# GRatTWCU/Social-STGCNN

Hardware: AMD Instinct MI355X
Metric: scene-windows/sec fwd+bwd (obs=8,pred=12) (higher is better)
Workload: dtype f32; 1 GPU; synthetic V=32 scene-windows, obs 8 / pred 12, batch 2048 per GPU, f32 (BASELINE north-star: V<=32, batch=2048; SURVEY 8d generator); global_batch=2048, step=aggregation + forward + bivariate NLL + backward + SGD update, parallelism=dp1

## Files before the change

include/stgcnn_hip.h:

```cpp
#ifndef STGCNN_HIP_H
#define STGCNN_HIP_H

#include <stddef.h>
#include <stdint.h>

#ifdef __cplusplus
extern "C" {
#endif

#define STG_OK 0
#define STG_EINVAL (-1)
#define STG_EUNSUPPORTED (-2)
#define STG_ELDS (-3)

#define STG_ABI_VERSION 8
#define STG_MAX_BLOCKS 4

int stg_abi_version(void);
const char *stg_last_error(void);

int stg_adj_build(const float *rel, int64_t rel_sn, int64_t rel_sv, int64_t rel_sc, int64_t rel_st,
                  const int32_t *num_peds, int N, int V, int T, int normalize,
                  float *nodes, float *adj, void *stream);

int stg_spatial_agg_fwd(const float *x, int64_t x_sn, int64_t x_sc, int64_t x_st, int64_t x_sv,
                        const float *adj, int64_t a_sn, const int32_t *num_peds,
                        int N, int C, int T, int V, float *y, void *stream);
int stg_spatial_agg_bwd(const float *dy, const float *adj, int64_t a_sn, const int32_t *num_peds,
                        int N, int C, int T, int V, float *dx, void *stream);

int stg_conv_t_fwd(const float *x, int64_t x_sn, int64_t x_sc, int64_t x_st, int64_t x_sv,
                   const float *w, const float *b, const int32_t *num_peds,
                   int N, int Cin, int Cout, int T, int V, int kt, int pad, float *y, void *stream);
int stg_conv_t_bwd(const float *x, int64_t x_sn, int64_t x_sc, int64_t x_st, int64_t x_sv,
                   const float *w, const float *dy, const int32_t *num_peds,
                   int N, int Cin, int Cout, int T, int V, int kt, int pad,
                   float *dx, float *dw, float *db, void *stream);

typedef struct {
    int32_t n_stgcnn;
    int32_t n_txpcnn;
    int32_t c_in;
    int32_t c_out;
    int32_t t_obs;
    int32_t t_pred;
    int32_t kt;
    int32_t residual0;
    int32_t use_mdn;
    int32_t bn_mode;
    float bn_eps;
    float bn_momentum;
    int32_t flags;
    int32_t wg_waves;
} stg_model_desc;

#define STG_OPT_WG_PATH 1
#define STG_OPT_SPLIT_BF16 2
#define STG_OPT_BF16_STORE 8
#define STG_OPT_F32_MFMA 16
#define STG_OPT_SEPARATE_FB 32
#define STG_OPT_GENERIC_WGRAD 64
#define STG_OPT_WAVE_PATH 4

int64_t stg_model_param_count(const stg_model_desc *d);
int64_t stg_model_buffer_count(const stg_model_desc *d);
int64_t stg_model_ws_floats(const stg_model_desc *d, int V);
int64_t stg_model_ws_tail_floats(const stg_model_desc *d, int N, int V);
int64_t stg_model_stat_floats(const stg_model_desc *d);
int64_t stg_model_fwd_scratch_floats(const stg_model_desc *d, int N, int V);
int64_t stg_model_bwd_scratch_floats(const stg_model_desc *d, int N, int V);
int64_t stg_model_fwd_stamps_offset(const stg_model_desc *d, int N, int V);
int64_t stg_model_bwd_stamps_offset(const stg_model_desc *d, int N, int V);

int stg_model_fwd(const stg_model_desc *d, const float *params, const float *buffers,
                  const float *x, int64_t x_sn, int64_t x_sc, int64_t x_st, int64_t x_sv,
                  const float *adj, int64_t a_sn, const int32_t *num_peds, int N, int V,
                  float *y, float *ws, float *stats, float *scratch, void **events, int n_events, void *stream);
int stg_model_bwd(const stg_model_desc *d, const float *params, const float *buffers,
                  const float *x, int64_t x_sn, int64_t x_sc, int64_t x_st, int64_t x_sv,
                  const float *adj, int64_t a_sn, const int32_t *num_peds, int N, int V,
                  const float *dy, const float *ws, float *scratch, float *grad_params, float *dx,
                  void **events, int n_events, void *stream);

int stg_model_bwd_nll(const stg_model_desc *d, const float *params, const float *buffers, const float *x, int64_t x_sn,
                      int64_t x_sc, int64_t x_st, int64_t x_sv, const float *adj, int64_t a_sn, const int32_t *num_peds,
                      int N, int V, const float *y, const float *target, const float *weights, float *losses,
                      const float *ws, float *scratch, float *grad_params, void **events, int n_events, void *stream);

typedef struct stg_step_tail {
    float *params;
    const float *lr_dev;
    float lr;
    const float *stats;
    float *buffers;
    int64_t *const *nbt;
    int n_bn;
    float *total;
} stg_step_tail;
int stg_model_bwd_step(const stg_model_desc *d, const float *params, const float *buffers, const float *x, int64_t x_sn,
                       int64_t x_sc, int64_t x_st, int64_t x_sv, const float *adj, int64_t a_sn, const int32_t *num_peds,
                       int N, int V, const float *y, const float *target, const float *weights, float *losses,
                       const float *ws, float *scratch, float *grad_params, const stg_step_tail *tail, void **events,
                       int n_events, void *stream);
int stg_model_step(const stg_model_desc *d, const float *params, const float *buffers, const float *x, int64_t x_sn,
                   int64_t x_sc, int64_t x_st, int64_t x_sv, const float *adj, int64_t a_sn, const int32_t *num_peds,
                   int N, int V, float *y, float *ws, float *stats, float *fwd_scratch, const float *target,
                   const float *weights, float *losses, float *bwd_scratch, float *grad_params,
                   const stg_step_tail *tail, void **fwd_events, int n_fwd_events, void **bwd_events,
                   int n_bwd_events, void *stream);
int stg_bn_fold(const stg_model_desc *d, const float *stats, const int32_t *num_peds, int N,
                float *buffers, int64_t *const *nbt, int n_bn, void *stream);

int stg_nll_fwd(const float *pred, int64_t p_sn, int64_t p_sf, int64_t p_sp, int64_t p_sv,
                const float *target, const int32_t *num_peds, const float *grad_scale, int N, int P, int V,
                float *loss, float *grad, void *stream);
int stg_nll_bwd(const float *grad, const float *gloss, int N, int P, int V, float *out, void *stream);

int stg_sgd_step(float *params, const float *grads, int64_t count, float lr, void *stream);

int stg_scene_order(const int32_t *num_peds, int N, int V, int32_t *order, int32_t *key_start, void *stream);

int stg_optim_step(float *params, float *grads, int64_t count, const float *lr_dev, float lr, float max_norm,
                   float *grad_norm, void *stream);

int stg_gather_windows(const float *seq_rel_all, const int32_t *win_start, const int32_t *index, int n_windows, int N,
                       int V, int T_obs, int T_pred, float *obs_rel, float *target, int32_t *num_peds, void *stream);

int stg_dp_pack(const float *grads, const float *bn_before, const float *bn_after, const int32_t *num_peds, int N,
                float momentum, int rank, int world, int n_params, int n_buffers, float *pack, void *stream);
int stg_dp_fold(const float *pack, const float *bn_before, float momentum, int rank, int world, int n_params,
                int n_buffers, float *buffers, int64_t *const *nbt, int n_bn, void *stream);
int stg_weighted_sum(const float *values, const float *weights, int N, float *out, void *stream);

int stg_train_tail(const stg_model_desc *d, const float *stats, const int32_t *num_peds, int N, float *buffers,
                   int64_t *const *nbt, int n_bn, const float *losses, const float *weights, float *total,
                   float *params, float *grads, int64_t count, const float *lr_dev, float lr, float max_norm,
                   float *grad_norm, void *stream);

int stg_bestofk_eval(const float *pred, int64_t p_sn, int64_t p_sf, int64_t p_sp, int64_t p_sv,
                     const float *target_rel, const float *obs_last, const int32_t *num_peds, const float *noise,
                     uint64_t seed, int N, int P, int V, int K, float *ade, float *fde, void *stream);

int stg_sample_trajectories(const float *pred, int64_t p_sn, int64_t p_sf, int64_t p_sp, int64_t p_sv,
                            const float *obs_last, const int32_t *num_peds, const float *noise, uint64_t seed,
                            const uint64_t *seed_dev, int N, int P, int V, int K, float *samples, float *mean,
                            void *stream);

#define STG_TRACK_MAX_DETECTIONS 2048
#define STG_TRACK_MAX_SLOTS 2048
#define STG_TRACK_DUPLICATE 1
#define STG_TRACK_OVERFLOW 2
#define STG_TRACK_TRUNCATED 4
#define STG_TRACK_TOO_MANY 8
int stg_frame_scene_counts(const int32_t *frame_start, const int64_t *ids, int F, int T_obs, int32_t *count,
                           void *stream);
int stg_frame_scenes(const int32_t *frame_start, const int64_t *ids, const double *xy, const int32_t *frames, int N,
                     int V, int T_obs, double scale, double *obs_abs, int64_t *out_ids, int32_t *num_peds,
                     void *stream);
int stg_track_push(const int64_t *det_id, const double *det_xy, const int32_t *det_count, int M_max, int64_t *slot_id,
                   uint32_t *mask, double *ring, int32_t *head_flags, int S, int T_obs, double scale, int V,
                   double *obs_abs, int64_t *out_ids, int32_t *num_peds, void *stream);

#define STG_TRACK_MAX_STREAMS 4096
#define STG_TRACK_MAX_TOTAL_DETECTIONS (STG_TRACK_MAX_STREAMS * STG_TRACK_MAX_DETECTIONS)
int stg_track_push_streams(const int64_t *det_id, int64_t id_stride, const double *det_xy, int64_t xy_stride,
                           int M_total, const int32_t *det_start, const int32_t *pushed, int NS, int M_max,
                           int64_t *slot_id, uint32_t *mask, double *ring, int32_t *head_flags, int S, int T_obs,
                           double scale, int V, double *obs_abs, int64_t *out_ids, int32_t *num_peds,
                           int32_t *out_flags, int block_threads, void *stream);

int stg_fill_tracks(double *obs_abs, const int32_t *seen, const int32_t *num_peds, int N, int T_obs, int V,
                    double scale, void *stream);
int stg_frame_scene_counts_rule(const int32_t *frame_start, const int64_t *ids, int F, int T_obs, int min_seen,
                                int max_gap, int32_t *count, void *stream);
int stg_frame_scenes_rule(const int32_t *frame_start, const int64_t *ids, const double *xy, const int32_t *frames,
                          int N, int V, int T_obs, double scale, int min_seen, int max_gap, double *obs_abs,
                          int64_t *out_ids, int32_t *num_peds, int32_t *seen, void *stream);
int stg_track_push_rule(const int64_t *det_id, const double *det_xy, const int32_t *det_count, int M_max,
                        int64_t *slot_id, uint32_t *mask, double *ring, int32_t *head_flags, int S, int T_obs,
                        double scale, int V, int min_seen, int max_gap, double *obs_abs, int64_t *out_ids,
                        int32_t *num_peds, int32_t *seen, void *stream);
int stg_track_push_streams_rule(const int64_t *det_id, int64_t id_stride, const double *det_xy, int64_t xy_stride,
                                int M_total, const int32_t *det_start, const int32_t *pushed, int NS, int M_max,
                                int64_t *slot_id, uint32_t *mask, double *ring, int32_t *head_flags, int S, int T_obs,
                                double scale, int V, int min_seen, int max_gap, double *obs_abs, int64_t *out_ids,
                                int32_t *num_peds, int32_t *out_flags, int32_t *seen, int block_threads,
                                void *stream);

#define STG_TRACK_MAX_HISTORY 256
#define STG_TRACK_TIME_ORDER 16
int stg_track_push_timed(const int64_t *det_id, const double *det_xy, const int32_t *det_count,
                         const int64_t *det_time, int M_max, int64_t *slot_id, int64_t *t_ring, double *xy_ring,
                         int32_t *slot_head, int64_t *clock, int32_t *head_flags, int S, int R, int T_obs, double scale,
                         int V, int64_t step, int64_t max_dt, int min_seen, int max_gap, double *obs_abs,
                         int64_t *out_ids, int32_t *num_peds, int32_t *seen, void *stream);
int stg_track_push_streams_timed(const int64_t *det_id, int64_t id_stride, const double *det_xy, int64_t xy_stride,
                                 int M_total, const int32_t *det_start, const int32_t *pushed, const int64_t *det_time,
                                 int NS, int M_max, int64_t *slot_id, int64_t *t_ring, double *xy_ring,
                                 int32_t *slot_head, int64_t *clock, int32_t *head_flags, int S, int R, int T_obs,
                                 double scale, int V, int64_t step, int64_t max_dt, int min_seen, int max_gap,
                                 double *obs_abs, int64_t *out_ids, int32_t *num_peds, int32_t *out_flags,
                                 int32_t *seen, int block_threads, void *stream);

#define STG_RISK_MAX_V 256
#define STG_RISK_MAX_K 64
#define STG_RISK_MAX_Z 16
#define STG_RISK_MAX_P 32
int stg_sample_risk(const float *pred, int64_t p_sn, int64_t p_sf, int64_t p_sp, int64_t p_sv, const float *obs_last,
                    const int32_t *num_peds, const float *noise, uint64_t seed, const uint64_t *seed_dev, int N, int P,
                    int V, int K, float radius, const float *zones, int64_t z_sn, int Z, int32_t *conflict,
                    int32_t *conflict_any, int32_t *partner, int32_t *pair, int32_t *zone_any, int32_t *zone_count,
                    int32_t *ped_zone, void *stream);

#define STG_SCORE_MAX_V 256
#define STG_SCORE_MAX_K 64
#define STG_SCORE_MAX_P 32
#define STG_SCORE_MAX_Q 4
typedef struct stg_score_state {
    int64_t *rec_ids;
    int32_t *rec_peds;
    float *rec_mean, *rec_cov, *rec_samples, *acc, *acc_mean;
    int32_t *steps, *head;
    double *totals, *traj_totals;
} stg_score_state;
typedef struct stg_score_out {
    int64_t *rec_ids;
    int32_t *matched;
    float *err, *d2, *nll, *best;
    int32_t *traj_steps;
    float *traj_ade, *traj_fde, *traj_ade_mean, *traj_fde_mean;
} stg_score_out;
int stg_score_push(const int64_t *det_id, const double *det_xy, const int32_t *det_count, int M_max, double scale,
                   const float *mean, const float *v_pred, int64_t p_sn, int64_t p_sf, int64_t p_sp, int64_t p_sv,
                   const float *samples, const int64_t *ids, const int32_t *num_peds, int P, int V, int K,
                   const stg_score_state *state, const float *thr, int Q, const stg_score_out *out, void *stream);
int stg_score_push_streams(const int64_t *det_id, int64_t id_stride, const double *det_xy, int64_t xy_stride,
                           int M_total, const int32_t *det_start, const int32_t *pushed, int NS, int M_max,
                           double scale, const float *mean, const float *v_pred, int64_t p_sn, int64_t p_sf,
                           int64_t p_sp, int64_t p_sv, const float *samples, const int64_t *ids,
                           const int32_t *num_peds, int P, int V, int K, const stg_score_state *state,
                           const float *thr, int Q, const stg_score_out *out, void *stream);


#define STG_ASSOC_MAX_SLOTS STG_TRACK_MAX_SLOTS
#define STG_ASSOC_MAX_DETECTIONS STG_TRACK_MAX_DETECTIONS
#define STG_ASSOC_FULL 1
int stg_associate(int64_t *det_id, const double *det_xy, const int32_t *det_count, int M_max, int64_t *trk_id,
                  double *trk_pos, double *trk_vel, int32_t *trk_miss, int32_t *trk_hits, int64_t *next_id,
                  int32_t *assoc_flags, int C, double scale, double gate2, double gate_new2, int max_miss,
                  void *stream);
int stg_associate_streams(int64_t *det_id, int64_t id_stride, const double *det_xy, int64_t xy_stride, int M_total,
                          const int32_t *det_start, const int32_t *pushed, int NS, int M_max, int64_t *trk_id,
                          double *trk_pos, double *trk_vel, int32_t *trk_miss, int32_t *trk_hits, int64_t *next_id,
                          int32_t *assoc_flags, int C, double scale, double gate2, double gate_new2, int max_miss,
                          void *stream);

int stg_selftest_mfma(const float *a, const float *b, int K, float *c, void *stream);

#include "stgcnn_hip_score_time.h"

#include "stgcnn_hip_harvest.h"

#include "stgcnn_hip_harvest_time.h"

#include "stgcnn_hip_assoc_time.h"

#include "stgcnn_hip_assoc_filter.h"

#ifdef __cplusplus
}
#endif
#endif
```

social_stgcnn_amd/_lib.py:

```python
import ctypes
import os
import subprocess

import torch

_HERE = os.path.dirname(os.path.abspath(__file__))
CSRC = os.path.join(_HERE, "csrc")
DIAG = os.environ.get("STG_USE_DIAG_LIB", "0") not in ("", "0")
LIB_PATH = os.path.join(CSRC, "libstgcnn_hip_diag.so" if DIAG else "libstgcnn_hip.so")
ABI_VERSION = 8
OPT_WG_PATH, OPT_SPLIT_BF16, OPT_WAVE_PATH, OPT_BF16_STORE, OPT_F32_MFMA, OPT_SEPARATE_FB = 1, 2, 4, 8, 16, 32
OPT_GENERIC_WGRAD = 64
EUNSUPPORTED = -2

c_f = ctypes.c_void_p
c_i = ctypes.c_int
c_l = ctypes.c_int64


class ModelDesc(ctypes.Structure):
    _fields_ = [("n_stgcnn", ctypes.c_int32), ("n_txpcnn", ctypes.c_int32), ("c_in", ctypes.c_int32),
                ("c_out", ctypes.c_int32), ("t_obs", ctypes.c_int32), ("t_pred", ctypes.c_int32),
                ("kt", ctypes.c_int32), ("residual0", ctypes.c_int32), ("use_mdn", ctypes.c_int32),
                ("bn_mode", ctypes.c_int32), ("bn_eps", ctypes.c_float), ("bn_momentum", ctypes.c_float),
                ("flags", ctypes.c_int32), ("wg_waves", ctypes.c_int32)]


class ScoreState(ctypes.Structure):
    _fields_ = [(n, ctypes.c_void_p) for n in ("rec_ids", "rec_peds", "rec_mean", "rec_cov", "rec_samples", "acc",
                                               "acc_mean", "steps", "head", "totals", "traj_totals")]


class ScoreOut(ctypes.Structure):
    _fields_ = [(n, ctypes.c_void_p) for n in ("rec_ids", "matched", "err", "d2", "nll", "best", "traj_steps",
                                               "traj_ade", "traj_fde", "traj_ade_mean", "traj_fde_mean")]


class ScoreTimedState(ctypes.Structure):
    _fields_ = [(n, ctypes.c_void_p) for n in ("rec_t", "rec_status", "rec_peds", "rec_ids", "rec_mean", "rec_cov",
                                               "rec_samples", "acc", "acc_mean", "steps", "matched", "err", "d2", "nll",
                                               "best", "traj_steps", "traj_ade", "traj_fde", "traj_ade_mean",
                                               "traj_fde_mean", "counters", "totals", "traj_totals")]


class ScoreTimedOut(ctypes.Structure):
    _fields_ = [(n, ctypes.c_void_p) for n in ("push_totals", "push_traj")]


_SIGNATURES = {
    "stg_abi_version": (c_i, []),
    "stg_last_error": (ctypes.c_char_p, []),
    "stg_adj_build": (c_i, [c_f, c_l, c_l, c_l, c_l, c_f, c_i, c_i, c_i, c_i, c_f, c_f, c_f]),
    "stg_spatial_agg_fwd": (c_i, [c_f, c_l, c_l, c_l, c_l, c_f, c_l, c_f, c_i, c_i, c_i, c_i, c_f, c_f]),
    "stg_spatial_agg_bwd": (c_i, [c_f, c_f, c_l, c_f, c_i, c_i, c_i, c_i, c_f, c_f]),
    "stg_conv_t_fwd": (c_i, [c_f, c_l, c_l, c_l, c_l, c_f, c_f, c_f, c_i, c_i, c_i, c_i, c_i, c_i, c_i, c_f, c_f]),
    "stg_conv_t_bwd": (c_i, [c_f, c_l, c_l, c_l, c_l, c_f, c_f, c_f, c_i, c_i, c_i, c_i, c_i, c_i, c_i,
                             c_f, c_f, c_f, c_f]),
    "stg_model_param_count": (c_l, [ctypes.POINTER(ModelDesc)]),
    "stg_model_buffer_count": (c_l, [ctypes.POINTER(ModelDesc)]),
    "stg_model_ws_floats": (c_l, [ctypes.POINTER(ModelDesc), c_i]),
    "stg_model_ws_tail_floats": (c_l, [ctypes.POINTER(ModelDesc), c_i, c_i]),
    "stg_model_stat_floats": (c_l, [ctypes.POINTER(ModelDesc)]),
    "stg_model_fwd_scratch_floats": (c_l, [ctypes.POINTER(ModelDesc), c_i, c_i]),
    "stg_model_bwd_scratch_floats": (c_l, [ctypes.POINTER(ModelDesc), c_i, c_i]),
    "stg_model_fwd_stamps_offset": (c_l, [ctypes.POINTER(ModelDesc), c_i, c_i]),
    "stg_model_bwd_stamps_offset": (c_l, [ctypes.POINTER(ModelDesc), c_i, c_i]),
    "stg_model_fwd": (c_i, [ctypes.POINTER(ModelDesc), c_f, c_f, c_f, c_l, c_l, c_l, c_l, c_f, c_l, c_f, c_i, c_i,
                            c_f, c_f, c_f, c_f, ctypes.POINTER(ctypes.c_void_p), c_i, c_f]),
    "stg_model_bwd": (c_i, [ctypes.POINTER(ModelDesc), c_f, c_f, c_f, c_l, c_l, c_l, c_l, c_f, c_l, c_f, c_i, c_i,
                            c_f, c_f, c_f, c_f, c_f, ctypes.POINTER(ctypes.c_void_p), c_i, c_f]),
    "stg_model_bwd_nll": (c_i, [ctypes.POINTER(ModelDesc), c_f, c_f, c_f, c_l, c_l, c_l, c_l, c_f, c_l, c_f, c_i, c_i,
                                c_f, c_f, c_f, c_f, c_f, c_f, c_f, ctypes.POINTER(ctypes.c_void_p), c_i, c_f]),
    "stg_model_bwd_step": (c_i, [ctypes.POINTER(ModelDesc), c_f, c_f, c_f, c_l, c_l, c_l, c_l, c_f, c_l, c_f, c_i, c_i,
                                 c_f, c_f, c_f, c_f, c_f, c_f, c_f, ctypes.c_void_p, ctypes.POINTER(ctypes.c_void_p), c_i,
                                 c_f]),
    "stg_model_step": (c_i, [ctypes.POINTER(ModelDesc), c_f, c_f, c_f, c_l, c_l, c_l, c_l, c_f, c_l, c_f, c_i, c_i,
                             c_f, c_f, c_f, c_f, c_f, c_f, c_f, c_f, c_f, ctypes.c_void_p,
                             ctypes.POINTER(ctypes.c_void_p), c_i, ctypes.POINTER(ctypes.c_void_p), c_i, c_f]),
    "stg_bn_fold": (c_i, [ctypes.POINTER(ModelDesc), c_f, c_f, c_i, c_f, ctypes.POINTER(ctypes.c_void_p), c_i, c_f]),
    "stg_nll_fwd": (c_i, [c_f, c_l, c_l, c_l, c_l, c_f, c_f, c_f, c_i, c_i, c_i, c_f, c_f, c_f]),
    "stg_nll_bwd": (c_i, [c_f, c_f, c_i, c_i, c_i, c_f, c_f]),
    "stg_sgd_step": (c_i, [c_f, c_f, c_l, ctypes.c_float, c_f]),
    "stg_scene_order": (c_i, [c_f, c_i, c_i, c_f, c_f, c_f]),
    "stg_optim_step": (c_i, [c_f, c_f, c_l, c_f, ctypes.c_float, ctypes.c_float, c_f, c_f]),
    "stg_bestofk_eval": (c_i, [c_f, c_l, c_l, c_l, c_l, c_f, c_f, c_f, c_f, ctypes.c_uint64, c_i, c_i, c_i, c_i,
                               c_f, c_f, c_f]),
    "stg_sample_trajectories": (c_i, [c_f, c_l, c_l, c_l, c_l, c_f, c_f, c_f, ctypes.c_uint64, c_f, c_i, c_i, c_i, c_i,
                                      c_f, c_f, c_f]),
    "stg_sample_risk": (c_i, [c_f, c_l, c_l, c_l, c_l, c_f, c_f, c_f, ctypes.c_uint64, c_f, c_i, c_i, c_i, c_i,
                              ctypes.c_float, c_f, c_l, c_i, c_f, c_f, c_f, c_f, c_f, c_f, c_f, c_f]),
    "stg_gather_windows": (c_i, [c_f, c_f, c_f, c_i, c_i, c_i, c_i, c_i, c_f, c_f, c_f, c_f]),
    "stg_dp_pack": (c_i, [c_f, c_f, c_f, c_f, c_i, ctypes.c_float, c_i, c_i, c_i, c_i, c_f, c_f]),
    "stg_dp_fold": (c_i, [c_f, c_f, ctypes.c_float, c_i, c_i, c_i, c_i, c_f, ctypes.POINTER(ctypes.c_void_p), c_i, c_f]),
    "stg_weighted_sum": (c_i, [c_f, c_f, c_i, c_f, c_f]),
    "stg_train_tail": (c_i, [ctypes.POINTER(ModelDesc), c_f, c_f, c_i, c_f, ctypes.POINTER(ctypes.c_void_p), c_i, c_f, c_f,
                             c_f, c_f, c_f, c_l, c_f, ctypes.c_float, ctypes.c_float, c_f, c_f]),
    "stg_frame_scene_counts": (c_i, [c_f, c_f, c_i, c_i, c_f, c_f]),
    "stg_frame_scenes": (c_i, [c_f, c_f, c_f, c_f, c_i, c_i, c_i, ctypes.c_double, c_f, c_f, c_f, c_f]),
    "stg_track_push": (c_i, [c_f, c_f, c_f, c_i, c_f, c_f, c_f, c_f, c_i, c_i, ctypes.c_double, c_i, c_f, c_f, c_f,
                             c_f]),
    "stg_track_push_streams": (c_i, [c_f, c_l, c_f, c_l, c_i, c_f, c_f, c_i, c_i, c_f, c_f, c_f, c_f, c_i, c_i,
                                     ctypes.c_double, c_i, c_f, c_f, c_f, c_f, c_i, c_f]),
    "stg_fill_tracks": (c_i, [c_f, c_f, c_f, c_i, c_i, c_i, ctypes.c_double, c_f]),
    "stg_frame_scene_counts_rule": (c_i, [c_f, c_f, c_i, c_i, c_i, c_i, c_f, c_f]),
    "stg_frame_scenes_rule": (c_i, [c_f, c_f, c_f, c_f, c_i, c_i, c_i, ctypes.c_double, c_i, c_i, c_f, c_f, c_f, c_f,
                                    c_f]),
    "stg_track_push_rule": (c_i, [c_f, c_f, c_f, c_i, c_f, c_f, c_f, c_f, c_i, c_i, ctypes.c_double, c_i, c_i, c_i,
                                  c_f, c_f, c_f, c_f, c_f]),
    "stg_track_push_streams_rule": (c_i, [c_f, c_l, c_f, c_l, c_i, c_f, c_f, c_i, c_i, c_f, c_f, c_f, c_f, c_i, c_i,
                                          ctypes.c_double, c_i, c_i, c_i, c_f, c_f, c_f, c_f, c_f, c_i, c_f]),
    "stg_track_push_timed": (c_i, [c_f, c_f, c_f, c_f, c_i, c_f, c_f, c_f, c_f, c_f, c_f, c_i, c_i, c_i,
                                   ctypes.c_double, c_i, c_l, c_l, c_i, c_i, c_f, c_f, c_f, c_f, c_f]),
    "stg_track_push_streams_timed": (c_i, [c_f, c_l, c_f, c_l, c_i, c_f, c_f, c_f, c_i, c_i, c_f, c_f, c_f, c_f, c_f,
                                           c_f, c_i, c_i, c_i, ctypes.c_double, c_i, c_l, c_l, c_i, c_i, c_f, c_f, c_f,
                                           c_f, c_f, c_i, c_f]),
    "stg_score_push": (c_i, [c_f, c_f, c_f, c_i, ctypes.c_double, c_f, c_f, c_l, c_l, c_l, c_l, c_f, c_f, c_f, c_i, c_i,
                             c_i, ctypes.POINTER(ScoreState), c_f, c_i, ctypes.POINTER(ScoreOut), c_f]),
    "stg_score_push_streams": (c_i, [c_f, c_l, c_f, c_l, c_i, c_f, c_f, c_i, c_i, ctypes.c_double, c_f, c_f, c_l, c_l,
                                     c_l, c_l, c_f, c_f, c_f, c_i, c_i, c_i, ctypes.POINTER(ScoreState), c_f, c_i,
                                     ctypes.POINTER(ScoreOut), c_f]),
    "stg_associate": (c_i, [c_f, c_f, c_f, c_i, c_f, c_f, c_f, c_f, c_f, c_f, c_f, c_i, ctypes.c_double,
                            ctypes.c_double, ctypes.c_double, c_i, c_f]),
    "stg_associate_streams": (c_i, [c_f, c_l, c_f, c_l, c_i, c_f, c_f, c_i, c_i, c_f, c_f, c_f, c_f, c_f, c_f, c_f,
                                    c_i, ctypes.c_double, ctypes.c_double, ctypes.c_double, c_i, c_f]),
    "stg_selftest_mfma": (c_i, [c_f, c_f, c_i, c_f, c_f]),
}
EXPORTS = tuple(_SIGNATURES)
_SIGNATURES_SCORE_TIME = {
    "stg_score_push_timed": (c_i, [c_f, c_f, c_f, c_f, c_f, c_f, c_i, c_i, ctypes.c_double, c_l, c_l, c_f, c_f, c_l, c_l,
                                   c_l, c_l, c_f, c_f, c_f, c_i, c_i, c_i, c_i, c_f, c_f, c_i, c_f, c_f]),
    "stg_score_push_streams_timed": (c_i, [c_f, c_f, c_f, c_f, c_f, c_f, c_f, c_i, c_i, c_i, ctypes.c_double, c_l, c_l,
                                           c_f, c_f, c_l, c_l, c_l, c_l, c_f, c_f, c_f, c_i, c_i, c_i, c_i, c_f, c_f, c_i,
                                           c_f, c_f]),
}
_SIGNATURES_HARVEST = {
    "stg_window_harvest": (c_i, [c_f, c_f, c_f, c_f, c_i, c_i, c_i, c_i, c_i, c_f, c_f, c_f, c_f, c_f, c_f, c_f, c_i, c_i,
                                 c_f]),
    "stg_window_harvest_streams": (c_i, [c_f, c_f, c_f, c_f, c_f, c_i, c_i, c_i, c_i, c_i, c_f, c_f, c_f, c_f, c_f, c_f,
                                         c_f, c_f, c_i, c_i, c_f]),
}
c_d = ctypes.c_double
_SIGNATURES_HARVEST_TIME = {
    "stg_window_harvest_timed": (c_i, [c_f, c_f, c_f, c_f, c_f, c_f, c_i, c_i, c_i, c_i, c_i, c_d, c_l, c_l, c_l, c_i,
                                       c_f, c_f, c_f, c_f, c_f, c_f, c_f, c_f, c_i, c_i, c_f]),
    "stg_window_harvest_streams_timed": (c_i, [c_f, c_f, c_f, c_f, c_f, c_f, c_f, c_i, c_i, c_i, c_i, c_i, c_i, c_d, c_l,
                                               c_l, c_l, c_f, c_f, c_f, c_f, c_f, c_f, c_f, c_f, c_f, c_i, c_i, c_f]),
}
_SIGNATURES_ASSOC_TIME = {
    "stg_associate_timed": (c_i, [c_f, c_f, c_f, c_f, c_f, c_i, c_f, c_f, c_f, c_f, c_f, c_f, c_f, c_i, c_d, c_d, c_d, c_l,
                                  c_l, c_f]),
    "stg_associate_streams_timed": (c_i, [c_f, c_l, c_f, c_l, c_i, c_f, c_f, c_f, c_f, c_i, c_i, c_f, c_f, c_f, c_f, c_f,
                                          c_f, c_f, c_i, c_d, c_d, c_d, c_l, c_l, c_f]),
}
_SIGNATURES_ASSOC_FILTER = {
    "stg_associate_filtered": (c_i, [c_f, c_f, c_f, c_f, c_f, c_i, c_f, c_f, c_f, c_f, c_f, c_f, c_f, c_f, c_i, c_d, c_d,
                                     c_d, c_d, c_d, c_d, c_l, c_l, c_f]),
    "stg_associate_streams_filtered": (c_i, [c_f, c_l, c_f, c_l, c_i, c_f, c_f, c_f, c_f, c_i, c_i, c_f, c_f, c_f, c_f,
                                             c_f, c_f, c_f, c_f, c_i, c_d, c_d, c_d, c_d, c_d, c_d, c_l, c_l, c_f]),
}

_lib = None


def build(verbose=False):
    cmd = ["make", "-C", CSRC, "-j8"] + (["DIAG=1"] if DIAG else [])
    res = subprocess.run(cmd, stdout=subprocess.PIPE, stderr=subprocess.STDOUT, text=True)
    if verbose or res.returncode != 0:
        print(res.stdout)
    if res.returncode != 0:
        raise RuntimeError("building libstgcnn_hip.so failed (exit %d)" % res.returncode)
    return LIB_PATH


def lib():
    global _lib
    if _lib is None:
        if not os.path.exists(LIB_PATH):
            raise RuntimeError(
                "social_stgcnn_amd: %s is missing -- build it with `make -C %s` (hipcc, "
                "--offload-arch=gfx950) or `python -c 'import __graft_entry__ as g; g.build()'`. "
                "There is no CPU or eager-PyTorch fallback for this path." % (LIB_PATH, CSRC))
        h = ctypes.CDLL(LIB_PATH)
        for name, (res, args) in {**_SIGNATURES, **_SIGNATURES_SCORE_TIME, **_SIGNATURES_HARVEST,
                                    **_SIGNATURES_HARVEST_TIME, **_SIGNATURES_ASSOC_TIME,
                                    **_SIGNATURES_ASSOC_FILTER}.items():
            fn = getattr(h, name)
            fn.restype = res
            fn.argtypes = args
        if h.stg_abi_version() != ABI_VERSION:
            raise RuntimeError("libstgcnn_hip.so ABI %d != binding ABI %d" % (h.stg_abi_version(), ABI_VERSION))
        _lib = h
    return _lib


class StepTail(ctypes.Structure):
    _fields_ = [("params", ctypes.c_void_p), ("lr_dev", ctypes.c_void_p), ("lr", ctypes.c_float),
                ("stats", ctypes.c_void_p), ("buffers", ctypes.c_void_p), ("nbt", ctypes.POINTER(ctypes.c_void_p)),
                ("n_bn", ctypes.c_int), ("total", ctypes.c_void_p)]


class HipEvents:
    _hip = None

    @classmethod
    def hip(cls):
        if cls._hip is None:
            h = ctypes.CDLL("libamdhip64.so")
            h.hipEventCreate.argtypes = [ctypes.POINTER(ctypes.c_void_p)]
            h.hipEventElapsedTime.argtypes = [ctypes.POINTER(ctypes.c_float), ctypes.c_void_p, ctypes.c_void_p]
            h.hipEventSynchronize.argtypes = [ctypes.c_void_p]
            h.hipEventDestroy.argtypes = [ctypes.c_void_p]
            cls._hip = h
        return cls._hip

    def __init__(self, n):
        self.n = n
        self.arr = (ctypes.c_void_p * n)()
        for i in range(n):
            ev = ctypes.c_void_p()
            if self.hip().hipEventCreate(ctypes.byref(ev)) != 0:
                raise RuntimeError("hipEventCreate failed")
            self.arr[i] = ev

    def intervals_ms(self):
        out = []
        self.hip().hipEventSynchronize(self.arr[self.n - 1])
        for k in range(1, self.n):
            ms = ctypes.c_float()
            if self.hip().hipEventElapsedTime(ctypes.byref(ms), self.arr[k - 1], self.arr[k]) != 0:
                raise RuntimeError("hipEventElapsedTime failed")
            out.append(ms.value)
        return out

    def __del__(self):
        try:
            for i in range(self.n):
                self.hip().hipEventDestroy(self.arr[i])
        except Exception:
            pass


def check(rc, what):
    if rc != 0:
        msg = lib().stg_last_error().decode("utf-8", "replace")
        raise RuntimeError("%s failed (status %d): %s" % (what, rc, msg))


def stream_ptr():
    return ctypes.c_void_p(torch.cuda.current_stream().cuda_stream)


def ptr(t):
    if t is None:
        return None
    return ctypes.c_void_p(t.data_ptr())


def require_gpu(*tensors):
    for t in tensors:
        if t is not None and not t.is_cuda:
            raise RuntimeError("social_stgcnn_amd runs on MI355X only: got a %s tensor (no CPU fallback)"
                               % t.device.type)


def seed_u64(seed):
    return int(seed) & 0xFFFFFFFFFFFFFFFF


def seed_i64(seed):
    s = seed_u64(seed)
    return s - (1 << 64) if s >= 1 << 63 else s


def as_f32(t, what):
    if t.dtype != torch.float32:
        raise TypeError("%s must be float32 (got %s)" % (what, t.dtype))
    return t


def peds_arg(num_peds, n, device):
    if num_peds is None:
        return None
    if not torch.is_tensor(num_peds):
        num_peds = torch.as_tensor(num_peds, dtype=torch.int32)
    num_peds = num_peds.to(device=device, dtype=torch.int32).contiguous()
    if num_peds.numel() != n:
        raise ValueError("num_peds has %d entries for a batch of %d scenes" % (num_peds.numel(), n))
    return num_peds
```

social_stgcnn_amd/csrc/model_bwd.hip:

```cpp
#include "model_common.hpp"
#include "stgcn_block.hpp"
#include "txp_scene_common.hpp"
#include "txp_f32_operands.hpp"
#include "step_plan.hpp"
#include "txp_wgrad.hpp"
#include "tail_parts.hpp"
#include "nll_elem.hpp"

namespace stg {

struct BwdArgs {
    ModelLayout lay;
    const float *params, *buffers, *x;
    int64_t x_sn, x_sc, x_st, x_sv;
    const float *adj;
    int64_t a_sn;
    const int32_t *num_peds;
    int N, V;
    const float *dy, *ws;
    const float *nll_target, *nll_weights;
    float *nll_losses;
    int64_t ws_stride;
    float *slab1;
    float *dzg;
// ... 93 lines not shown
    const ModelLayout &L = a.lay;
    const int scmax = txp_sc(Vl);
    const int plane_floats = P * scmax;
    const int st_floats = (2 * C * (T + 2) + C * T) * Vl;
    const int reg_floats = plane_floats > st_floats ? plane_floats : st_floats;
    const int dcur_floats = P * C * Vl;
    const int n_small = L.n_blk_params + L.n_txp;
    float *gsm = sm;
    float *dzb = gsm + ((n_small + 3) & ~3);
    float *dcur = dzb + reg_floats;
    float *red = dcur + dcur_floats;
    float *tot = red + WAVES * kRedMax;
    const float *Pm = params;
    __shared__ float nll_part[WAVES];

    for (int e = tid; e < n_small; e += NT) gsm[e] = 0.f;

    int t_begin, t_end;
    tier_range(a.tier, a.N, V, t_begin, t_end);
    const int M = t_end - t_begin;
    for (int r = 0; r * (int)gridDim.x < M; ++r) {
        const int it = walk_item(r, blockIdx.x, gridDim.x, M, a.tier.order != nullptr && a.tier.serpentine);
        if (it < 0) continue;
        const int n = a.tier.order ? a.tier.order[t_begin + it] : it;
        int vi = a.num_peds ? a.num_peds[n] : V;
        vi = vi < 0 ? 0 : (vi > V ? V : vi);
        float *dxn = a.dx ? a.dx + (int64_t)n * L.blk[0].cin * T * V : nullptr;
        if (dxn && vi < V)
            for (int e = tid; e < L.blk[0].cin * T * (V - vi); e += NT) {
                const int r = e / (V - vi), w = vi + (e - r * (V - vi));
                dxn[(int64_t)r * V + w] = 0.f;
            }
        if (vi == 0) {
            if (a.nll_target && tid == 0) a.nll_losses[n] = 0.f;
            continue;
        }
        const float *wsn = a.ws + n * a.ws_stride;
        const int SW = txp_sw(vi), SC = txp_sc(vi), npos = C * vi;
        const int out_rows = L.n_txp > 0 ? C * P : C * T;
        const float *dyn = a.dy + (int64_t)n * out_rows * V;
        __syncthreads();
        if (L.n_txp > 0) {
            for (int e = tid; e < P * SC; e += NT) dzb[e] = 0.f;
            __syncthreads();
            for (int l = L.L; l >= 0; --l) {
                const bool is_out = l == L.L;
                if (is_out) {
                    float *dzo = a.dzg + ((int64_t)n * (L.L + 1) + L.L) * dz_slot(V);
                    constexpr int U = 4;
                    if (a.nll_target) {
                        bwd_nll_stage(dyn, a.nll_target + (int64_t)n * P * V * 2, a.nll_weights ? a.nll_weights[n] : 1.f,
                                      vi, V, SC, SW, dzb, dzo, nll_part, a.nll_losses + n);
                    } else
                    for (int e0 = tid; e0 < P * npos; e0 += NT * U) {
                        float dv[U];
                        int li[U];
#pragma unroll
                        for (int u = 0; u < U; ++u) {
                            const int e = e0 + u * NT;
                            const int ec = e < P * npos ? e : 0;
                            const int ch = ec / npos, p = ec - ch * npos, h = p / vi, w = p - h * vi;
                            li[u] = ch * SC + (h + 1) * SW + (w + 1);
                            dv[u] = dyn[(int64_t)(ch * C + h) * V + w];
                        }
#pragma unroll
                        for (int u = 0; u < U; ++u)
                            if (e0 + u * NT < P * npos) {
                                const int e = e0 + u * NT, ch = e / npos;
                                dzb[li[u]] = dv[u];
                                dzo[(e - ch * npos) * P + ch] = dv[u];
                            }
                    }
                    __syncthreads();
                } else {
                    const float *zl = wsn + L.ws_hdr_floats + (int64_t)L.ws_z[l] * V;
                    float *dzo = a.dzg + ((int64_t)n * (L.L + 1) + l) * dz_slot(V);
                    const float alpha = Pm[L.prelus + l];
                    float s[1] = {0.f};
                    constexpr int U = 4;
                    for (int e0 = tid; e0 < P * npos; e0 += NT * U) {
                        float zv[U];
#pragma unroll
                        for (int u = 0; u < U; ++u) {
                            const int e = e0 + u * NT;
                            zv[u] = e < P * npos ? zl[e] : 1.f;
                        }
#pragma unroll
                        for (int u = 0; u < U; ++u) {
                            const int e = e0 + u * NT;
                            if (e < P * npos) {
                                const int ch = e / npos, p = e - ch * npos, h = p / vi, w = p - h * vi;
                                const float z = zv[u], d = dcur[e];
                                float dz = d;
                                if (!(z > 0.f)) {
                                    dz = alpha * d;
                                    s[0] = fmaf(d, z, s[0]);
                                }
                                dzb[ch * SC + (h + 1) * SW + (w + 1)] = dz;
                                dzo[p * P + ch] = dz;
                            }
                        }
                    }
                    block_reduce<1, WAVES>(s, red, tot);
                    if (tid == 0) gsm[L.n_blk_params + l] += tot[0];
                }
                const int w_off = is_out ? L.out_w : L.txp_w[l];
                if (!STG_SKIP(a, 2)) {
                    if (l == 0)
                        txp_dgrad<Cfg::T, WAVES>(Pm + w_off, dzb, dcur, vi, false);
                    else
                        txp_dgrad<Cfg::P, WAVES>(Pm + w_off, dzb, dcur, vi, !is_out);
                }
                __syncthreads();
            }
        } else {
            for (int e = tid; e < C * T * vi; e += NT) {
                const int r = e / vi, w = e - r * vi;
                dcur[e] = dyn[(int64_t)r * V + w];
            }
            __syncthreads();
        }
        float *H1 = dzb, *DH2 = dzb + C * (T + 2) * Vl, *DB1 = DH2 + C * (T + 2) * Vl;
        for (int j = L.n_blocks - 1; j >= 0 && !STG_SKIP(a, 4); --j) {
            const float *xin = j > 0 ? wsn + L.ws_hdr_floats + (int64_t)L.blk[j - 1].ws_s * V : nullptr;
            float *dxs = j > 0 ? dcur : nullptr;
            float *dxg = j == 0 ? dxn : nullptr;
            if (L.blk[j].cin == Cfg::CIN0)
                stgcn_block_bwd<Cfg::CIN0, WAVES, true>(a, params, L.blk[j], n, vi, dcur, H1, DH2, DB1, red, tot, gsm, wsn,
                                                        xin, dxs, dxg, nullptr);
            else
                stgcn_block_bwd<Cfg::C, WAVES, true>(a, params, L.blk[j], n, vi, dcur, H1, DH2, DB1, red, tot, gsm, wsn, xin,
                                                     dxs, dxg, nullptr);
        }
    }
    __syncthreads();
    float *slab = a.slab1 + (int64_t)blockIdx.x * n_small;
    for (int e = tid; e < n_small; e += NT) slab[e] = gsm[e];
}

struct ReduceSeg {
    int p0, len, rows, row_stride;
    int64_t base;
};
struct ReduceArgs {
    ReduceSeg seg[kMaxTxp + 3];
    int n_seg;
    const float *slabs;
    float *grad;
    int n_params;
};

struct TailArgs {
    float *params;
    const float *lr_dev;
    float lr;
    const float *stats, *losses, *weights;
    const int32_t *num_peds;
    float *buffers, *total;
    NbtPtrs nbt;
    int n_reduce, n_buffers, N, stat_floats;
    float momentum;
};

__global__ __launch_bounds__(256) void reduce_slabs_kernel(const ReduceArgs a, const TailArgs t_) {
    __shared__ float part[32][8];
    if ((int)blockIdx.x >= t_.n_reduce) {
        float *acc_s = &part[0][0];
        __shared__ float dec_s[256];
        __shared__ int cnt_s[256];
        const int b = (int)blockIdx.x - t_.n_reduce;
        if (b < t_.n_buffers)
            bn_fold_body<256>(b, t_.stats, t_.num_peds, t_.N, t_.stat_floats, t_.momentum, t_.buffers, t_.nbt, acc_s, dec_s,
                              cnt_s);
        else if (t_.total)
            weighted_sum_body(t_.losses, t_.weights, t_.N, t_.total, acc_s);
        return;
    }
    const int col = threadIdx.x & 7, grp = threadIdx.x >> 3;
    const int p = blockIdx.x * 8 + col;
    float s = 0.f;
    if (p < a.n_params) {
        for (int q = 0; q < a.n_seg; ++q) {
            const ReduceSeg g = a.seg[q];
            if (p >= g.p0 && p < g.p0 + g.len) {
                const float *src = a.slabs + g.base + (p - g.p0);
                int k = grp;
                for (; k + 992 < g.rows; k += 1024) {
                    float v[32];
#pragma unroll
                    for (int u = 0; u < 32; ++u) v[u] = src[(int64_t)(k + 32 * u) * g.row_stride];
#pragma unroll
                    for (int u = 0; u < 32; ++u) s += v[u];
                }
                for (; k + 480 < g.rows; k += 512) {
                    float v[16];
#pragma unroll
                    for (int u = 0; u < 16; ++u) v[u] = src[(int64_t)(k + 32 * u) * g.row_stride];
#pragma unroll
                    for (int u = 0; u < 16; ++u) s += v[u];
                }
                for (; k + 96 < g.rows; k += 128) {
                    float v[4];
#pragma unroll
                    for (int u = 0; u < 4; ++u) v[u] = src[(int64_t)(k + 32 * u) * g.row_stride];
#pragma unroll
                    for (int u = 0; u < 4; ++u) s += v[u];
                }
                for (; k < g.rows; k += 32) s += src[(int64_t)k * g.row_stride];
            }
        }
    }
    part[grp][col] = s;
    __syncthreads();
    if (grp == 0 && p < a.n_params) {
        float t = 0.f;
#pragma unroll
        for (int g = 0; g < 32; ++g) t += part[g][col];
        a.grad[p] = t;
        if (t_.params) t_.params[p] -= (t_.lr_dev ? t_.lr_dev[0] : t_.lr) * t;
    }
}

static size_t bwd_lds_bytes(const ModelLayout &L, int V, int waves) {
    const int plane = Cfg::P * txp_sc(V);
    const int st = (2 * Cfg::C * (Cfg::T + 2) + Cfg::C * Cfg::T) * V;
    const int reg = plane > st ? plane : st;
    const int dcur = Cfg::P * Cfg::C * V;
    const int n_small = L.n_blk_params + L.n_txp;
    const size_t fl = ((n_small + 3) & ~3) + (size_t)reg + (size_t)dcur + (size_t)waves * kRedMax + kRedMax;
    return fl * sizeof(float);
}

static int bwd_waves(const StepPath &path, int V) {
    return path.wg_waves ? path.wg_waves : (V <= 40 ? 1 : (V <= 80 ? 4 : 8));
}

static int bwd_grid_w(const ModelLayout &L, int N, int V, int waves) {
    const size_t lds = bwd_lds_bytes(L, V, waves);
    if (lds > (size_t)kLdsBytes) return -1;
    int per_cu = (int)(kLdsBytes / lds);
    const int by_waves = 8 / waves > 0 ? 8 / waves : 1;
    if (per_cu > by_waves) per_cu = by_waves;
    if (per_cu < 1) per_cu = 1;
    int grid = kNumCU * per_cu;
    if (const int g = diag_env("STG_BWD_GRID", 0)) grid = g > 0 ? g : grid;
    return grid < N ? grid : N;
}
static int bwd_grid(const ModelLayout &L, const StepPath &path, int N, int V) { return bwd_grid_w(L, N, V, bwd_waves(path, V)); }
constexpr int kBwdTierV = 32;
static int bwd_grid_small(const ModelLayout &L, int N, int V) {
    return V > kBwdTierV ? bwd_grid_w(L, N, kBwdTierV, 1) : 0;
}

struct BwdCarve {
    int64_t rows, slab2, dzg, order, stamps, total;
};
static bool bwd_carve(const ModelLayout &L, const StepPath &path, int N, int V, BwdCarve *c, WgradGeom *wg) {
    const int g1 = bwd_grid(L, path, N, V);
    if (g1 < 0) return false;
    int gs = bwd_grid_small(L, N, V);
    if (gs < 0) gs = 0;
    int64_t n_rows = g1 + gs;
    if (path.scene() && N > n_rows) n_rows = N;
    c->rows = 0;
    int64_t fl = (n_rows * (L.n_blk_params + L.n_txp) + 3) & ~(int64_t)3;
    c->slab2 = fl;
    c->dzg = fl;
    if (L.n_txp > 0) {
        if (!wgrad_geom(L, N, V, wg)) return false;
        fl = (fl + wgrad_slab_base(L.L + 1, wg->rows) + 3) & ~(int64_t)3;
        c->dzg = fl;
        fl = (fl + (int64_t)N * (L.L + 1) * dz_slot(V) + 3) & ~(int64_t)3;
    }
    c->order = fl;
    c->total = fl + order_floats(N, V);
    c->stamps = -1;
    if (diag_env("STG_STAMPS", 0) != 0) {
        c->stamps = c->total;
        c->total += (int64_t)N * 32;
    }
    return true;
}

static int64_t bwd_query(const char *what, const stg_model_desc *d, int N, int V, int64_t BwdCarve::*item) {
    StepPlan p;
    const int rc = plan_sized(what, d, nullptr, N, V, 1, &p);
    if (rc != STG_OK) return rc;
    BwdCarve c;
    WgradGeom wg{};
    STG_REQUIRE(bwd_carve(p.lay, p.path, N, V, &c, &wg), STG_ELDS, "stg_model_bwd: V=%d does not fit the LDS of one CU", V);
    return c.*item >= 0 ? c.*item : STG_EUNSUPPORTED;
}

}

extern "C" {

int64_t stg_model_bwd_scratch_floats(const stg_model_desc *d, int N, int V) {
    return stg::bwd_query("stg_model_bwd_scratch_floats:", d, N, V, &stg::BwdCarve::total);
}
int64_t stg_model_bwd_stamps_offset(const stg_model_desc *d, int N, int V) {
    return stg::bwd_query("stg_model_bwd_stamps_offset:", d, N, V, &stg::BwdCarve::stamps);
}

}

namespace stg {

int model_bwd_impl(const ModelCall &c, const BwdBuffers &b, const StepPlan &p, const TxpFwdArgs *deferred) {
    const SceneInput &in = c.in;
    const int N = in.N, V = in.V;
    const ModelLayout &L = p.lay;
    STG_REQUIRE(b.grad_params, STG_EINVAL, "stg_model_bwd: null grad_params");
    STG_REQUIRE(N == 0 || (c.params && c.buffers && in.x && in.adj && b.dy && b.ws && b.scratch), STG_EINVAL,
                "stg_model_bwd: null pointer");
    STG_REQUIRE(aligned(b.ws, 16) && aligned(b.scratch, 16), STG_EINVAL, "stg_model_bwd: ws / scratch must be 16-byte aligned");
    hipStream_t st = as_stream(c.stream);
    EventList evl{b.events, b.events ? b.n_events : 0, 0, st};
    evl.mark();
    if (N == 0) {
        hipError_t e = hipMemsetAsync(b.grad_params, 0, sizeof(float) * L.n_params, st);
        if (e != hipSuccess) return hip_fail(e, "stg_model_bwd: memset");
        return STG_OK;
    }
    BwdCarve cv;
    WgradGeom wg{};
    const StepPath &path = p.path;
    STG_REQUIRE(bwd_carve(L, path, N, V, &cv, &wg), STG_ELDS, "stg_model_bwd: V=%d does not fit the LDS of one CU", V);
    const int n_small = L.n_blk_params + L.n_txp;
    float *rows = b.scratch + cv.rows, *slab2 = b.scratch + cv.slab2;
    float *dzg = L.n_txp > 0 ? b.scratch + cv.dzg : nullptr;
    STG_REQUIRE(path.scene() || !(L.flags & STG_OPT_BF16_STORE), STG_EUNSUPPORTED,
                "stg_model_bwd: bf16 storage (STG_OPT_BF16_STORE) is built for the wave-per-scene kernels only");
    STG_REQUIRE(!((L.flags & STG_OPT_BF16_STORE) && (L.flags & STG_OPT_SPLIT_BF16)), STG_EUNSUPPORTED,
                "stg_model_bwd: STG_OPT_BF16_STORE and STG_OPT_SPLIT_BF16 cannot be combined");
    if (b.nll_target && ((L.flags & STG_OPT_SPLIT_BF16) || L.n_txp == 0))
        return STG_EUNSUPPORTED;
    STG_REQUIRE(!(path.scene() && b.dx), STG_EUNSUPPORTED,
                "stg_model_bwd: dx is only computed by the workgroup-per-scene kernels: set STG_OPT_WG_PATH in the "
                "descriptor of the forward and the backward call");
    const float *ws_end = b.ws + p.tail.base;
    const bool in_tail = tail_has_order(path, in.num_peds, N, V);
    float *order = in_tail ? const_cast<float *>(ws_end) + p.tail.order : b.scratch + cv.order;
    const SceneOrder so = scene_order_at(reinterpret_cast<int32_t *>(order), N, V);
    const bool sorted = in_tail || launch_scene_order(in.num_peds, N, V, so, st);
    const SceneTier tier{sorted ? so.order : nullptr, sorted ? so.key_start : nullptr, -1, V, diag_env("STG_WALK", 1)};
    const auto fill = [&](auto &a) {
        set_input(a, c);
        a.lay = L; a.ws_stride = p.ws_stride; a.ws = b.ws; a.dzg = dzg;
        a.debug_skip = diag_env("STG_DEBUG_SKIP", 0);
    };
    const auto fill_k1 = [&](auto &a) {
        fill(a);
        a.dy = b.dy; a.nll_target = b.nll_target; a.nll_weights = b.nll_weights; a.nll_losses = b.nll_losses;
        a.tier = tier;
    };
    int slab_rows;
    if (path.scene()) {
        TxpBwdArgs t{};
        fill_k1(t);
        t.rows = rows; t.Vl = V;
        t.split_bf16 = (L.flags & STG_OPT_SPLIT_BF16) ? 1 : 0;
        t.stagger = diag_env("STG_STAGGER_B", 0);
        if (p.tail.wp >= 0) t.wp = reinterpret_cast<const unsigned *>(ws_end + p.tail.wp);
        if (cv.stamps >= 0) t.stamps = reinterpret_cast<unsigned long long *>(b.scratch + cv.stamps);
        STG_REQUIRE(!deferred || p.one_launch, STG_EINVAL, "stg_model_bwd: a deferred scene launch outside the one-launch step");
        const int rcw = deferred ? launch_scene_step(*deferred, t, st) : launch_scene_bwd(path, t, st);
        if (rcw != STG_OK) return rcw;
        slab_rows = N;
    } else {
        STG_REQUIRE(!deferred, STG_EINVAL, "stg_model_bwd: a deferred scene launch outside the one-launch step");
        BwdArgs a{};
        fill_k1(a);
        a.buffers = c.buffers; a.slab1 = rows; a.dx = b.dx;
        const int waves = bwd_waves(path, V);
        const size_t lds = bwd_lds_bytes(L, V, waves);
        STG_REQUIRE(lds <= (size_t)kLdsBytes, STG_ELDS, "stg_model_bwd: V=%d needs %zu bytes of LDS (> %d)", V, lds,
                    kLdsBytes);
        const int grid = bwd_grid(L, path, N, V);
        void (*k1)(BwdArgs, const float *);
        switch (waves) {
            case 1: k1 = model_bwd_kernel<1>; break;
            case 2: k1 = model_bwd_kernel<2>; break;
            case 4: k1 = model_bwd_kernel<4>; break;
            default: k1 = model_bwd_kernel<8>; break;
        }
        slab_rows = grid;
        const int grid_small = a.tier.order ? bwd_grid_small(L, N, V) : 0;
        if (grid_small > 0) a.tier.v_lo = kBwdTierV;
        int rck = launch(Launch{"stg_model_bwd: K1", dim3(grid), dim3(waves * 64), lds, st}, k1, a, c.params);
        if (rck != STG_OK) return rck;
        if (grid_small > 0) {
            a.Vl = kBwdTierV;
            a.tier.v_lo = -1; a.tier.v_hi = kBwdTierV;
            a.slab1 = rows + (int64_t)grid * n_small;
            rck = launch(Launch{"stg_model_bwd: K1 (small scenes)", dim3(grid_small), dim3(64), bwd_lds_bytes(L, kBwdTierV, 1), st},
                         model_bwd_kernel<1>, a, c.params);
            if (rck != STG_OK) return rck;
            slab_rows = grid + grid_small;
        }
    }
    evl.mark();

    ReduceArgs r{};
    r.slabs = b.scratch;
    r.grad = b.grad_params;
    r.n_params = L.n_params;
    r.seg[r.n_seg++] = ReduceSeg{0, L.n_blk_params, slab_rows, n_small, cv.rows};
    if (L.n_txp > 0) {
        r.seg[r.n_seg++] = ReduceSeg{L.prelus, L.n_txp, slab_rows, n_small, cv.rows + (int64_t)L.n_blk_params};
        WgradArgs w{};
        fill(w);
        w.order = tier.order; w.order_peds = sorted ? so.order_peds : nullptr; w.key_start = tier.key_start;
        w.serpentine = tier.serpentine;
        w.slab2 = slab2; w.rows = wg.rows;
        for (int l = 0; l <= L.L + 1; ++l) w.wg_begin[l] = wg.wg_begin[l];
        if (!STG_SKIP(w, 1)) {
            const int rck = launch_txp_wgrad(w, wg, st);
            if (rck != STG_OK) return rck;
        }
        evl.mark();
        for (int l = 0; l <= L.L; ++l) {
            const int p0 = l == L.L ? L.out_w : L.txp_w[l];
            r.seg[r.n_seg++] = ReduceSeg{p0, wgrad_row_len(l), STG_SKIP(w, 1) ? 0 : wg.wg_begin[l + 1] - wg.wg_begin[l],
                                         wgrad_row_len(l), cv.slab2 + wgrad_slab_base(l, wg.rows)};
        }
    }
    TailArgs ta{};
    ta.n_reduce = (L.n_params + 7) / 8;
    int extra = 0;
    if (const stg_step_tail *tail = b.tail) {
        ta.params = tail->params; ta.lr_dev = tail->lr_dev; ta.lr = tail->lr;
        ta.stats = tail->stats; ta.buffers = tail->buffers; ta.total = tail->total;
        ta.losses = b.nll_losses; ta.weights = b.nll_weights; ta.num_peds = in.num_peds;
        ta.N = N; ta.stat_floats = L.stat_floats; ta.momentum = c.d->bn_momentum;
        ta.n_buffers = (tail->stats && N > 0) ? L.n_buffers : 0;
        ta.nbt.n = tail->nbt ? tail->n_bn : 0;
        for (int k = 0; k < ta.nbt.n; ++k) ta.nbt.p[k] = tail->nbt[k];
        extra = ta.n_buffers + 1;
    }
    hipLaunchKernelGGL(reduce_slabs_kernel, dim3(ta.n_reduce + extra), dim3(256), 0, st, r, ta);
    STG_LAUNCH_CHECK("stg_model_bwd: reduce_slabs");
    evl.mark();
    evl.finish();
    return STG_OK;
}

static bool tail_ok(const stg_step_tail *tail) {
    return tail && tail->params && !(tail->stats && !tail->buffers) && tail->n_bn >= 0 && tail->n_bn <= 3 * STG_MAX_BLOCKS;
}

static int run_bwd(const ModelCall &c, const BwdBuffers &b) {
    StepPlan p;
    const int rc = plan_sized("stg_model_bwd: bad sizes", c.d, c.in.num_peds, c.in.N, c.in.V, 0, &p);
    return rc != STG_OK ? rc : model_bwd_impl(c, b, p, nullptr);
}

}

extern "C" {

using namespace stg;

int stg_model_bwd(const stg_model_desc *d, const float *params, const float *buffers, const float *x, int64_t x_sn,
                  int64_t x_sc, int64_t x_st, int64_t x_sv, const float *adj, int64_t a_sn, const int32_t *num_peds,
                  int N, int V, const float *dy, const float *ws, float *scratch, float *grad_params, float *dx,
                  void **events, int n_events, void *stream) {
    const ModelCall c{d, params, buffers, {x, x_sn, x_sc, x_st, x_sv, adj, a_sn, num_peds, N, V}, stream};
    return run_bwd(c, BwdBuffers{dy, nullptr, nullptr, nullptr, nullptr, ws, scratch, grad_params, dx, events, n_events});
}

int stg_model_bwd_nll(const stg_model_desc *d, const float *params, const float *buffers, const float *x, int64_t x_sn,
                      int64_t x_sc, int64_t x_st, int64_t x_sv, const float *adj, int64_t a_sn, const int32_t *num_peds,
                      int N, int V, const float *y, const float *target, const float *weights, float *losses,
                      const float *ws, float *scratch, float *grad_params, void **events, int n_events, void *stream) {
    if (!target || !losses || (N > 0 && !y)) return fail(STG_EINVAL, "stg_model_bwd_nll: null pointer");
    const ModelCall c{d, params, buffers, {x, x_sn, x_sc, x_st, x_sv, adj, a_sn, num_peds, N, V}, stream};
    return run_bwd(c, BwdBuffers{y, target, weights, losses, nullptr, ws, scratch, grad_params, nullptr, events, n_events});
}

int stg_model_bwd_step(const stg_model_desc *d, const float *params, const float *buffers, const float *x, int64_t x_sn,
                       int64_t x_sc, int64_t x_st, int64_t x_sv, const float *adj, int64_t a_sn, const int32_t *num_peds,
                       int N, int V, const float *y, const float *target, const float *weights, float *losses,
                       const float *ws, float *scratch, float *grad_params, const stg_step_tail *tail, void **events,
                       int n_events, void *stream) {
    if (!target || !losses || (N > 0 && !y)) return fail(STG_EINVAL, "stg_model_bwd_step: null pointer");
    if (!tail_ok(tail)) return fail(STG_EINVAL, "stg_model_bwd_step: bad tail");
    if (N == 0) return STG_EUNSUPPORTED;
    const ModelCall c{d, params, buffers, {x, x_sn, x_sc, x_st, x_sv, adj, a_sn, num_peds, N, V}, stream};
    return run_bwd(c, BwdBuffers{y, target, weights, losses, tail, ws, scratch, grad_params, nullptr, events, n_events});
}

int stg_model_step(const stg_model_desc *d, const float *params, const float *buffers, const float *x, int64_t x_sn,
                   int64_t x_sc, int64_t x_st, int64_t x_sv, const float *adj, int64_t a_sn, const int32_t *num_peds,
                   int N, int V, float *y, float *ws, float *stats, float *fwd_scratch, const float *target,
                   const float *weights, float *losses, float *bwd_scratch, float *grad_params,
                   const stg_step_tail *tail, void **fwd_events, int n_fwd_events, void **bwd_events,
                   int n_bwd_events, void *stream) {
    if (!target || !losses || !y || !ws) return fail(STG_EINVAL, "stg_model_step: null pointer");
    if (!tail_ok(tail)) return fail(STG_EINVAL, "stg_model_step: bad tail");
    StepPlan p;
    const int rc = plan_sized("stg_model_step: bad sizes", d, num_peds, N, V, 0, &p);
    if (rc != STG_OK) return rc;
    if (N == 0 || (p.lay.flags & STG_OPT_SPLIT_BF16) || p.lay.n_txp == 0) return STG_EUNSUPPORTED;
    STG_REQUIRE(grad_params && bwd_scratch, STG_EINVAL, "stg_model_step: null pointer");
    const ModelCall c{d, params, buffers, {x, x_sn, x_sc, x_st, x_sv, adj, a_sn, num_peds, N, V}, stream};
    TxpFwdArgs f{};
    TxpFwdArgs *both = p.one_launch ? &f : nullptr;
    const int rcf = model_fwd_impl(c, FwdBuffers{y, ws, stats, fwd_scratch, fwd_events, n_fwd_events}, p, both);
    if (rcf != STG_OK) return rcf;
    return model_bwd_impl(c, BwdBuffers{y, target, weights, losses, tail, ws, bwd_scratch, grad_params, nullptr, bwd_events,
                                        n_bwd_events}, p, both);
}

}
```

social_stgcnn_amd/csrc/model_layout.hip:

```cpp
#include <cstring>
#include <type_traits>
#include "model_common.hpp"
#include "scene_order.hpp"
#include "step_plan.hpp"
#include "txp_wave.hpp"

namespace stg {

int make_layout(const stg_model_desc *d, ModelLayout *lay) {
    STG_REQUIRE(d && lay, STG_EINVAL, "model descriptor is null");
    STG_REQUIRE(d->n_stgcnn >= 1 && d->n_stgcnn <= STG_MAX_BLOCKS, STG_EUNSUPPORTED,
                "n_stgcnn=%d outside 1..%d", d->n_stgcnn, STG_MAX_BLOCKS);
    STG_REQUIRE(d->n_txpcnn >= 0 && d->n_txpcnn <= kMaxTxp, STG_EUNSUPPORTED, "n_txpcnn=%d outside 0..%d",
                d->n_txpcnn, kMaxTxp);
    STG_REQUIRE(d->c_out == Cfg::C && d->t_obs == Cfg::T && d->kt == Cfg::KT, STG_EUNSUPPORTED,
                "fused kernels are built for output_feat=%d seq_len=%d kernel_size=%d (got %d,%d,%d)", Cfg::C,
                Cfg::T, Cfg::KT, d->c_out, d->t_obs, d->kt);
    STG_REQUIRE(d->c_in == Cfg::CIN0 || d->c_in == Cfg::C, STG_EUNSUPPORTED,
                "fused kernels are built for input_feat %d or %d (got %d)", Cfg::CIN0, Cfg::C, d->c_in);
    STG_REQUIRE(d->n_txpcnn == 0 || d->t_pred == Cfg::P, STG_EUNSUPPORTED,
                "fused kernels are built for pred_seq_len=%d (got %d)", Cfg::P, d->t_pred);
    STG_REQUIRE(d->bn_mode == 0 || d->bn_mode == 1, STG_EINVAL, "bn_mode=%d (0 eval, 1 per-scene train)", d->bn_mode);
    STG_REQUIRE(d->residual0 >= 0 && d->residual0 <= 2, STG_EINVAL, "residual0=%d", d->residual0);
    STG_REQUIRE(d->residual0 != 1 || d->c_in == d->c_out, STG_EINVAL, "identity residual needs c_in == c_out");
    STG_REQUIRE((d->flags & ~(STG_OPT_WG_PATH | STG_OPT_SPLIT_BF16 | STG_OPT_WAVE_PATH | STG_OPT_BF16_STORE | STG_OPT_F32_MFMA |
                              STG_OPT_SEPARATE_FB | STG_OPT_GENERIC_WGRAD)) == 0, STG_EINVAL,
                "unknown flags 0x%x", d->flags);
    STG_REQUIRE(d->wg_waves == 0 || d->wg_waves == 1 || d->wg_waves == 2 || d->wg_waves == 4 || d->wg_waves == 8,
                STG_EINVAL, "wg_waves=%d (0 auto, 1, 2, 4, 8)", d->wg_waves);
    ModelLayout &l = *lay;
    l = layout_of(ModelShape{d->n_stgcnn, d->n_txpcnn, d->c_in, d->residual0, d->use_mdn});
    l.bn_mode = d->bn_mode;
    l.eps = d->bn_eps;
    l.momentum = d->bn_momentum;
    l.flags = d->flags;
    l.wg_waves = d->wg_waves;
    return STG_OK;
}

bool is_canonical(const ModelLayout &L) {
    ModelLayout c = L;
    c.eps = kCanonLayout.eps;
    c.momentum = kCanonLayout.momentum;
    c.bn_mode = kCanonLayout.bn_mode;
    c.flags = kCanonLayout.flags;
    c.wg_waves = kCanonLayout.wg_waves;
    static_assert(std::is_trivially_copyable<ModelLayout>::value && sizeof(ModelLayout) % 4 == 0, "compared bytewise");
    return std::memcmp(&c, &kCanonLayout, sizeof c) == 0;
}

constexpr int kSmallBatch = 288;

static StepPath choose_path(const ModelLayout &L, int N, int V) {
    StepPath p{StepPath::Workgroup, L.wg_waves, txp_fwd_x6_fits(L, V), txp_bwd_x6_fits(L, V)};
    if (L.n_txp < 1 || L.n_blocks != 1 || L.blk[0].cin != Cfg::CIN0 || (L.flags & STG_OPT_WG_PATH)) return p;
    if (p.fwd_x6 && p.bwd_x6) {
        p.kind = StepPath::SceneX6;
    } else if (txp_wave_f32_fits(V)) {
        if (N >= kSmallBatch || L.wg_waves != 0 || V > 40 || (L.flags & (STG_OPT_WAVE_PATH | STG_OPT_BF16_STORE)))
            p.kind = StepPath::WaveF32;
        else
            p.wg_waves = N <= 192 ? 8 : 4;
    }
    return p;
}

static FwdCarve fwd_carve(const ModelLayout &L, const StepPath &path, int N, int V) {
    const bool stamps = diag_env("STG_STAMPS", 0) != 0;
    FwdCarve c;
    c.agg = 0;
    c.order = (((int64_t)N * (L.blk[0].cin + 1) * Cfg::T * V + 3) & ~(int64_t)3) + 4;
    c.stamps = stamps ? c.order + order_floats(N, V) : -1;
    const int64_t wp = (c.order + order_floats(N, V) + (stamps ? (int64_t)N * 32 : 0) + 3) & ~(int64_t)3;
    c.wp_fwd = path.scene() && path.fwd_x6 ? wp : -1;
    c.total = wp + (path.fwd_x6 ? txp_bwd_x6_wp_floats(L) : 0);
    return c;
}

static WsTail ws_tail(const ModelLayout &L, const StepPath &path, int N, int V) {
    WsTail t;
    t.base = (int64_t)N * ws_floats_per_scene(L, V);
    t.wp = path.scene() && path.bwd_x6 ? 0 : -1;
    t.order = path.bwd_x6 ? txp_bwd_x6_wp_floats(L) : 0;
    t.total = t.order + order_floats(N, V);
    return t;
}

int launch_scene_fwd(const StepPath &path, const TxpFwdArgs &a, hipStream_t st) {
    return path.fwd_x6 ? launch_txp_fwd_x6(a, st) : launch_txp_fwd_wave(a, st);
}
int launch_scene_bwd(const StepPath &path, const TxpBwdArgs &a, hipStream_t st) {
    return path.bwd_x6 ? launch_txp_bwd_x6(a, st) : launch_txp_bwd_wave(a, st);
}

static bool step_one_launch(const ModelLayout &L, const StepPath &path, const int32_t *num_peds, int N, int V) {
    return path.kind == StepPath::SceneX6 && path.fwd_x6 && path.bwd_x6 && !(L.flags & STG_OPT_SEPARATE_FB) &&
           txp_step_x6_fits(L, num_peds, N, V);
}
int launch_scene_step(const TxpFwdArgs &f, const TxpBwdArgs &b, hipStream_t st) { return launch_txp_step_x6(f, b, st); }

int plan_step(const stg_model_desc *d, const int32_t *num_peds, int N, int V, StepPlan *p) {
    const int rc = make_layout(d, &p->lay);
    p->sized = rc == STG_OK && N >= 0 && V > 0;
    if (!p->sized) return rc;
    const ModelLayout &L = p->lay;
    p->path = choose_path(L, N, V);
    p->ws_stride = ws_floats_per_scene(L, V);
    p->tail = ws_tail(L, p->path, N, V);
    p->fwd = fwd_carve(L, p->path, N, V);
    p->one_launch = step_one_launch(L, p->path, num_peds, N, V);
    return STG_OK;
}
int plan_sized(const char *what, const stg_model_desc *d, const int32_t *num_peds, int N, int V, int min_N, StepPlan *p) {
    const int rc = plan_step(d, num_peds, N, V, p);
    if (rc != STG_OK) return rc;
    STG_REQUIRE(p->sized && N >= min_N, STG_EINVAL, "%s N=%d V=%d", what, N, V);
    return STG_OK;
}

__global__ __launch_bounds__(1024) void scene_order_kernel(const int32_t *__restrict__ num_peds, int N, int V,
                                                           int32_t *__restrict__ order,
                                                           int32_t *__restrict__ key_start,
                                                           int32_t *__restrict__ order_peds) {
    extern __shared__ int hist[];
    __shared__ int wave_tot[16];
    scene_order_body<16>(num_peds, N, V, order, key_start, order_peds, hist, wave_tot);
}

bool launch_scene_order(const int32_t *num_peds, int N, int V, const SceneOrder &o, hipStream_t st) {
    if (!o.order || !scene_order_applies(num_peds, N, V)) return false;
    const size_t lds = (size_t)(V + 1) * 16 * sizeof(int);
    if (lds > 48 * 1024 &&
        hipFuncSetAttribute(reinterpret_cast<const void *>(&scene_order_kernel),
                            hipFuncAttributeMaxDynamicSharedMemorySize, (int)lds) != hipSuccess)
        return false;
    hipLaunchKernelGGL(scene_order_kernel, dim3(1), dim3(1024), lds, st, num_peds, N, V, o.order, o.key_start, o.order_peds);
    return hipGetLastError() == hipSuccess;
}

}

extern "C" {

static int64_t layout_query(const stg_model_desc *d, int32_t stg::ModelLayout::*count) {
    stg::ModelLayout l;
    const int rc = stg::make_layout(d, &l);
    return rc == STG_OK ? l.*count : rc;
}
int64_t stg_model_param_count(const stg_model_desc *d) { return layout_query(d, &stg::ModelLayout::n_params); }
int64_t stg_model_buffer_count(const stg_model_desc *d) { return layout_query(d, &stg::ModelLayout::n_buffers); }
int64_t stg_model_stat_floats(const stg_model_desc *d) { return layout_query(d, &stg::ModelLayout::stat_floats); }
int64_t stg_model_ws_floats(const stg_model_desc *d, int V) {
    stg::ModelLayout l;
    const int rc = stg::make_layout(d, &l);
    if (rc != STG_OK) return rc;
    if (V <= 0) return stg::fail(STG_EINVAL, "stg_model_ws_floats: V=%d", V);
    return stg::ws_floats_per_scene(l, V);
}
int64_t stg_model_ws_tail_floats(const stg_model_desc *d, int N, int V) {
    stg::StepPlan p;
    const int rc = stg::plan_sized("stg_model_ws_tail_floats:", d, nullptr, N, V, 0, &p);
    return rc == STG_OK ? p.tail.total : rc;
}
int64_t stg_model_fwd_scratch_floats(const stg_model_desc *d, int N, int V) {
    stg::StepPlan p;
    const int rc = stg::plan_sized("stg_model_fwd_scratch_floats:", d, nullptr, N, V, 0, &p);
    return rc == STG_OK ? p.fwd.total : rc;
}
int64_t stg_model_fwd_stamps_offset(const stg_model_desc *d, int N, int V) {
    stg::StepPlan p;
    const int rc = stg::plan_sized("stg_model_fwd_stamps_offset:", d, nullptr, N, V, 0, &p);
    return rc != STG_OK ? rc : p.fwd.stamps >= 0 ? p.fwd.stamps : STG_EUNSUPPORTED;
}
int stg_scene_order(const int32_t *num_peds, int N, int V, int32_t *order, int32_t *key_start, void *stream) {
    STG_REQUIRE(N >= 0 && V > 0, STG_EINVAL, "stg_scene_order: bad sizes N=%d V=%d", N, V);
    if (N == 0) return STG_OK;
    STG_REQUIRE(num_peds && order, STG_EINVAL, "stg_scene_order: null pointer");
    STG_REQUIRE(N >= 2, STG_EUNSUPPORTED, "stg_scene_order: a single scene needs no order");
    STG_REQUIRE(N <= stg::kOrderMaxN && V <= stg::kOrderMaxV, STG_EUNSUPPORTED,
                "stg_scene_order: N=%d V=%d outside the single-workgroup sort (N <= %d, V <= %d)", N, V,
                stg::kOrderMaxN, stg::kOrderMaxV);
    STG_REQUIRE(stg::launch_scene_order(num_peds, N, V, stg::SceneOrder{order, key_start, nullptr}, stg::as_stream(stream)),
                STG_EINVAL, "stg_scene_order: launch failed");
    return STG_OK;
}

}
```

social_stgcnn_amd/csrc/step_plan.hpp:

```cpp
#pragma once
#include "model_common.hpp"

namespace stg {

struct TxpFwdArgs;
struct TxpBwdArgs;

struct StepPath {
    enum Kind { SceneX6, WaveF32, Workgroup } kind;
    int wg_waves;
    bool fwd_x6, bwd_x6;
    bool scene() const { return kind != Workgroup; }
};

struct FwdCarve {
    int64_t agg, order, stamps, wp_fwd, total;
};

struct WsTail {
    int64_t base, wp, order, total;
};
inline bool tail_has_order(const StepPath &path, const int32_t *num_peds, int N, int V) {
    return path.scene() && scene_order_applies(num_peds, N, V);
}

int launch_scene_fwd(const StepPath &path, const TxpFwdArgs &a, hipStream_t st);
int launch_scene_bwd(const StepPath &path, const TxpBwdArgs &a, hipStream_t st);

int launch_scene_step(const TxpFwdArgs &f, const TxpBwdArgs &b, hipStream_t st);

struct StepPlan {
    ModelLayout lay;
    bool sized, one_launch;
    StepPath path;
    int64_t ws_stride;
    WsTail tail;
    FwdCarve fwd;
};
int plan_step(const stg_model_desc *d, const int32_t *num_peds, int N, int V, StepPlan *p);
int plan_sized(const char *what, const stg_model_desc *d, const int32_t *num_peds, int N, int V, int min_N, StepPlan *p);

struct SceneInput {
    const float *x; int64_t x_sn, x_sc, x_st, x_sv; const float *adj; int64_t a_sn; const int32_t *num_peds; int N, V;
};
struct ModelCall { const stg_model_desc *d; const float *params, *buffers; SceneInput in; void *stream; };
struct FwdBuffers { float *y, *ws, *stats, *scratch; void **events; int n_events; };
struct BwdBuffers {
    const float *dy, *nll_target, *nll_weights; float *nll_losses;
    const stg_step_tail *tail;
    const float *ws; float *scratch, *grad_params, *dx; void **events; int n_events;
};

template <class A> constexpr auto has_batch(int) -> decltype(A::x, true) { return true; }
template <class A> constexpr bool has_batch(...) { return false; }
template <class A>
void set_input(A &a, const ModelCall &c) {
    const SceneInput &in = c.in;
    a.num_peds = in.num_peds; a.N = in.N; a.V = in.V;
    if constexpr (has_batch<A>(0)) {
        a.params = c.params; a.x = in.x; a.x_sn = in.x_sn; a.x_sc = in.x_sc; a.x_st = in.x_st; a.x_sv = in.x_sv;
        a.adj = in.adj; a.a_sn = in.a_sn;
    }
}

int model_fwd_impl(const ModelCall &c, const FwdBuffers &b, const StepPlan &p, TxpFwdArgs *defer);
int model_bwd_impl(const ModelCall &c, const BwdBuffers &b, const StepPlan &p, const TxpFwdArgs *deferred);

}
```

social_stgcnn_amd/csrc/txp_scene_common.hpp:

```cpp
#pragma once
#include "model_common.hpp"
#include "stgcn_block.hpp"

namespace stg {

struct MixGeom {
    int on;
    int v_small, v_mid;
    int block_floats;
};

constexpr int kTeamMaxV = 128;
struct TeamGeom {
    int on;
    int v1, v2;
    int region_floats;
};

struct TxpFwdArgs {
    ModelLayout lay;
    const float *params, *buffers;
    const int32_t *num_peds;
    SceneTier tier;
    int Vl;
    MixGeom mix;
    TeamGeom team;
    int N, V;
    const float *x;
    int64_t x_sn, x_sc, x_st, x_sv;
    const float *adj;
    int64_t a_sn;
    const float *agg;
    int64_t agg_stride, agg_ax, agg_cs;
    float *y;
    const unsigned *wpf;
    float *ws;
    int64_t ws_stride;
    float *stats;
    unsigned long long *stamps;
    int debug_skip;
    int stagger;
};

struct TxpBwdArgs {
    ModelLayout lay;
    const float *params;
    const int32_t *num_peds;
    SceneTier tier;
    int Vl;
    MixGeom mix;
    TeamGeom team;
    int N, V;
    const float *x;
    int64_t x_sn, x_sc, x_st, x_sv;
    const float *adj;
    int64_t a_sn;
    const float *dy;
    const float *nll_target;
    const float *nll_weights;
    float *nll_losses;
    const float *ws;
    int64_t ws_stride;
    float *dzg;
    const unsigned *wp;
    float *rows;
    unsigned long long *stamps;
    int debug_skip;
    int split_bf16;
    int stagger;
};

bool txp_fwd_x6_fits(const ModelLayout &L, int V);
bool txp_bwd_x6_fits(const ModelLayout &L, int V);
int64_t txp_bwd_x6_wp_floats(const ModelLayout &L);
int launch_txp_fwd_x6(const TxpFwdArgs &a, hipStream_t st);
int launch_txp_bwd_x6(const TxpBwdArgs &a, hipStream_t st);
bool txp_step_x6_fits(const ModelLayout &L, const int32_t *num_peds, int N, int V);
int launch_txp_step_x6(const TxpFwdArgs &f, const TxpBwdArgs &b, hipStream_t st);

__host__ __device__ inline int ptab_floats(int v) { return ((Cfg::T * v + 1) / 2 + 3) & ~3; }
__host__ __device__ inline int bwd_ptab_floats(int v) { return ptab_floats(v) + kRedMax; }
__host__ __device__ inline int wave_param_floats(const ModelLayout &L) {
    return ((L.n_blk_params + 3) & ~3) + ((L.n_buffers + 3) & ~3);
}

__device__ __forceinline__ void build_ptab(ptab_t *ptab, int vi) {
    const int lane = threadIdx.x & 63;
    for (int p = lane; p < Cfg::T * vi; p += 64) {
        const int h = p / vi;
        ptab[p] = (ptab_t)((h << 8) | (p - h * vi));
    }
}
__device__ __forceinline__ void build_ptab(ptab_t *ptab, int w0, int wc) {
    const int lane = threadIdx.x & 63;
    if (wc <= 0 && lane == 0) ptab[0] = 0;
    for (int p = lane; p < Cfg::T * wc; p += 64) {
        const int h = p / wc;
        ptab[p] = (ptab_t)((h << 8) | (w0 + p - h * wc));
    }
}


__device__ __forceinline__ void vm_drain() { __builtin_amdgcn_s_waitcnt(0x0F70); }

__device__ __forceinline__ void stage_block_params(const ModelLayout &L, const float *__restrict__ params,
                                                   const float *__restrict__ buffers, float *blk_p, float *blk_b, int nt) {
    for (int e = threadIdx.x; e < L.n_blk_params; e += nt) blk_p[e] = params[e];
    if (buffers)
        for (int e = threadIdx.x; e < L.n_buffers; e += nt) blk_b[e] = buffers[e];
    __syncthreads();
}

inline int wave_wpb(size_t per_wave) {
    int wpb = diag_env("STG_TXP_WPB", 4);
    if (wpb != 1 && wpb != 2 && wpb != 8) wpb = 4;
    while (wpb > 1 && per_wave * wpb > (size_t)kLdsBytes) wpb >>= 1;
    return wpb;
}

inline int wave_grid(size_t lds, int wpb, int N) {
    int per_cu = (int)(kLdsBytes / lds);
    if (per_cu * wpb > 8) per_cu = 8 / wpb;
    if (per_cu < 1) per_cu = 1;
    const int need = (N + wpb - 1) / wpb;
    const int g = kNumCU * per_cu;
    if (g >= need) return need;
    const int rounds = (need + g - 1) / g;
    return (need + rounds - 1) / rounds;
}

}
```

social_stgcnn_amd/csrc/txp_wgrad.hip:

```cpp
#include "txp_wgrad.hpp"

namespace stg {

namespace {

constexpr int C = Cfg::C, P = Cfg::P;
constexpr int kWaves = 8;

__device__ __forceinline__ void wait_vmcnt(int n) {
    switch (n) {
        case 0: asm volatile("s_waitcnt vmcnt(0)" ::: "memory"); break;
        case 1: asm volatile("s_waitcnt vmcnt(1)" ::: "memory"); break;
        case 2: asm volatile("s_waitcnt vmcnt(2)" ::: "memory"); break;
        case 3: asm volatile("s_waitcnt vmcnt(3)" ::: "memory"); break;
        case 4: asm volatile("s_waitcnt vmcnt(4)" ::: "memory"); break;
        case 5: asm volatile("s_waitcnt vmcnt(5)" ::: "memory"); break;
        case 6: asm volatile("s_waitcnt vmcnt(6)" ::: "memory"); break;
        case 7: asm volatile("s_waitcnt vmcnt(7)" ::: "memory"); break;
        case 8: asm volatile("s_waitcnt vmcnt(8)" ::: "memory"); break;
        default: asm volatile("s_waitcnt vmcnt(0)" ::: "memory"); break;
    }
}

__device__ __forceinline__ void dma_piece(const float *__restrict__ src, float *lds_dst, int nvec, int piece) {
    const int lane = threadIdx.x & 63;
    const int e = piece * 64 + lane;
    const unsigned dst = __builtin_amdgcn_readfirstlane(
        (unsigned)(uintptr_t)(__attribute__((address_space(3))) float *)(lds_dst + 256 * piece));
    if (e < nvec) {
        const float *g = src + 4 * e;
        unsigned keep;
        asm volatile("s_mov_b32 %0, m0\n\ts_mov_b32 m0, %2\n\ts_nop 0\n\tglobal_load_lds_dwordx4 %1, off\n\ts_mov_b32 m0, %0"
                     : "=&s"(keep)
                     : "v"(g), "s"(dst)
                     : "memory");
    }
}

struct Item {
    int vi, w0, vc;
    bool valid;
    const float *pl, *dz;
};

template <int CINL, int NBUF, bool BF>
__device__ __forceinline__ void wgrad_layer(const WgradArgs &a, const int32_t *__restrict__ order,
                                            const int32_t *__restrict__ order_peds, const int32_t *__restrict__ num_peds,
                                            int layer, float *sm, int wg, int nwg) {
    constexpr int NCOL = 9 * CINL + 1, NTILE = (NCOL + 15) / 16;
    const ModelLayout &L = a.lay;
    const int V = a.V, tid = threadIdx.x, lane = tid & 63;
    const int wave = __builtin_amdgcn_readfirstlane(tid >> 6);
    const int nq = lane & 15, kq = lane >> 4;
    const int co_a = nq < P ? nq : P - 1;
    constexpr int ES = BF ? 2 : 4;
    const int image = wgrad_image_floats(V, BF), pslot = wgrad_plane_floats(V, BF);
    auto ld = [&](const float *base, int idx) -> float {
        if (BF) return __uint_as_float((unsigned)reinterpret_cast<const unsigned short *>(base)[idx] << 16);
        return base[idx];
    };
    const int nch = wgrad_chunks(V), items = a.N * nch;
    const int64_t plane_off = ws_plane_off(L, V, layer), dzs_floats = dz_slot(V);
    int tapr[NTILE], tapc[NTILE], cic[NTILE];
    bool bone[NTILE];
#pragma unroll
    for (int tl = 0; tl < NTILE; ++tl) {
        int col = tl * 16 + nq;
        bone[tl] = col == NCOL - 1;
        if (col > NCOL - 2) col = NCOL - 2;
        const int tap = col / CINL;
        cic[tl] = col - tap * CINL;
        tapr[tl] = tap / 3 - 1;
        tapc[tl] = tap % 3 - 1;
    }
    f32x4 acc[NTILE];
#pragma unroll
    for (int tl = 0; tl < NTILE; ++tl) acc[tl] = f32x4{0.f, 0.f, 0.f, 0.f};

    struct Raw { int at, n, v; };
    auto fetch = [&](int r) -> Raw {
        Raw w{-1, 0, 0};
        w.at = walk_item(r, wg, nwg, items, order != nullptr && a.serpentine);
        if (w.at >= 0) {
            const int si = nch > 1 ? w.at / nch : w.at;
            w.n = order ? order[si] : si;
            w.v = order ? order_peds[si] : (num_peds ? num_peds[si] : V);
        }
        return w;
    };
    auto finish = [&](const Raw &w) -> Item {
        Item it{0, 0, 0, false, nullptr, nullptr};
        if (w.at < 0) return it;
        const int chunk = nch > 1 ? w.at - (w.at / nch) * nch : 0;
        const int vfull = w.v < 0 ? 0 : (w.v > V ? V : w.v);
        const int nc = wgrad_chunks(vfull);
        if (vfull == 0 || chunk >= nc) return it;
        int wc = vfull;
        if (nc > 1) wc = (vfull + nc - 1) / nc;
        if (BF && nc > 1) wc = (wc + 1) & ~1;
        it.pl = a.ws + w.n * a.ws_stride + plane_off;
        it.dz = a.dzg + ((int64_t)w.n * (L.L + 1) + layer) * dzs_floats;
        it.vi = vfull;
        it.w0 = chunk * wc;
        it.vc = (vfull - it.w0) < wc ? (vfull - it.w0) : wc;
        it.valid = true;
        return it;
    };
    auto stage = [&](const Item &it, float *buf) -> int {
        if (!it.valid || STG_SKIP(a, 64)) return 0;
        const int vi = it.vi, vc = it.vc, w0 = it.w0;
        const int SWf = save_sw(vi, BF), VWf = save_vw(vi, BF);
        const int SWc = save_sw(vc, BF), VWc = save_vw(vc, BF);
        if (tid < 2 * SWc * 3) {
            const int b = tid / 3, q = tid - b * 3;
            const int pos = b < SWc ? b : (C + 1) * SWc + (b - SWc);
            store_vec4(buf, pos * 3 + q, f32x4{0.f, 0.f, 0.f, 0.f}, BF);
        }
        const float *pl = it.pl, *dz = it.dz;
        int issued = 0;
        if (vc == vi) {
            const int nv0 = (C * SWf * P * ES + 15) >> 4, nv1 = (C * VWf * P * ES + 15) >> 4;
            const int np0 = (nv0 + 63) >> 6, np1 = (nv1 + 63) >> 6;
            for (int q = wave; q < np0 + np1; q += kWaves) {
                if (q < np0) dma_piece(pl, buf + (SWc * P * ES) / 4, nv0, q);
                else dma_piece(dz, buf + pslot, nv1, q - np0);
                ++issued;
            }
        } else {
            const int nvp = (SWc * P * ES + 15) >> 4, nvd = (vc * P * ES + 15) >> 4;
            const int npp = (nvp + 63) >> 6, npd = (nvd + 63) >> 6;
            for (int q = wave; q < C * (npp + npd); q += kWaves) {
                if (q < C * npp) {
                    const int h = q / npp, pc = q - h * npp;
                    dma_piece(pl + ((int64_t)(h * SWf + w0) * P * ES) / 4, buf + ((h + 1) * SWc * P * ES) / 4, nvp, pc);
                } else {
                    const int q2 = q - C * npp, h = q2 / npd, pc = q2 - h * npd;
                    dma_piece(dz + ((int64_t)(h * VWf + w0) * P * ES) / 4, buf + pslot + (h * VWc * P * ES) / 4, nvd, pc);
                }
                ++issued;
            }
        }
        return issued;
    };
    auto compute = [&](const Item &it, const float *buf) {
        if (!it.valid || STG_SKIP(a, 128)) return;
        const float *plane = buf, *dzs = buf + pslot;
        const int vc = it.vc, SW = save_sw(vc, BF), VW = save_vw(vc, BF), npos = C * vc, nsteps = (npos + 3) >> 2;
        unsigned inv = (unsigned)(65536.0f * __builtin_amdgcn_rcpf((float)vc));
        while (inv * (unsigned)vc < 65536u) ++inv;
        while ((inv - 1u) * (unsigned)vc >= 65536u) --inv;
        int boff[NTILE];
#pragma unroll
        for (int tl = 0; tl < NTILE; ++tl) boff[tl] = (tapr[tl] * SW + tapc[tl]) * P + cic[tl];
        for (int s = wave; s < nsteps; s += kWaves) {
            const int p = 4 * s + kq;
            const bool ok = p < npos;
            const int pc = ok ? p : 0;
            const int hh = (int)(((unsigned)pc * inv) >> 16), ww = pc - hh * vc;
            const float av = ok ? ld(dzs, (hh * VW + ww) * P + co_a) : 0.f;
            const int offb = ((hh + 1) * SW + (ww + 1)) * P;
            float raw[NTILE];
#pragma unroll
            for (int tl = 0; tl < NTILE; ++tl) raw[tl] = ld(plane, boff[tl] + offb);
#pragma unroll
            for (int tl = 0; tl < NTILE; ++tl)
                acc[tl] = __builtin_amdgcn_mfma_f32_16x16x4f32(av, bone[tl] ? 1.f : raw[tl], acc[tl], 0, 0, 0);
        }
    };

    constexpr int D = NBUF - 1;
    const int rounds = (items + nwg - 1) / nwg;
    Item q[D + 1];
    Raw nxt;
    int ahead[D];
#pragma unroll
    for (int j = 0; j < D + 1; ++j) q[j] = finish(fetch(j));
    nxt = fetch(D + 1);
#pragma unroll
    for (int j = 0; j < D; ++j) {
        const int c = stage(q[j], sm + (j % NBUF) * image);
        if (j > 0) ahead[j - 1] = c;
    }
    ahead[D - 1] = 0;
    for (int r = 0; r < rounds; ++r) {
        int newer = 0;
#pragma unroll
        for (int j = 0; j < D - 1; ++j) newer += ahead[j];
        wait_vmcnt(newer);
        asm volatile("s_waitcnt lgkmcnt(0)" ::: "memory");
        __builtin_amdgcn_s_barrier();
        ahead[D - 1] = stage(q[D], sm + ((r + D) % NBUF) * image);
        compute(q[0], sm + (r % NBUF) * image);
#pragma unroll
        for (int j = 0; j < D; ++j) q[j] = q[j + 1];
        q[D] = finish(nxt);
        nxt = fetch(r + D + 2);
#pragma unroll
        for (int j = 0; j < D - 1; ++j) ahead[j] = ahead[j + 1];
    }
    asm volatile("s_waitcnt vmcnt(0) lgkmcnt(0)" ::: "memory");
    __builtin_amdgcn_s_barrier();
    constexpr int ROW = (P * CINL * 9 + P + 3) & ~3;
    float *row = sm + wave * ROW;
    if (kq < 3) {
#pragma unroll
        for (int tl = 0; tl < NTILE; ++tl) {
            const int col = tl * 16 + nq;
            if (col < NCOL) {
#pragma unroll
                for (int r = 0; r < 4; ++r) {
                    const int co = 4 * kq + r;
                    if (col == NCOL - 1) {
                        row[P * CINL * 9 + co] = acc[tl][r];
                    } else {
                        const int tap = col / CINL, ci = col - tap * CINL;
                        row[(co * CINL + ci) * 9 + tap] = acc[tl][r];
                    }
                }
            }
        }
    }
    __syncthreads();
    const int len = wgrad_row_len(layer);
    float *dst = a.slab2 + wgrad_slab_base(layer, a.rows) + (int64_t)wg * len;
    for (int e = tid; e < len; e += kWaves * 64) {
        float t = 0.f;
#pragma unroll
        for (int w2 = 0; w2 < kWaves; ++w2) t += sm[w2 * ROW + e];
        dst[e] = t;
    }
}

template <int NBUF, bool BF>
__global__ __launch_bounds__(kWaves * 64, 4) void txp_wgrad_kernel(const WgradArgs a, const int32_t *__restrict__ order,
                                                                   const int32_t *__restrict__ order_peds,
                                                                   const int32_t *__restrict__ num_peds) {
    extern __shared__ __attribute__((aligned(16))) float sm[];
    int layer = 0;
    while (layer < a.lay.L && (int)blockIdx.x >= a.wg_begin[layer + 1]) ++layer;
    const int wg = (int)blockIdx.x - a.wg_begin[layer];
    const int nwg = a.wg_begin[layer + 1] - a.wg_begin[layer];
    if (layer == 0)
        wgrad_layer<Cfg::T, NBUF, BF>(a, order, order_peds, num_peds, layer, sm, wg, nwg);
    else
        wgrad_layer<Cfg::P, NBUF, BF>(a, order, order_peds, num_peds, layer, sm, wg, nwg);
}

}

bool wgrad_geom(const ModelLayout &L, int N, int V, WgradGeom *g) {
    const bool bf16 = (L.flags & STG_OPT_BF16_STORE) != 0;
    const size_t image = (size_t)wgrad_image_floats(V, bf16) * sizeof(float);
    const size_t row = (size_t)((Cfg::P * Cfg::P * 9 + Cfg::P + 3) & ~3) * sizeof(float) * kWaves;
    int nbuf = diag_env("STG_WGRAD_NBUF", 4);
    if (nbuf != 3) nbuf = 4;
    int per_cu = 2;
    while (nbuf > 3 && image * nbuf * per_cu > (size_t)kLdsBytes) --nbuf;
    if (image * nbuf * per_cu > (size_t)kLdsBytes) per_cu = 1;
    size_t lds = image * nbuf;
    if (lds < row) lds = row;
    if (lds > (size_t)kLdsBytes) return false;
    g->waves = kWaves;
    g->nbuf = nbuf;
    g->lds = lds;
    g->bf16mma = wgrad_bf16_fits(L, V) && !diag_env("STG_WGRAD_F32", 0);
    if (g->bf16mma) {
        wgrad_bf16_geom(g, L, V);
        per_cu = (int)((size_t)kLdsBytes / g->lds);
    }
    int total = kNumCU * per_cu;
    if (const int v = diag_env("STG_WGRAD_GRID", 0)) total = v > 0 ? v : total;
    const int nl = L.L + 1;
    if (total < nl) total = nl;
    const int need = N * wgrad_chunks(V);
    const int w0 = g->bf16mma ? 15 : 6, w1 = g->bf16mma ? 18 : 7, wsum = w0 + w1 * (nl - 1);
    int begin = 0, maxw = 0;
    for (int l = 0; l < nl; ++l) {
        int cnt = (int)((int64_t)total * (l == 0 ? w0 : w1) / wsum);
        if (cnt < 1) cnt = 1;
        if (cnt > need) cnt = need;
        g->wg_begin[l] = begin;
        begin += cnt;
        if (cnt > maxw) maxw = cnt;
    }
    g->wg_begin[nl] = begin;
    g->grid = begin;
    g->rows = maxw;
    return true;
}

int launch_txp_wgrad(const WgradArgs &w, const WgradGeom &g, hipStream_t st) {
    if (g.bf16mma) return launch_txp_wgrad_bf16(w, g, st);
    const Launch lc{"txp_wgrad", dim3(g.grid), dim3(kWaves * 64), g.lds, st};
    const bool bf16 = (w.lay.flags & STG_OPT_BF16_STORE) != 0;
    if (g.nbuf == 3)
        return launch(lc, bf16 ? txp_wgrad_kernel<3, true> : txp_wgrad_kernel<3, false>, w, w.order, w.order_peds, w.num_peds);
    return launch(lc, bf16 ? txp_wgrad_kernel<4, true> : txp_wgrad_kernel<4, false>, w, w.order, w.order_peds, w.num_peds);
}

}
```

social_stgcnn_amd/csrc/txp_wgrad.hpp:

```cpp
#pragma once
#include "model_common.hpp"

namespace stg {

constexpr int kWgradChunkV = 32;
__host__ __device__ inline int wgrad_chunks(int V) { return (V + kWgradChunkV - 1) / kWgradChunkV; }
__host__ __device__ inline int wgrad_image_v(int V) { return V < kWgradChunkV ? V : kWgradChunkV; }
__host__ __device__ inline int wgrad_plane_floats(int V0, bool bf16) {
    const int V = wgrad_image_v(V0);
    if (!bf16) return plane_slot(V);
    return (((Cfg::C + 2) * save_sw(V, true) * Cfg::P) / 2 + 3) & ~3;
}
__host__ __device__ inline int wgrad_image_floats(int V0, bool bf16 = false) {
    const int V = wgrad_image_v(V0);
    if (!bf16) return plane_slot(V) + dz_slot(V);
    return wgrad_plane_floats(V0, true) + (((Cfg::C * save_vw(V, true) * Cfg::P) / 2 + 3 + 4) & ~3);
}
__host__ __device__ inline int wgrad_row_len(int layer) {
    return Cfg::P * (layer == 0 ? Cfg::T : Cfg::P) * 9 + Cfg::P;
}
__host__ __device__ inline int64_t wgrad_slab_base(int layer, int rows) {
    return layer == 0 ? 0 : (int64_t)rows * (wgrad_row_len(0) + (int64_t)(layer - 1) * wgrad_row_len(1));
}

struct WgradGeom {
    int waves, nbuf, grid, rows;
    bool bf16mma;
    int wg_begin[kMaxTxp + 2];
    size_t lds;
};
bool wgrad_geom(const ModelLayout &L, int N, int V, WgradGeom *g);

struct WgradArgs {
    ModelLayout lay;
    const int32_t *num_peds;
    const int32_t *order;
    const int32_t *order_peds;
    const int32_t *key_start;
    int serpentine;
    int N, V;
    const float *ws;
    const float *dzg;
    int64_t ws_stride;
    float *slab2;
    int rows;
    int wg_begin[kMaxTxp + 2];
    int debug_skip;
};
int launch_txp_wgrad(const WgradArgs &w, const WgradGeom &g, hipStream_t st);
bool wgrad_bf16_fits(const ModelLayout &L, int V);
void wgrad_bf16_geom(WgradGeom *g, const ModelLayout &L, int V);
int launch_txp_wgrad_bf16(const WgradArgs &w, const WgradGeom &g, hipStream_t st);
int launch_txp_wgrad_bf16_canon32(const WgradArgs &w, const WgradGeom &g, hipStream_t st);

}
```

social_stgcnn_amd/csrc/txp_wgrad_bf16.hip:

```cpp
#include "txp_conv_bf16.hpp"
#include "txp_wgrad.hpp"
#include "scene_team.hpp"
#include <type_traits>

namespace stg {

namespace {

constexpr int C = Cfg::C, P = Cfg::P;
constexpr int kRec = 96;
constexpr int kPiece = 32;
constexpr int SWI = kWgradChunkV + 2, VWI = kWgradChunkV;
constexpr int kARecs = (C + 2) * SWI;
constexpr int kZRecs = C * VWI;
constexpr int kZeroRec = kARecs + kZRecs;
constexpr int kOnesRec = kZeroRec + 1;
constexpr int kImageBytes = (kOnesRec + 1) * kRec;
constexpr int kATasks = C * SWI * 3, kZTasks = C * VWI * 3;

typedef unsigned u32x2 __attribute__((ext_vector_type(2)));
typedef unsigned u32x4 __attribute__((ext_vector_type(4)));

struct Item {
    int vc, w0;
    int swf, vwf;
    bool valid;
    const float *pl, *dz;
};

struct Op {
    u32x2 h[2], m[2], l[2];
};
__device__ __forceinline__ u32x4 cat(const u32x2 (&p)[2]) { return u32x4{p[0].x, p[0].y, p[1].x, p[1].y}; }

template <int OFF>
__device__ __forceinline__ void read_op(unsigned a0, unsigned a1, Op &o) {
    asm volatile("ds_read_b64_tr_b16 %0, %6 offset:%8\n\tds_read_b64_tr_b16 %1, %7 offset:%8\n\t"
                 "ds_read_b64_tr_b16 %2, %6 offset:%9\n\tds_read_b64_tr_b16 %3, %7 offset:%9\n\t"
                 "ds_read_b64_tr_b16 %4, %6 offset:%10\n\tds_read_b64_tr_b16 %5, %7 offset:%10\n\t"
                 "s_waitcnt lgkmcnt(0)"
                 : "=&v"(o.h[0]), "=&v"(o.h[1]), "=&v"(o.m[0]), "=&v"(o.m[1]), "=&v"(o.l[0]), "=&v"(o.l[1])
                 : "v"(a0), "v"(a1), "n"(OFF), "n"(OFF + kPiece), "n"(OFF + 2 * kPiece)
                 : "memory");
}
template <int OFF, int D>
__device__ __forceinline__ void read_op1(unsigned a0, Op &o) {
    asm volatile("ds_read_b64_tr_b16 %0, %6 offset:%7\n\tds_read_b64_tr_b16 %1, %6 offset:%8\n\t"
                 "ds_read_b64_tr_b16 %2, %6 offset:%9\n\tds_read_b64_tr_b16 %3, %6 offset:%10\n\t"
                 "ds_read_b64_tr_b16 %4, %6 offset:%11\n\tds_read_b64_tr_b16 %5, %6 offset:%12\n\t"
                 "s_waitcnt lgkmcnt(0)"
                 : "=&v"(o.h[0]), "=&v"(o.h[1]), "=&v"(o.m[0]), "=&v"(o.m[1]), "=&v"(o.l[0]), "=&v"(o.l[1])
                 : "v"(a0), "n"(OFF), "n"(OFF + D), "n"(OFF + kPiece), "n"(OFF + D + kPiece), "n"(OFF + 2 * kPiece),
                   "n"(OFF + D + 2 * kPiece)
                 : "memory");
}
template <int OFF, int D>
__device__ __forceinline__ void read_op1_h(unsigned a0, Op &o) {
    asm volatile("ds_read_b64_tr_b16 %0, %2 offset:%3\n\tds_read_b64_tr_b16 %1, %2 offset:%4\n\ts_waitcnt lgkmcnt(0)"
                 : "=&v"(o.h[0]), "=&v"(o.h[1])
                 : "v"(a0), "n"(OFF), "n"(OFF + D)
                 : "memory");
}
template <int OFF>
__device__ __forceinline__ void read_op_h(unsigned a0, unsigned a1, Op &o) {
    asm volatile("ds_read_b64_tr_b16 %0, %2 offset:%4\n\tds_read_b64_tr_b16 %1, %3 offset:%4\n\ts_waitcnt lgkmcnt(0)"
                 : "=&v"(o.h[0]), "=&v"(o.h[1])
                 : "v"(a0), "v"(a1), "n"(OFF)
                 : "memory");
}
__device__ __forceinline__ f32x4 mma(const u32x4 &a, const u32x4 &b, const f32x4 &c) {
    return __builtin_amdgcn_mfma_f32_16x16x32_bf16(__builtin_bit_cast(cv::bf16x8, a), __builtin_bit_cast(cv::bf16x8, b), c, 0,
                                                   0, 0);
}
__device__ __forceinline__ void mma6(const u32x4 &zh, const u32x4 &zm, const u32x4 &zl, const Op &a, f32x4 &acc) {
    const u32x4 ah = cat(a.h), am = cat(a.m), al = cat(a.l);
    asm volatile("s_nop 3\n\tv_mfma_f32_16x16x32_bf16 %0, %1, %4, %0\n\t"
                 "v_mfma_f32_16x16x32_bf16 %0, %2, %4, %0\n\t"
                 "v_mfma_f32_16x16x32_bf16 %0, %1, %5, %0\n\t"
                 "v_mfma_f32_16x16x32_bf16 %0, %2, %5, %0\n\t"
                 "v_mfma_f32_16x16x32_bf16 %0, %3, %4, %0\n\t"
                 "v_mfma_f32_16x16x32_bf16 %0, %1, %6, %0\n\t"
                 "s_nop 7"
                 : "+v"(acc)
                 : "v"(zh), "v"(zm), "v"(zl), "v"(ah), "v"(am), "v"(al));
}
__device__ __forceinline__ void mma1(const u32x4 &zh, const u32x4 &ah, f32x4 &acc) {
    asm volatile("s_nop 3\n\tv_mfma_f32_16x16x32_bf16 %0, %1, %2, %0\n\ts_nop 7" : "+v"(acc) : "v"(zh), "v"(ah));
}
template <bool BF> struct StageType { typedef f32x4 type; };
template <> struct StageType<true> { typedef u32x2 type; };

template <int CINL, bool BF, bool CH, int NW, int NIMG, Shape SH>
__device__ __forceinline__ void layer(const WgradArgs &a, const int32_t *__restrict__ order,
                                      const int32_t *__restrict__ order_peds, const int32_t *__restrict__ num_peds,
                                      const int32_t *__restrict__ key_start, int layer, unsigned char *sm, int wg, int nwg) {
    constexpr bool K32 = SH == Shape::Canon32;
    static_assert(SH != Shape::Canon && !(K32 && CH), "Generic, or Canon32 with one chunk per scene");
    static_assert(kCanonV == kWgradChunkV && save_sw(kCanonV, BF) == SWI && save_vw(kCanonV, BF) == VWI,
                  "Canon32: the saved rows have the image's strides");
    constexpr int NTH = NW * 64;
    constexpr int HS = NW / 5;
    constexpr int QPT = CINL / 4;
    constexpr int NQ = 9 * QPT;
    constexpr int NT = (9 * CINL + 1 + 15) / 16;
    constexpr int T0 = HS == 1 ? NT : (NT + 1) / 2;
    constexpr int TA = (kATasks + NTH - 1) / NTH, TZ = (kZTasks + NTH - 1) / NTH;
    const ModelLayout &L = a.lay;
    const int V = K32 ? kCanonV : a.V, tid = threadIdx.x, lane = tid & 63;
    const int wave = __builtin_amdgcn_readfirstlane(tid >> 6);
    const int ks = wave / HS, hf = wave - ks * HS;
    const int kg = lane >> 4, rq = (lane & 15) >> 2, cp = lane & 3;
    const unsigned lds0 = (unsigned)(uintptr_t)(__attribute__((address_space(3))) unsigned char *)sm;

    const int nch = CH ? wgrad_chunks(V) : 1;
    const bool compact = CH && order && key_start && nch > 1;
    int items = a.N * nch;
    if (compact) {
        items = a.N;
        for (int c = 1; c < nch; ++c) {
            const int more = key_start[V - kWgradChunkV * c];
            items += more < 0 ? 0 : (more > a.N ? a.N : more);
        }
    }
    const int64_t plane_off = K32 ? ws_plane_off(kCanonLayout, kCanonV, 0) + (int64_t)layer * plane_slot(kCanonV)
                                  : ws_plane_off(L, V, layer);
    const int64_t dzs_floats = dz_slot(V);
    const bool bf = BF;
    constexpr int64_t kDzScene = (int64_t)(kCanonLayout.L + 1) * dz_slot(kCanonV);
    auto plane32 = [&](int n) { return a.ws + n * kCanonWs32 + plane_off; };
    auto dz32 = [&](int n) { return a.dzg + n * kDzScene + layer * (int64_t)dz_slot(kCanonV); };
    auto fetch = [&](int r) -> Item {
        Item it{0, 0, 0, 0, false, nullptr, nullptr};
        const int at = walk_item(r, wg, nwg, items, order != nullptr && a.serpentine);
        if (at < 0) return it;
        int si = at, chunk = 0;
        if (compact) {
            int cnt = a.N;
            while (si >= cnt) {
                si -= cnt;
                ++chunk;
                cnt = key_start[V - kWgradChunkV * chunk];
                cnt = cnt < 0 ? 0 : (cnt > a.N ? a.N : cnt);
                if (chunk >= nch - 1) break;
            }
            if (si >= a.N) si = a.N - 1;
        } else if (nch > 1) {
            si = at / nch;
            chunk = at - si * nch;
        }
        const int n = order ? scene_index(order[si], a.N) : si;
        int vfull = order ? order_peds[si] : (num_peds ? num_peds[si] : V);
        vfull = vfull < 0 ? 0 : (vfull > V ? V : vfull);
        const int nc = CH ? wgrad_chunks(vfull) : 1;
        if (vfull == 0 || chunk >= nc) return it;
        const int wc = nc > 1 ? (vfull + nc - 1) / nc : vfull;
        it.pl = a.ws + n * a.ws_stride + plane_off;
        it.dz = a.dzg + ((int64_t)n * (L.L + 1) + layer) * dzs_floats;
        it.w0 = chunk * wc;
        it.vc = (vfull - it.w0) < wc ? (vfull - it.w0) : wc;
        it.swf = save_sw(vfull, bf);
        it.vwf = save_vw(vfull, bf);
        it.valid = true;
        return it;
    };

    constexpr int TF = BF ? 2 : 4;
    using StageV = typename StageType<BF>::type;
    struct Stage { StageV a[TA], z[TZ]; };
    unsigned dsta[TA], dstz[TZ];
    int rowa[TA], cola[TA], rowz[TZ], colz[TZ];
#pragma unroll
    for (int u = 0; u < TA; ++u) {
        const int e = tid + u * NTH, rec = e / 3, q = e - rec * 3, row = rec / SWI, col = rec - row * SWI;
        dsta[u] = (unsigned)((SWI + rec) * kRec + 8 * q);
        rowa[u] = row * 3 * TF;
        cola[u] = e < kATasks ? ((col * 3 + q) * TF) | (col << 16) : -1;
    }
#pragma unroll
    for (int u = 0; u < TZ; ++u) {
        const int e = tid + u * NTH, rec = e / 3, q = e - rec * 3, row = rec / VWI, col = rec - row * VWI;
        dstz[u] = (unsigned)((kARecs + rec) * kRec + 8 * q);
        rowz[u] = row * 3 * TF;
        colz[u] = e < kZTasks ? ((col * 3 + q) * TF) | (col << 16) : -1;
    }
    auto load32 = [&](bool ok, const float *pl, const float *dz, Stage &s) {
        const bool live = ok && !STG_SKIP(a, 64);
        const float *pa = live ? pl : a.ws, *pz = live ? dz : a.ws;
#pragma unroll
        for (int u = 0; u < TA; ++u) {
            const int e = tid + u * NTH;
            s.a[u] = *reinterpret_cast<const StageV *>(pa + (e < kATasks ? e * TF : 0));
        }
#pragma unroll
        for (int u = 0; u < TZ; ++u) {
            const int e = tid + u * NTH;
            s.z[u] = *reinterpret_cast<const StageV *>(pz + (e < kZTasks ? e * TF : 0));
        }
    };
    auto load = [&](const Item &it, Stage &s) {
        const bool live = it.valid && !STG_SKIP(a, 64);
        const int lima = live ? it.vc + 2 : 0, limz = live ? it.vc : 0;
        const float *pa = (live ? it.pl : a.ws) + (live ? it.w0 * 3 * TF : 0);
        const float *pz = (live ? it.dz : a.ws) + (live ? it.w0 * 3 * TF : 0);
#pragma unroll
        for (int u = 0; u < TA; ++u) {
            const bool used = cola[u] >= 0 && (cola[u] >> 16) < lima;
            const int off = used ? rowa[u] * it.swf + (cola[u] & 0xffff) : 0;
            s.a[u] = *reinterpret_cast<const StageV *>(pa + off);
        }
#pragma unroll
        for (int u = 0; u < TZ; ++u) {
            const bool used = colz[u] >= 0 && (colz[u] >> 16) < limz;
            const int off = used ? rowz[u] * it.vwf + (colz[u] & 0xffff) : 0;
            s.z[u] = *reinterpret_cast<const StageV *>(pz + off);
        }
    };
    auto put = [&](unsigned char *dst, const StageV &v) {
        if constexpr (BF) {
            *reinterpret_cast<uint2 *>(dst) = make_uint2(v.x, v.y);
        } else {
            uint2 ph, pm, pl;
            cv::split_pack4(v, ph, pm, pl);
            *reinterpret_cast<uint2 *>(dst) = ph;
            *reinterpret_cast<uint2 *>(dst + kPiece) = pm;
            *reinterpret_cast<uint2 *>(dst + 2 * kPiece) = pl;
        }
    };
    auto convert = [&](const Item &it, const Stage &s, unsigned char *img) {
        if (!it.valid || STG_SKIP(a, 64)) return;
#pragma unroll
        for (int u = 0; u < TA; ++u)
            if (cola[u] >= 0 && (cola[u] >> 16) < it.vc + 2) put(img + dsta[u], s.a[u]);
#pragma unroll
        for (int u = 0; u < TZ; ++u)
            if (colz[u] >= 0 && (colz[u] >> 16) < it.vc) put(img + dstz[u], s.z[u]);
    };
    auto convert32 = [&](bool ok, const Stage &s, unsigned char *img) {
        if (!ok || STG_SKIP(a, 64)) return;
#pragma unroll
        for (int u = 0; u < TA; ++u)
            if (tid + u * NTH < kATasks) put(img + dsta[u], s.a[u]);
#pragma unroll
        for (int u = 0; u < TZ; ++u)
            if (tid + u * NTH < kZTasks) put(img + dstz[u], s.z[u]);
    };

    int toff[T0];
    bool ones_last = false;
#pragma unroll
    for (int k = 0; k < T0; ++k) {
        const int t = hf * T0 + k, Q = 4 * t + cp;
        const int tap = Q / QPT, cq = Q - tap * QPT;
        toff[k] = ((tap / 3) * SWI + (tap % 3)) * kRec + 8 * cq;
        if (Q >= NQ) {
            toff[k] = 0;
            if (t == NT - 1) ones_last = true;
        }
    }
    f32x4 acc[T0];
#pragma unroll
    for (int k = 0; k < T0; ++k) acc[k] = f32x4{0.f, 0.f, 0.f, 0.f};

    int vc_cur = -1;
    unsigned za[2] = {0u, 0u}, aa[2] = {0u, 0u};
    auto kslots = [&](int vc) {
        vc_cur = vc;
        const int npos = C * vc;
        const float inv = __builtin_amdgcn_rcpf((float)vc);
#pragma unroll
        for (int rd = 0; rd < 2; ++rd) {
            const int p = 32 * ks + 16 * rd + 4 * kg + rq;
            const bool ok = p < npos;
            const int hh = (int)(((float)p + 0.5f) * inv), ww = p - hh * vc;
            za[rd] = (unsigned)((ok ? kARecs + hh * VWI + ww : kZeroRec) * kRec + 8 * cp);
            aa[rd] = (unsigned)((ok ? hh * SWI + ww : 0) * kRec);
        }
    };
    auto addr = [&](int k, int rd, unsigned base) -> unsigned {
        const unsigned rel = base + aa[rd] + (unsigned)toff[k];
        return (hf * T0 + k == NT - 1 && ones_last) ? base + (unsigned)(kOnesRec * kRec + 8 * cp) : rel;
    };
    auto compute = [&](const Item &it, unsigned base) {
        if (!it.valid || STG_SKIP(a, 128)) return;
        if (32 * ks >= C * it.vc) return;
        if (it.vc != vc_cur) kslots(it.vc);
        __builtin_amdgcn_s_setprio(2);
        Op z, x0;
        u32x4 zh, zm = u32x4{0u, 0u, 0u, 0u}, zl = zm;
        if constexpr (BF) {
            read_op_h<0>(base + za[0], base + za[1], z);
            zh = cat(z.h);
        } else {
            read_op<0>(base + za[0], base + za[1], z);
            zh = cat(z.h); zm = cat(z.m); zl = cat(z.l);
        }
#pragma unroll
        for (int k = 0; k < T0; ++k) {
            if (hf * T0 + k < NT) {
                if constexpr (BF) {
                    read_op_h<0>(addr(k, 0, base), addr(k, 1, base), x0);
                    mma1(zh, cat(x0.h), acc[k]);
                } else {
                    read_op<0>(addr(k, 0, base), addr(k, 1, base), x0);
                    mma6(zh, zm, zl, x0, acc[k]);
                }
            }
        }
        (void)zm; (void)zl;
        __builtin_amdgcn_s_setprio(0);
    };
    constexpr int kHalf = 16 * kRec;
    static_assert(kImageBytes + kHalf + 3 * kPiece < 65536, "the operand offsets are 16-bit immediates");
    unsigned za32 = 0u, tb32 = 0u, ta32[T0];
#pragma unroll
    for (int k = 0; k < T0; ++k) ta32[k] = 0u;
    if constexpr (K32) {
        const int ww = 4 * kg + rq;
        za32 = lds0 + (unsigned)((kARecs + ks * VWI + ww) * kRec + 8 * cp);
#pragma unroll
        for (int k = 0; k < T0; ++k) {
            ta32[k] = lds0 + (unsigned)((ks * SWI + ww) * kRec) + (unsigned)toff[k];
            if (hf * T0 + k == NT - 1) {
                tb32 = ta32[k] + (unsigned)kHalf;
                if (ones_last) ta32[k] = tb32 = lds0 + (unsigned)(kOnesRec * kRec + 8 * cp);
            }
        }
    }
    auto compute32 = [&](bool ok, unsigned ib) {
        if (!ok || STG_SKIP(a, 128)) return;
        __builtin_amdgcn_s_setprio(2);
        Op z, x0;
        u32x4 zh, zm = u32x4{0u, 0u, 0u, 0u}, zl = zm;
        if constexpr (BF) {
            read_op1_h<0, kHalf>(za32 + ib, z);
            zh = cat(z.h);
        } else {
            read_op1<0, kHalf>(za32 + ib, z);
            zh = cat(z.h); zm = cat(z.m); zl = cat(z.l);
        }
#pragma unroll
        for (int k = 0; k < T0; ++k) {
            if (hf * T0 + k < NT) {
                const bool last = hf * T0 + k == NT - 1;
                if constexpr (BF) {
                    if (last) read_op_h<0>(ta32[k] + ib, tb32 + ib, x0);
                    else read_op1_h<0, kHalf>(ta32[k] + ib, x0);
                    mma1(zh, cat(x0.h), acc[k]);
                } else {
                    if (last) read_op<0>(ta32[k] + ib, tb32 + ib, x0);
                    else read_op1<0, kHalf>(ta32[k] + ib, x0);
                    mma6(zh, zm, zl, x0, acc[k]);
                }
            }
        }
        (void)zm; (void)zl;
        __builtin_amdgcn_s_setprio(0);
    };

    for (int i = 0; i < NIMG; ++i) {
        unsigned char *img = sm + i * kImageBytes;
        constexpr int U = kRec / 8;
        for (int e = tid; e < (kOnesRec + 1) * U; e += NTH)
            *reinterpret_cast<uint2 *>(img + e * 8) =
                (e >= kOnesRec * U && e < kOnesRec * U + kPiece / 8) ? make_uint2(0x3f803f80u, 0x3f803f80u) : make_uint2(0u, 0u);
    }
    team_barrier();

    const int rounds = (items + nwg - 1) / nwg;
    Stage s;
#pragma unroll
    for (int u = 0; u < TA; ++u) s.a[u] = StageV{};
#pragma unroll
    for (int u = 0; u < TZ; ++u) s.z[u] = StageV{};
    if constexpr (K32) {
        int n = wg;
        const float *pl = plane32(n), *dz = dz32(n);
        bool cur = n < a.N;
        load32(cur, pl, dz, s);
        for (int r = 0; r < rounds; ++r) {
            const int ib = NIMG == 1 ? 0 : (r & 1) * kImageBytes;
            if (NIMG == 1 && r > 0) team_barrier();
            convert32(cur, s, sm + ib);
            n += nwg;
            pl += nwg * kCanonWs32;
            dz += nwg * kDzScene;
            const bool nxt = n < a.N;
            load32(nxt, pl, dz, s);
            team_barrier();
            compute32(cur, (unsigned)ib);
            cur = nxt;
        }
    } else {
        Item cur = fetch(0), nxt = fetch(1);
        load(cur, s);
        for (int r = 0; r < rounds; ++r) {
            const int ib = NIMG == 1 ? 0 : (r & 1) * kImageBytes;
            if (NIMG == 1 && r > 0) team_barrier();
            convert(cur, s, sm + ib);
            load(nxt, s);
            team_barrier();
            compute(cur, lds0 + (unsigned)ib);
            cur = nxt;
            nxt = fetch(r + 2);
        }
    }
    asm volatile("s_waitcnt vmcnt(0) lgkmcnt(0)" ::: "memory");
    __builtin_amdgcn_s_barrier();
    constexpr int ROW = (P * CINL * 9 + P + 3) & ~3;
    float *rowsm = reinterpret_cast<float *>(sm);
    float *row = rowsm + wave * ROW;
    const int nq = lane & 15, kq = lane >> 4;
    if (kq < 3) {
#pragma unroll
        for (int k = 0; k < T0; ++k) {
            const int t = hf * T0 + k;
            if (t < NT) {
                const int jj = 16 * t + nq;
                const int tap = jj / CINL, ci = jj - tap * CINL;
#pragma unroll
                for (int r = 0; r < 4; ++r) {
                    const int co = 4 * kq + r;
                    if (jj < 9 * CINL) row[(co * CINL + ci) * 9 + tap] = acc[k][r];
                    else if (jj == 9 * CINL) row[P * CINL * 9 + co] = acc[k][r];
                }
            }
        }
    }
    __syncthreads();
    const int len = wgrad_row_len(layer);
    float *dst = a.slab2 + wgrad_slab_base(layer, a.rows) + (int64_t)wg * len;
    for (int e = tid; e < len; e += NTH) {
        int jj = 9 * CINL;
        if (e < P * CINL * 9) {
            const int tap = e % 9, ci = (e / 9) % CINL;
            jj = tap * CINL + ci;
        }
        const int h = (jj >> 4) >= T0 ? 1 : 0;
        float t = 0.f;
#pragma unroll
        for (int sidx = 0; sidx < 5; ++sidx) t += rowsm[(sidx * HS + h) * ROW + e];
        dst[e] = t;
    }
}

template <bool BF, bool CH, int NW, int NIMG, Shape SH = Shape::Generic>
__global__ __launch_bounds__(NW * 64, NW == 5 ? 5 : 6) void txp_wgrad_bf16_kernel(const WgradArgs a, const int32_t *__restrict__ order,
                                                                   const int32_t *__restrict__ order_peds,
                                                                   const int32_t *__restrict__ num_peds,
                                                                   const int32_t *__restrict__ key_start) {
    extern __shared__ __attribute__((aligned(16))) unsigned char smb[];
    int l = 0;
    const int hidden = SH == Shape::Canon32 ? kCanonLayout.L : a.lay.L;
    while (l < hidden && (int)blockIdx.x >= a.wg_begin[l + 1]) ++l;
    const int wg = (int)blockIdx.x - a.wg_begin[l];
    const int nwg = a.wg_begin[l + 1] - a.wg_begin[l];
    if (l == 0)
        layer<Cfg::T, BF, CH, NW, NIMG, SH>(a, order, order_peds, num_peds, key_start, l, smb, wg, nwg);
    else
        layer<Cfg::P, BF, CH, NW, NIMG, SH>(a, order, order_peds, num_peds, key_start, l, smb, wg, nwg);
}


}

#ifndef STG_K2_CANON32_TU
bool wgrad_bf16_fits(const ModelLayout &L, int V) {
    (void)V;
    return !(L.flags & STG_OPT_F32_MFMA);
}

void wgrad_bf16_geom(WgradGeom *g, const ModelLayout &L, int V) {
    (void)V;
    const bool bf = (L.flags & STG_OPT_BF16_STORE) != 0;
    g->waves = bf ? 5 : 10;
    g->nbuf = bf ? 1 : 2;
    const size_t row = (size_t)((Cfg::P * Cfg::P * 9 + Cfg::P + 3) & ~3) * sizeof(float) * g->waves;
    size_t lds = (size_t)g->nbuf * kImageBytes;
    if (lds < row) lds = row;
    g->lds = lds;
}
#endif

#if defined(STG_K2_CANON32_TU) || defined(STG_K2_ALL_SHAPES)
int launch_txp_wgrad_bf16_canon32(const WgradArgs &w, const WgradGeom &g, hipStream_t st) {
    const Launch lc{"txp_wgrad_bf16 (Canon32)", dim3(g.grid), dim3(g.waves * 64), g.lds, st};
    const bool bf = (w.lay.flags & STG_OPT_BF16_STORE) != 0;
    const bool five = g.waves == 5 && g.nbuf == 1, ten = g.waves == 10 && g.nbuf == 2;
    constexpr Shape S = Shape::Canon32;
#ifdef STG_K2_ALL_SHAPES
    if (five || ten) {
        const auto k = five ? (bf ? txp_wgrad_bf16_kernel<true, false, 5, 1, S> : txp_wgrad_bf16_kernel<false, false, 5, 1, S>)
                            : (bf ? txp_wgrad_bf16_kernel<true, false, 10, 2, S> : txp_wgrad_bf16_kernel<false, false, 10, 2, S>);
        return launch(lc, k, w, w.order, w.order_peds, w.num_peds, w.key_start);
    }
#else
    if (bf ? five : ten)
        return launch(lc, bf ? txp_wgrad_bf16_kernel<true, false, 5, 1, S> : txp_wgrad_bf16_kernel<false, false, 10, 2, S>, w,
                      w.order, w.order_peds, w.num_peds, w.key_start);
#endif
    return fail(STG_EINVAL, "txp_wgrad_bf16 (Canon32): no kernel for %d waves / %d images", g.waves, g.nbuf);
}
#endif

#ifndef STG_K2_CANON32_TU
static bool wgrad_canon32(const WgradArgs &w) {
    return is_canonical(w.lay) && w.V == kCanonV && !w.num_peds && !w.order && !w.key_start && w.ws_stride == kCanonWs32 &&
           !(w.lay.flags & STG_OPT_GENERIC_WGRAD);
}

template <bool B, int NW, int NI>
static auto wgrad_bf16_kernel(bool ch) { return ch ? txp_wgrad_bf16_kernel<B, true, NW, NI> : txp_wgrad_bf16_kernel<B, false, NW, NI>; }

int launch_txp_wgrad_bf16(const WgradArgs &w, const WgradGeom &g, hipStream_t st) {
    if (wgrad_canon32(w)) return launch_txp_wgrad_bf16_canon32(w, g, st);
    const Launch lc{"txp_wgrad_bf16", dim3(g.grid), dim3(g.waves * 64), g.lds, st};
    const bool bf = (w.lay.flags & STG_OPT_BF16_STORE) != 0, ch = w.V > kWgradChunkV;
    const bool five = g.waves == 5 && g.nbuf == 1, ten = g.waves == 10 && g.nbuf == 2;
#ifdef STG_K2_ALL_SHAPES
    if (five || ten) {
        const auto k = five ? (bf ? wgrad_bf16_kernel<true, 5, 1>(ch) : wgrad_bf16_kernel<false, 5, 1>(ch))
                            : (bf ? wgrad_bf16_kernel<true, 10, 2>(ch) : wgrad_bf16_kernel<false, 10, 2>(ch));
        return launch(lc, k, w, w.order, w.order_peds, w.num_peds, w.key_start);
    }
#else
    if (bf ? five : ten)
        return launch(lc, bf ? wgrad_bf16_kernel<true, 5, 1>(ch) : wgrad_bf16_kernel<false, 10, 2>(ch), w, w.order, w.order_peds,
                      w.num_peds, w.key_start);
#endif
    return fail(STG_EINVAL, "txp_wgrad_bf16: no kernel for %d waves / %d images", g.waves, g.nbuf);
}
#endif

}
```

social_stgcnn_amd/csrc/txp_x6.hip:

```cpp
#include "txp_scene_common.hpp"
#include "nll_elem.hpp"
#include "txp_conv_bf16.hpp"

namespace stg {

namespace {

constexpr int C = Cfg::C, P = Cfg::P, T = Cfg::T;

constexpr int64_t kCanonAggStride32[2] = {(int64_t)(Cfg::CIN0 + 1) * Cfg::T * kCanonV, kCanonWs32};
constexpr int64_t kCanonAggAx32[2] = {0, kCanonLayout.ws_hdr_floats + (int64_t)kCanonLayout.blk[0].ws_ax * kCanonV};
constexpr int64_t kCanonAggCs32[2] = {(int64_t)Cfg::CIN0 * Cfg::T * kCanonV,
                                      kCanonLayout.ws_hdr_floats + (int64_t)kCanonLayout.blk[0].ws_cs * kCanonV};

template <Shape S, typename Args>
__device__ __forceinline__ void fold_shape(Args &a) {
    if constexpr (S != Shape::Generic) {
        ModelLayout k = kCanonLayout;
        k.eps = a.lay.eps;
        k.momentum = a.lay.momentum;
        k.bn_mode = a.lay.bn_mode;
        k.flags = a.lay.flags;
        k.wg_waves = a.lay.wg_waves;
        a.lay = k;
    }
    if constexpr (S == Shape::Canon32) {
        a.V = a.Vl = kCanonV;
        a.num_peds = nullptr;
        a.tier.order = nullptr;
        a.tier.key_start = nullptr;
        a.ws_stride = kCanonWs32;
    }
}
__device__ __forceinline__ unsigned canon32_code(int t, int nq) {
    return (unsigned)(cv::tile_row(kCanonV, t) << 8 | (cv::tile_col0(kCanonV, t) + nq));
}
template <Shape S>
__device__ __forceinline__ int lay_txp_b(const ModelLayout &L, int l) {
    if constexpr (S == Shape::Generic) return L.txp_b[l];
    else return kCanonLayout.txp_b[l];
}
template <Shape S>
__device__ __forceinline__ int lay_ws_z(const ModelLayout &L, int l) {
    if constexpr (S == Shape::Generic) return L.ws_z[l];
    else return kCanonLayout.ws_z[l];
}

#ifdef STG_DIAG
#define STG_X6_STAMP(a, n, k)                                                                                          \
    do {                                                                                                              \
        if ((a).stamps && (threadIdx.x & 63) == 0) (a).stamps[(int64_t)(n) * 16 + (k)] = __builtin_amdgcn_s_memrealtime(); \
    } while (0)
#else
#define STG_X6_STAMP(a, n, k) do { } while (0)
#endif

constexpr int kF6Tiles = 10, kF6Slots = 7;

__host__ __device__ inline int fwd6_region_floats(int v) { return (cv::image_bytes(v, kF6Slots) / 4 + 3) & ~3; }

template <bool BF, typename CK, Shape SH = Shape::Generic>
__device__ __forceinline__ void txp_fwd_scene_x6(const TxpFwdArgs &a, const float *__restrict__ params,
                                                 const float *blk_params, const float *blk_buffers, int n, int vi,
                                                 float *region, ptab_t *ptab, const CK &ck) {
    const ModelLayout &L = a.lay;
    const int V = a.V, lane = threadIdx.x & 63, nq = lane & 15, kq = lane >> 4;
    float *yn = a.y + (int64_t)n * (C * P) * V;
    if (vi < V)
        for (int e = lane + 64 * ck.ci(); e < C * P * (V - vi); e += 64 * ck.nch()) {
            const int r = e / (V - vi), w = vi + (e - r * (V - vi));
            yn[(int64_t)r * V + w] = 0.f;
        }
    if (vi == 0) return;
    const int npos = C * ck.wc(), ntiles = (npos + 15) >> 4;
    const float *Pm = params;
    float *wsn = a.ws ? a.ws + n * a.ws_stride : nullptr;
    float *statn = a.stats ? a.stats + (int64_t)n * L.stat_floats : nullptr;
    unsigned char *img = reinterpret_cast<unsigned char *>(region);
    const cv::LaneGeom lg = cv::lane_geom(vi, kF6Slots);
    constexpr bool bf16 = BF;
    const int SWs = save_sw(vi, bf16), VWs = save_vw(vi, bf16);

    {
        float sv[C * T / 2];
        const float *agn = a.agg + n * a.agg_stride;
        stgcn_block_fwd_cols<true, SH != Shape::Canon32>(a, blk_params, blk_buffers, L.blk[0], n, vi, wsn, statn,
                                                         agn + a.agg_ax, agn + a.agg_cs, nullptr, 0, region,
                                                         cv::image_bytes(vi, kF6Slots) >> 4, ptab, sv, ck);
        float *d2 = wsn ? wsn + ws_plane_off(L, V, 0) : nullptr;
        const int pl = lane & 31, pw = ck.w0() + pl, q = lane >> 5;
        if (pl < ck.wc()) {
#pragma unroll
            for (int row = 0; row < C; ++row) {
                const f32x4 v4 = {sv[row], sv[C + row], sv[2 * C + row], sv[3 * C + row]};
                cv::put4(img, (unsigned)(cv::pos_off(vi, 1 + row, pw) + 8 * q), lg.PL, v4);
                if (d2) {
                    store_vec4(d2, (row * SWs + pw + 1) * 3 + q, v4, bf16);
                    if (q == 0) store_vec4(d2, (row * SWs + pw + 1) * 3 + 2, f32x4{0.f, 0.f, 0.f, 0.f}, bf16);
                }
            }
        }
        if (wsn && lane < 2 * C * 3 && ck.lead()) {
            const int b = lane / 3, q = lane - b * 3, pos = (b >> 1) * SWs + ((b & 1) ? vi + 1 : 0);
            for (int l = 0; l <= L.L; ++l)
                store_vec4(wsn + ws_plane_off(L, V, l), pos * 3 + q, f32x4{0.f, 0.f, 0.f, 0.f}, bf16);
        }
    }
    ck.sync();

    if (STG_SKIP(a, 16)) return;
    const unsigned lds_base = (unsigned)(uintptr_t)img;
    [[maybe_unused]] cv::LaneBases lb;
    if constexpr (SH == Shape::Canon32) {
        static_assert(!CK::kTeam && 16 * kF6Tiles == C * kCanonV, "Canon32: one wave, ten full tiles");
        lb = cv::lane_bases(lds_base, lg, vi);
    }
    f32x4 av[kF6Tiles];
#pragma unroll
    for (int t = 0; t < kF6Tiles; ++t) av[t] = f32x4{0.f, 0.f, 0.f, 0.f};
    for (int l = 0; l <= L.L; ++l) {
        const bool is_out = l == L.L;
        cv::u32x4 w[cv::kWpVecs];
        cv::load_wp(a.wpf + (int64_t)l * cv::kWpDwords, w);
        const float *bias = Pm + (is_out ? L.out_b : lay_txp_b<SH>(L, l));
        f32x4 binit;
#pragma unroll
        for (int r = 0; r < 4; ++r) binit[r] = kq < 3 ? bias[4 * kq + r] : 0.f;
        const float alpha = is_out ? 0.f : Pm[L.prelus + l];
        float *zs = (wsn && !is_out) ? wsn + L.ws_hdr_floats + (int64_t)lay_ws_z<SH>(L, l) * V : nullptr;
        float *ps = (wsn && !is_out) ? wsn + ws_plane_off(L, V, l + 1) : nullptr;
        asm volatile("" ::"v"(w[0]), "v"(w[cv::kWpVecs - 1]), "v"(binit), "v"(alpha) : "memory");
        vm_drain();
        __builtin_amdgcn_s_setprio(1);
        auto finish = [&](int t, int h, int wc, bool ok, const f32x4 &z) __attribute__((always_inline)) {
            if (ok && kq < 3) {
                if (is_out) {
#pragma unroll
                    for (int r = 0; r < 4; ++r) yn[(int64_t)((4 * kq + r) * C + h) * V + wc] = z[r];
                } else {
                    f32x4 v4;
#pragma unroll
                    for (int r = 0; r < 4; ++r) v4[r] = (z[r] > 0.f ? z[r] : alpha * z[r]) + av[t][r];
                    av[t] = v4;
                    if (zs) {
                        store_vec4(zs, (h * VWs + wc) * 3 + kq, z, bf16);
                        store_vec4(ps, (h * SWs + wc + 1) * 3 + kq, v4, bf16);
                    }
                }
            }
        };
        if constexpr (SH == Shape::Canon32) {
            cv::for_tiles<kF6Tiles>([&](auto tc) __attribute__((always_inline)) {
                constexpr int t = decltype(tc)::value;
                cv::BHalf b;
                f32x4 z = binit;
                cv::load_b_half_imm<0, kCanonV, t>(lb, b);
                cv::mma_half<0>(w, b, z);
                cv::load_b_half_imm<1, kCanonV, t>(lb, b);
                cv::mma_half<1>(w, b, z);
                finish(t, cv::tile_row(kCanonV, t), cv::tile_col0(kCanonV, t) + nq, true, z);
            });
        } else {
            unsigned code = cv::tile_code(0, ptab, npos);
#pragma unroll
            for (int t = 0; t < kF6Tiles; ++t) {
                if (t < ntiles) {
                    const cv::Tile tl = cv::tile_from<1>(t, code, npos, lg, vi);
                    if (t + 1 < kF6Tiles) code = cv::tile_code(t + 1, ptab, npos);
                    cv::BHalf b;
                    f32x4 z = binit;
                    cv::load_b_half<0>(lds_base, tl, b);
                    cv::mma_half<0>(w, b, z);
                    cv::load_b_half<1>(lds_base, tl, b);
                    cv::mma_half<1>(w, b, z);
                    finish(t, tl.h, tl.w, tl.ok, z);
                }
            }
        }
        __builtin_amdgcn_s_setprio(0);
        if (is_out) break;
        ck.sync();
        unsigned codes[kF6Tiles];
#pragma unroll
        for (int t = 0; t < kF6Tiles; ++t) codes[t] = SH == Shape::Canon32 ? canon32_code(t, nq) : cv::tile_code(t, ptab, npos);
#pragma unroll
        for (int t = 0; t < kF6Tiles; ++t) {
            const int p = 16 * t + nq;
            if (p < npos && kq < 3) {
                const unsigned hw = codes[t];
                cv::put4(img, (unsigned)(cv::pos_off(vi, 1 + (int)(hw >> 8), (int)(hw & 0xffu)) + 8 * kq), lg.PL, av[t]);
            }
        }
        ck.sync();
    }
}

template <int WPB, bool BF, Shape S>
__global__ __launch_bounds__(WPB * 64, WPB == 8 ? 1 : 2) __attribute__((amdgpu_waves_per_eu(2, 2))) void txp_fwd_x6_kernel(
    const TxpFwdArgs a0, const float *__restrict__ params, const float *__restrict__ buffers) {
    extern __shared__ __attribute__((aligned(16))) float sm[];
    TxpFwdArgs a = a0;
    fold_shape<S>(a);
    if constexpr (S == Shape::Canon32) {
        const int w = a.ws != nullptr;
        a.agg_stride = kCanonAggStride32[w];
        a.agg_ax = kCanonAggAx32[w];
        a.agg_cs = kCanonAggCs32[w];
    }
    const int Vl = a.Vl, wave = threadIdx.x >> 6;
    const int per_wave = fwd6_region_floats(Vl) + ptab_floats(Vl);
    float *region = sm + wave * per_wave;
    ptab_t *ptab = reinterpret_cast<ptab_t *>(region + fwd6_region_floats(Vl));
    float *blk_p = sm + WPB * per_wave, *blk_b = blk_p + ((a.lay.n_blk_params + 3) & ~3);
    stage_block_params(a.lay, params, buffers, blk_p, blk_b, WPB * 64);
    const int gw = __builtin_amdgcn_readfirstlane(blockIdx.x * WPB + wave), nw = gridDim.x * WPB;
    int begin, end;
    tier_range(a.tier, a.N, a.V, begin, end);
    const int M = end - begin;
    for (int r = 0; r * nw < M; ++r) {
        const int it = walk_item(r, gw, nw, M, a.tier.order != nullptr && a.tier.serpentine);
        if (it < 0) continue;
        const int n = __builtin_amdgcn_readfirstlane(a.tier.order ? scene_index(a.tier.order[begin + it], a.N) : it);
        int vi = a.num_peds ? a.num_peds[n] : a.V;
        vi = __builtin_amdgcn_readfirstlane(vi < 0 ? 0 : (vi > a.V ? a.V : vi));
        STG_X6_STAMP(a, n, 0);
        txp_fwd_scene_x6<BF, SoloScene, S>(a, params, blk_p, blk_b, n, vi, region, ptab, SoloScene{vi});
        __builtin_amdgcn_wave_barrier();
        STG_X6_STAMP(a, n, 8);
    }
}

constexpr int kX6Tiles = 10;
constexpr int kX6Slots = 7;
__host__ __device__ inline int bwd6_region_floats(int v) {
    const int img = cv::image_bytes(v, kX6Slots) / 4, tail = (2 * C * (T + 2) + C * T) * v;
    return ((img > tail ? img : tail) + 3) & ~3;
}

template <bool BF, typename CK, Shape SH = Shape::Generic>
__device__ __forceinline__ void txp_bwd_scene_x6(const TxpBwdArgs &a, const float *blk_params, int n, int vi, float *region,
                                                 ptab_t *ptab, const CK &ck) {
    const ModelLayout &L = a.lay;
    const int V = a.V, lane = threadIdx.x & 63, nq = lane & 15, kq = lane >> 4;
    float *slope_row = a.rows + (int64_t)n * (L.n_blk_params + L.n_txp) + L.n_blk_params;
    if (vi == 0) {
        for (int e = lane; e < L.n_blk_params + L.n_txp; e += 64) slope_row[e - L.n_blk_params] = 0.f;
        if (a.nll_target && lane == 0) a.nll_losses[n] = 0.f;
        return;
    }
    const int npos = C * ck.wc(), ntiles = (npos + 15) >> 4;
    const float *Pm = a.params;
    const float *wsn = a.ws + n * a.ws_stride;
    const float *dyn = a.dy + (int64_t)n * (C * P) * V;
    float *prow = ck.row(slope_row - L.n_blk_params);
    if constexpr (CK::kTeam) {
        for (int e = lane; e < kTeamRow; e += 64) prow[e] = 0.f;
    }
    unsigned char *img = reinterpret_cast<unsigned char *>(region);
    const cv::LaneGeom lg = cv::lane_geom(vi, kX6Slots);
    constexpr bool bf16 = BF;
    const int VWs = save_vw(vi, bf16);
    auto tile_slots = [&](int t, int &rec, int &quad) {
        if constexpr (SH == Shape::Canon32) {
            const int h = cv::tile_row(kCanonV, t), w = cv::tile_col0(kCanonV, t) + nq;
            quad = (h * VWs + w) * 3 + kq;
            rec = cv::pos_off(vi, 1 + h, w) + 8 * kq;
        } else {
            const int p = 16 * t + nq;
            const unsigned hw = ptab[p < npos ? p : 0];
            const int h = (int)(hw >> 8), w = (int)(hw & 0xffu);
            quad = (h * VWs + w) * 3 + kq;
            rec = (p < npos && kq < 3) ? cv::pos_off(vi, 1 + h, w) + 8 * kq : -1;
        }
    };
    auto has_quad = [&](int rec) { return SH == Shape::Canon32 ? kq < 3 : rec >= 0; };
    {
        uint4 *z4 = reinterpret_cast<uint4 *>(img);
        for (int e = lane + 64 * ck.ci(); e < cv::image_bytes(vi, kX6Slots) >> 4; e += 64 * ck.nch()) z4[e] = make_uint4(0u, 0u, 0u, 0u);
    }
    [[maybe_unused]] cv::LaneBases lb;
    if constexpr (SH == Shape::Canon32) {
        static_assert(!CK::kTeam && 16 * kX6Tiles == C * kCanonV, "Canon32: one wave, ten full tiles");
        lb = cv::lane_bases((unsigned)(uintptr_t)img, lg, vi);
    } else {
        build_ptab(ptab, ck.w0(), ck.wc());
    }
    ck.sync();
    f32x4 dcur[kX6Tiles];
#pragma unroll
    for (int t = 0; t < kX6Tiles; ++t) dcur[t] = f32x4{0.f, 0.f, 0.f, 0.f};

    for (int l = L.L; l >= 0; --l) {
        float *dzo = a.dzg + ((int64_t)n * (L.L + 1) + l) * dz_slot(V);
        if (STG_SKIP(a, 512) || (l == L.L && STG_SKIP(a, 2048)) || (l != L.L && STG_SKIP(a, 4096))) {
        } else if (l == L.L) {
            const int wcw = ck.wc();
            const int vp = wcw <= 1 ? 1 : (wcw <= 2 ? 2 : (wcw <= 4 ? 4 : (wcw <= 8 ? 8 : (wcw <= 16 ? 16 : 32))));
            const int sh = __builtin_ctz(vp), rpi = 64 >> sh;
            const int sub = lane >> sh, wl = lane & (vp - 1), w = ck.w0() + wl;
            const bool okw = wl < wcw;
            float *S = reinterpret_cast<float *>(img + lg.PL);
            auto put1 = [&](int rc, float g) { S[rc * vi + w] = g; };
            if (a.nll_target) {
                const float *tn = a.nll_target + (int64_t)n * P * V * 2;
                const float inv_cnt = 1.0f / (float)(P * vi);
                const float gs = inv_cnt * (a.nll_weights ? a.nll_weights[n] : 1.f);
                float lacc = 0.f;
#pragma unroll 1
                for (int p0 = 0; p0 < P; p0 += rpi) {
                    const int p = p0 + sub;
                    if (okw && p < P) {
                        const float *q = dyn + (int64_t)p * V + w;
                        const float2 tg = *reinterpret_cast<const float2 *>(tn + ((int64_t)p * V + w) * 2);
                        float g[5];
#ifdef STG_DIAG
                        if (STG_SKIP(a, 1 << 21))
                            lacc += nll_elem_t<true>(q[0], q[(int64_t)P * V], q[(int64_t)2 * P * V], q[(int64_t)3 * P * V],
                                                     q[(int64_t)4 * P * V], tg.x, tg.y, true, g);
                        else
#endif
                        lacc += nll_elem(q[0], q[(int64_t)P * V], q[(int64_t)2 * P * V], q[(int64_t)3 * P * V],
                                         q[(int64_t)4 * P * V], tg.x, tg.y, true, g);
#pragma unroll
                        for (int f = 0; f < C; ++f) put1(f * P + p, g[f] * gs);
                    }
                }
                float ls[1] = {lacc};
                ck.template reduce<1>(ls);
                if (ck.writer()) {
                    if constexpr (CK::kTeam) prow[kTeamRowLoss] = ls[0];
                    else a.nll_losses[n] = ls[0] * inv_cnt;
                }
            } else {
                constexpr int U = 4;
#pragma unroll 1
                for (int r0 = 0; r0 < C * P; r0 += rpi * U) {
                    float dv[U];
#pragma unroll
                    for (int u = 0; u < U; ++u) {
                        const int row = r0 + u * rpi + sub;
                        dv[u] = (okw && row < C * P) ? dyn[(int64_t)row * V + w] : 0.f;
                    }
#pragma unroll
                    for (int u = 0; u < U; ++u) {
                        const int row = r0 + u * rpi + sub;
                        if (okw && row < C * P) put1(row, dv[u]);
                    }
                }
            }
            __builtin_amdgcn_wave_barrier();
            vm_drain();
            f32x4 (&qd)[kX6Tiles] = dcur;
#pragma unroll
            for (int t = 0; t < kX6Tiles; ++t) {
                const int p = 16 * t + nq;
                const unsigned hw = SH == Shape::Canon32 ? canon32_code(t, nq) : ptab[p < npos ? p : 0];
                const float *sq = S + ((4 * (kq < 3 ? kq : 0)) * C + (int)(hw >> 8)) * vi + (int)(hw & 0xffu);
                qd[t] = f32x4{sq[0], sq[C * vi], sq[2 * C * vi], sq[3 * C * vi]};
            }
            ck.sync();
            {
                uint4 *z4 = reinterpret_cast<uint4 *>(img + lg.PL);
                for (int e = lane + 64 * ck.ci(); e < (2 * lg.PL + 128) >> 4; e += 64 * ck.nch()) z4[e] = make_uint4(0u, 0u, 0u, 0u);
            }
            ck.sync();
            int rec[kX6Tiles], qv[kX6Tiles];
#pragma unroll
            for (int t = 0; t < kX6Tiles; ++t) tile_slots(t, rec[t], qv[t]);
#pragma unroll
            for (int t = 0; t < kX6Tiles; ++t) {
                if (has_quad(rec[t])) {
                    cv::put4(img, (unsigned)rec[t], lg.PL, qd[t]);
                    store_vec4(dzo, qv[t], qd[t], bf16);
                }
            }
        } else {
            const float *zl = wsn + L.ws_hdr_floats + (int64_t)lay_ws_z<SH>(L, l) * V;
            const float alpha = Pm[L.prelus + l];
            float slope_acc = 0.f;
            f32x4 zv[kX6Tiles];
            int rec[kX6Tiles], qv[kX6Tiles];
#pragma unroll
            for (int t = 0; t < kX6Tiles; ++t) tile_slots(t, rec[t], qv[t]);
#pragma unroll
            for (int t = 0; t < kX6Tiles; ++t)
                zv[t] = has_quad(rec[t]) ? load_vec4_raw(zl, qv[t], bf16) : f32x4{1.f, 1.f, 1.f, 1.f};
            asm volatile("" ::"v"(zv[0]), "v"(zv[1]), "v"(zv[2]), "v"(zv[3]), "v"(zv[4]), "v"(zv[5]), "v"(zv[6]), "v"(zv[7]),
                         "v"(zv[8]), "v"(zv[9]), "v"(alpha)
                         : "memory");
            vm_drain();
#pragma unroll
            for (int t = 0; t < kX6Tiles; ++t) {
                if (has_quad(rec[t])) {
                    f32x4 dzv;
                    const f32x4 zq = finish_vec4(zv[t], bf16);
#pragma unroll
                    for (int r = 0; r < 4; ++r) {
                        const float z = zq[r], d = dcur[t][r];
                        float dz = d;
                        if (!(z > 0.f)) {
                            dz = alpha * d;
                            slope_acc = fmaf(d, z, slope_acc);
                        }
                        dzv[r] = dz;
                    }
                    cv::put4(img, (unsigned)rec[t], lg.PL, dzv);
                    store_vec4(dzo, qv[t], dzv, bf16);
                }
            }
            float ss[1] = {slope_acc};
            ck.template reduce<1>(ss);
            if (ck.writer()) prow[L.n_blk_params + l] = ss[0];
        }
        ck.sync();
        if (!STG_SKIP(a, 1024)) {
            cv::u32x4 w[cv::kWpVecs];
            cv::load_wp(a.wp + (int64_t)l * cv::kWpDwords, w);
            asm volatile("" ::"v"(w[0]), "v"(w[cv::kWpVecs - 1]) : "memory");
            vm_drain();
            const unsigned lds_base = (unsigned)(uintptr_t)img;
            const bool keep = l != L.L && l != 0;
            const f32x4 zero = {0.f, 0.f, 0.f, 0.f};
            if constexpr (SH == Shape::Canon32) {
                cv::for_tiles<kX6Tiles>([&](auto tc) __attribute__((always_inline)) {
                    constexpr int t = decltype(tc)::value;
                    cv::BHalf b;
                    f32x4 acc = keep ? dcur[t] : zero;
                    cv::load_b_half_imm<0, kCanonV, t>(lb, b);
                    cv::mma_half<0>(w, b, acc);
                    cv::load_b_half_imm<1, kCanonV, t>(lb, b);
                    cv::mma_half<1>(w, b, acc);
                    dcur[t] = acc;
                });
            } else {
                unsigned code = cv::tile_code(0, ptab, npos);
#pragma unroll
                for (int t = 0; t < kX6Tiles; ++t) {
                    if (t < ntiles) {
                        const cv::Tile tl = cv::tile_from<1>(t, code, npos, lg, vi);
                        if (t + 1 < kX6Tiles) code = cv::tile_code(t + 1, ptab, npos);
                        cv::BHalf b;
                        f32x4 acc = keep ? dcur[t] : zero;
                        cv::load_b_half<0>(lds_base, tl, b);
                        cv::mma_half<0>(w, b, acc);
                        cv::load_b_half<1>(lds_base, tl, b);
                        cv::mma_half<1>(w, b, acc);
                        dcur[t] = acc;
                    }
                }
            }
        }
        ck.sync();
    }
    float *D = region;
#pragma unroll
    for (int t = 0; t < kX6Tiles; ++t) {
        const int p = 16 * t + nq;
        if (p < npos && kq < T / 4) {
            const unsigned hw = SH == Shape::Canon32 ? canon32_code(t, nq) : ptab[p];
            const int h = (int)(hw >> 8), ww = (int)(hw & 0xffu);
#pragma unroll
            for (int r = 0; r < 4; ++r) D[((4 * kq + r) * C + h) * vi + ww] = dcur[t][r];
        }
    }
    __builtin_amdgcn_wave_barrier();
    if constexpr (!CK::kTeam) {
        for (int e = L.L + lane; e < L.n_txp; e += 64) slope_row[e] = 0.f;
    }
    if (!STG_SKIP(a, 4))
        stgcn_block_bwd_cols<true>(a, blk_params, L.blk[0], n, vi, D, slope_row - L.n_blk_params, a.ws + n * a.ws_stride, ck);
    if constexpr (CK::kTeam) {
        ck.sync();
        if (ck.lead()) {
            float *row = slope_row - L.n_blk_params;
            const int nrow = L.n_blk_params + L.n_txp;
            for (int e0 = 0; e0 < kTeamRow; e0 += 64) {
                const int e = e0 + lane < kTeamRow ? e0 + lane : kTeamRow - 2;
                float t = ck.row_of(0)[e];
                for (int c = 1; c < ck.nch(); ++c) t += ck.row_of(c)[e];
                if (e < nrow) row[e] = t;
                if (e == kTeamRowLoss && a.nll_target) a.nll_losses[n] = t * (1.0f / (float)(P * vi));
            }
        }
    }
}

template <int WPB, bool BF, Shape S>
__global__ __launch_bounds__(WPB * 64, WPB == 8 ? 1 : 2) __attribute__((amdgpu_waves_per_eu(2, 2))) void txp_bwd_x6_kernel(
    const TxpBwdArgs a0) {
    extern __shared__ __attribute__((aligned(16))) float sm[];
    TxpBwdArgs a = a0;
    fold_shape<S>(a);
    const int Vl = a.Vl, wave = threadIdx.x >> 6;
    const int per_wave = bwd6_region_floats(Vl) + bwd_ptab_floats(Vl);
    float *region = sm + wave * per_wave;
    ptab_t *ptab = reinterpret_cast<ptab_t *>(region + bwd6_region_floats(Vl));
    float *blk_p = sm + WPB * per_wave;
    stage_block_params(a.lay, a.params, nullptr, blk_p, nullptr, WPB * 64);
    const int gw = __builtin_amdgcn_readfirstlane(blockIdx.x * WPB + wave), nw = gridDim.x * WPB;
    int begin, end;
    tier_range(a.tier, a.N, a.V, begin, end);
    const int M = end - begin;
    for (int r = 0; r * nw < M; ++r) {
        const int it = walk_item(r, gw, nw, M, a.tier.order != nullptr && a.tier.serpentine);
        if (it < 0) continue;
        const int n = __builtin_amdgcn_readfirstlane(a.tier.order ? scene_index(a.tier.order[begin + it], a.N) : it);
        int vi = a.num_peds ? a.num_peds[n] : a.V;
        vi = __builtin_amdgcn_readfirstlane(vi < 0 ? 0 : (vi > a.V ? a.V : vi));
        STG_X6_STAMP(a, n, 0);
        txp_bwd_scene_x6<BF, SoloScene, S>(a, blk_p, n, vi, region, ptab, SoloScene{vi});
        __builtin_amdgcn_wave_barrier();
        STG_X6_STAMP(a, n, 8);
    }
}

__host__ __device__ inline int step6_per_wave_floats(int v) {
    const int f = fwd6_region_floats(v) + ptab_floats(v), b = bwd6_region_floats(v) + bwd_ptab_floats(v);
    return f > b ? f : b;
}

template <int WPB, bool BF>
__global__ __launch_bounds__(WPB * 64, 2) __attribute__((amdgpu_waves_per_eu(2, 2))) void txp_step_x6_kernel(
    const TxpFwdArgs f0, const TxpBwdArgs b0) {
    constexpr Shape S = Shape::Canon32;
    extern __shared__ __attribute__((aligned(16))) float sm[];
    TxpFwdArgs f = f0;
    fold_shape<S>(f);
    f.agg_stride = kCanonAggStride32[1];
    f.agg_ax = kCanonAggAx32[1];
    f.agg_cs = kCanonAggCs32[1];
    TxpBwdArgs b = b0;
    fold_shape<S>(b);
    const int wave = threadIdx.x >> 6;
    const int per_wave = step6_per_wave_floats(kCanonV);
    float *region = sm + wave * per_wave;
    ptab_t *ptab = reinterpret_cast<ptab_t *>(region + bwd6_region_floats(kCanonV));
    float *blk_p = sm + WPB * per_wave, *blk_b = blk_p + ((kCanonLayout.n_blk_params + 3) & ~3);
    stage_block_params(f.lay, f.params, f.buffers, blk_p, blk_b, WPB * 64);
    const int n = __builtin_amdgcn_readfirstlane(blockIdx.x * WPB + wave);
    if (n >= f.N) return;
    STG_X6_STAMP(f, n, 0);
    txp_fwd_scene_x6<BF, SoloScene, S>(f, f.params, blk_p, blk_b, n, kCanonV, region, ptab, SoloScene{kCanonV});
    __builtin_amdgcn_fence(__ATOMIC_RELEASE, "wavefront");
    __builtin_amdgcn_wave_barrier();
    __builtin_amdgcn_fence(__ATOMIC_ACQUIRE, "wavefront");
    STG_X6_STAMP(f, n, 8);
    STG_X6_STAMP(b, n, 0);
    txp_bwd_scene_x6<BF, SoloScene, S>(b, blk_p, n, kCanonV, region, ptab, SoloScene{kCanonV});
    __builtin_amdgcn_wave_barrier();
    STG_X6_STAMP(b, n, 8);
}

struct TeamCount {
    int n4, n2, n1;
    int u4, u2, units;
    bool sorted;
};
__device__ __forceinline__ TeamCount team_count(const SceneTier &t, const TeamGeom &g, const int32_t *num_peds, int N, int V) {
    TeamCount c;
    c.sorted = t.order && t.key_start;
    if (c.sorted) {
        const int a4 = g.v2 < V ? t.key_start[V - g.v2] : 0, a2 = g.v1 < V ? t.key_start[V - g.v1] : 0;
        c.n4 = a4;
        c.n2 = a2 - a4;
        c.u2 = (c.n2 + 1) >> 1;
    } else {
        const bool pairs = !num_peds && V > g.v1 && V <= g.v2;
        c.n4 = (V > g.v1 && !pairs) ? N : 0;
        c.n2 = pairs ? N : 0;
        c.u2 = (c.n2 + 1) >> 1;
    }
    c.n1 = N - c.n4 - c.n2;
    c.u4 = c.n4;
    c.units = c.u4 + c.u2 + ((c.n1 + 3) >> 2);
    return c;
}
struct TeamUnit {
    int n, vi;
    int nch, ci, slot;
    int w0, wc;
};
__device__ __forceinline__ TeamUnit team_unit(const SceneTier &t, const TeamCount &c, const int32_t *__restrict__ num_peds,
                                              int N, int V, int u) {
    const int wave = __builtin_amdgcn_readfirstlane(threadIdx.x >> 6);
    TeamUnit q;
    int idx;
    if (u < c.u4) {
        q.nch = 4; q.slot = 0; q.ci = wave; idx = u;
    } else if (u < c.u4 + c.u2) {
        const int i0 = c.n4 + 2 * (u - c.u4);
        if (i0 + 1 < c.n4 + c.n2) { q.nch = 2; q.slot = wave >> 1; q.ci = wave & 1; idx = i0 + q.slot; }
        else { q.nch = 4; q.slot = 0; q.ci = wave; idx = i0; }
    } else {
        q.nch = 1; q.slot = wave; q.ci = 0; idx = c.n4 + c.n2 + 4 * (u - c.u4 - c.u2) + wave;
    }
    q.n = idx < N ? (c.sorted ? scene_index(t.order[idx], N) : idx) : -1;
    q.n = __builtin_amdgcn_readfirstlane(q.n);
    int vi = q.n >= 0 ? (num_peds ? num_peds[q.n] : V) : 0;
    vi = __builtin_amdgcn_readfirstlane(vi < 0 ? 0 : (vi > V ? V : vi));
    q.vi = vi;
    const int wc = (vi + q.nch - 1) / q.nch;
    q.w0 = q.ci * wc;
    q.wc = vi - q.w0 < wc ? (vi - q.w0 > 0 ? vi - q.w0 : 0) : wc;
    return q;
}
__device__ __forceinline__ int team_workers(int units, int grid) {
    const int rounds = (units + grid - 1) / grid;
    return rounds > 0 ? (units + rounds - 1) / rounds : 1;
}
__host__ __device__ inline int team_ptab_floats() { return ptab_floats(32); }

template <bool BF>
__global__ __launch_bounds__(256, 2) __attribute__((amdgpu_waves_per_eu(2, 2))) void txp_fwd_team_kernel(
    const TxpFwdArgs a, const float *__restrict__ params, const float *__restrict__ buffers) {
    extern __shared__ __attribute__((aligned(16))) float sm[];
    const int wave = __builtin_amdgcn_readfirstlane(threadIdx.x >> 6);
    const int R = a.team.region_floats;
    ptab_t *ptab = reinterpret_cast<ptab_t *>(sm + R + wave * team_ptab_floats());
    float *xr = sm + R + 4 * team_ptab_floats();
    float *blk_p = xr + 2 * kXrFwd, *blk_b = blk_p + ((a.lay.n_blk_params + 3) & ~3);
    stage_block_params(a.lay, params, buffers, blk_p, blk_b, 256);
    const TeamCount tc = team_count(a.tier, a.team, a.num_peds, a.N, a.V);
    const int G = team_workers(tc.units, gridDim.x);
    int prev = 1;
    for (int r = 0; r * G < tc.units; ++r) {
        const int u = walk_item(r, blockIdx.x, G, tc.units, a.tier.serpentine != 0);
        if (u < 0 || (int)blockIdx.x >= G) continue;
        const TeamUnit q = team_unit(a.tier, tc, a.num_peds, a.N, a.V, u);
        if (q.nch > 1 || prev > 1) team_barrier();
        prev = q.nch;
        if (q.n >= 0) {
            const TeamScene ck{q.vi, q.w0, q.wc, q.nch, q.ci, xr + (q.slot & 1) * kXrFwd, nullptr, q.nch > 1 && !STG_SKIP(a, 1 << 20)};
            float *region = sm + q.slot * ((R >> 2) * q.nch);
            txp_fwd_scene_x6<BF>(a, params, blk_p, blk_b, q.n, q.vi, region, ptab, ck);
        }
        __builtin_amdgcn_wave_barrier();
    }
}

template <bool BF>
__global__ __launch_bounds__(256, 2) __attribute__((amdgpu_waves_per_eu(2, 2))) void txp_bwd_team_kernel(const TxpBwdArgs a) {
    extern __shared__ __attribute__((aligned(16))) float sm[];
    const int wave = __builtin_amdgcn_readfirstlane(threadIdx.x >> 6);
    const int R = a.team.region_floats;
    ptab_t *ptab = reinterpret_cast<ptab_t *>(sm + R + wave * team_ptab_floats());
    float *xr = sm + R + 4 * team_ptab_floats();
    float *blk_p = xr + kXrBwdWg;
    stage_block_params(a.lay, a.params, nullptr, blk_p, nullptr, 256);
    const TeamCount tc = team_count(a.tier, a.team, a.num_peds, a.N, a.V);
    const int G = team_workers(tc.units, gridDim.x);
    int prev = 1;
    for (int r = 0; r * G < tc.units; ++r) {
        const int u = walk_item(r, blockIdx.x, G, tc.units, a.tier.serpentine != 0);
        if (u < 0 || (int)blockIdx.x >= G) continue;
        const TeamUnit q = team_unit(a.tier, tc, a.num_peds, a.N, a.V, u);
        if (q.nch > 1 || prev > 1) team_barrier();
        prev = q.nch;
        if (q.n >= 0) {
            const TeamScene ck{q.vi, q.w0, q.wc, q.nch, q.ci, xr + (q.slot & 1) * kXrRows,
                               xr + 2 * kXrRows + q.slot * q.nch * kTeamRow, q.nch > 1 && !STG_SKIP(a, 1 << 20)};
            float *region = sm + q.slot * ((R >> 2) * q.nch);
            txp_bwd_scene_x6<BF>(a, blk_p, q.n, q.vi, region, ptab, ck);
        }
        __builtin_amdgcn_wave_barrier();
    }
}

}

bool txp_fwd_x6_fits(const ModelLayout &L, int V) {
    return L.n_txp > 0 && V <= kTeamMaxV && !(L.flags & STG_OPT_F32_MFMA) && L.n_blocks == 1 &&
           L.blk[0].cin == Cfg::CIN0 && !diag_env("STG_FWD_F32", 0);
}

constexpr int kTeamFineBatch = 1536, kTeamFinestBatch = 384;
static int team_waves(int v, int v1, int v2) { return v <= v1 ? 1 : (v <= v2 ? 2 : 4); }
static bool team_geom(int N, int V, bool uniform, TeamGeom *g) {
    g->on = 0;
    if (V > kTeamMaxV) return false;
    int v1 = 32, v2 = 64;
    if (N < kTeamFinestBatch) { v1 = 8; v2 = 16; }
    else if (N < kTeamFineBatch) { v1 = 16; v2 = 32; }
    if (uniform)
        while (v1 < 32 && (int64_t)N * team_waves(V, v1, v2) > 2048) { v1 *= 2; v2 *= 2; }
    if (const int e = diag_env("STG_TEAM_V1", 0)) v1 = e;
    if (const int e = diag_env("STG_TEAM_V2", 0)) v2 = e;
    if (v1 > 32) v1 = 32;
    if (v2 > 64) v2 = 64;
    if (v2 < v1) v2 = v1;
    auto region = [&](int v) { return fwd6_region_floats(v); };
    int r = 4 * region(v1 < V ? v1 : V);
    if (2 * region(v2 < V ? v2 : V) > r) r = 2 * region(v2 < V ? v2 : V);
    if (region(V) > r) r = region(V);
    g->on = 1; g->v1 = v1; g->v2 = v2; g->region_floats = (r + 15) & ~15;
    return true;
}
static bool team_wanted(int N, int V, bool uniform, TeamGeom *g) {
    if (!team_geom(N, V, uniform, g)) return false;
    return V > 16 * kF6Tiles / C || g->v1 < V || diag_env("STG_TEAM", 0) != 0;
}
static int team_grid(size_t lds_bytes, int N) {
    int per_cu = (int)(kLdsBytes / lds_bytes);
    if (per_cu > 2) per_cu = 2;
    if (per_cu < 1) per_cu = 1;
    const int g = kNumCU * per_cu;
    return g < N ? g : N;
}

template <typename Args>
static Shape canon_shape(const Args &a, bool *ok) {
    *ok = true;
    if (!is_canonical(a.lay)) return Shape::Generic;
    if (a.num_peds || a.V != kCanonV) return Shape::Canon;
    *ok = a.Vl == kCanonV && !a.tier.order && !a.tier.key_start && a.ws_stride == kCanonWs32;
    return Shape::Canon32;
}
static bool canon32_agg_matches(const TxpFwdArgs &a) {
    const int w = a.ws != nullptr;
    return a.agg_stride == kCanonAggStride32[w] && a.agg_ax == kCanonAggAx32[w] && a.agg_cs == kCanonAggCs32[w];
}

template <int W>
static auto fwd_x6_kernel(bool bf, Shape sh) {
    if (bf) return sh == Shape::Canon32 ? txp_fwd_x6_kernel<W, true, Shape::Canon32> : txp_fwd_x6_kernel<W, true, Shape::Generic>;
    if (sh == Shape::Canon32) return txp_fwd_x6_kernel<W, false, Shape::Canon32>;
    return sh == Shape::Canon ? txp_fwd_x6_kernel<W, false, Shape::Canon> : txp_fwd_x6_kernel<W, false, Shape::Generic>;
}
template <int W>
static auto bwd_x6_kernel(bool bf, Shape sh) {
    if (bf) {
        if (sh == Shape::Canon32) return txp_bwd_x6_kernel<W, true, Shape::Canon32>;
        return sh == Shape::Canon ? txp_bwd_x6_kernel<W, true, Shape::Canon> : txp_bwd_x6_kernel<W, true, Shape::Generic>;
    }
    if (sh == Shape::Canon32) return txp_bwd_x6_kernel<W, false, Shape::Canon32>;
    return sh == Shape::Canon ? txp_bwd_x6_kernel<W, false, Shape::Canon> : txp_bwd_x6_kernel<W, false, Shape::Generic>;
}

int launch_txp_fwd_x6(const TxpFwdArgs &a0, hipStream_t st) {
    TxpFwdArgs a = a0;
    STG_REQUIRE(a.wpf, STG_EINVAL, "txp_fwd_x6: the prepared operands are missing");
    const bool bf = (a.lay.flags & STG_OPT_BF16_STORE) != 0;
    if (team_wanted(a.N, a.V, a.num_peds == nullptr, &a.team)) {
        const size_t lds = ((size_t)a.team.region_floats + 4 * team_ptab_floats() + 2 * kXrFwd + wave_param_floats(a.lay)) * sizeof(float);
        STG_REQUIRE(lds <= (size_t)kLdsBytes, STG_ELDS, "txp_fwd_team: V=%d needs %zu bytes of LDS", a.V, lds);
        return launch(Launch{"txp_fwd_team", dim3(team_grid(lds, a.N)), dim3(256), lds, st},
                      bf ? txp_fwd_team_kernel<true> : txp_fwd_team_kernel<false>, a, a.params, a.buffers);
    }
    STG_REQUIRE(a.V <= 16 * kF6Tiles / C, STG_EUNSUPPORTED, "txp_fwd_x6: V=%d outside the exact-bf16 kernels", a.V);
    const size_t per_wave = (size_t)(fwd6_region_floats(a.Vl) + ptab_floats(a.Vl)) * sizeof(float);
    const int wpb = wave_wpb(per_wave) == 8 ? 8 : 4;
    const size_t lds = per_wave * wpb + wave_param_floats(a.lay) * sizeof(float);
    bool ok;
    const Shape sh = canon_shape(a, &ok);
    STG_REQUIRE(ok && (sh != Shape::Canon32 || canon32_agg_matches(a)), STG_EINVAL,
                "txp_fwd_x6: the canonical V=%d batch does not match its compiled layout", a.V);
    return launch(Launch{"txp_fwd_x6", dim3(wave_grid(lds, wpb, a.N)), dim3(wpb * 64), lds, st},
                  wpb == 8 ? fwd_x6_kernel<8>(bf, sh) : fwd_x6_kernel<4>(bf, sh), a, a.params, a.buffers);
}

bool txp_bwd_x6_fits(const ModelLayout &L, int V) {
    return L.n_txp > 0 && V <= kTeamMaxV && L.n_blocks == 1 && L.blk[0].cin == Cfg::CIN0 &&
           !(L.flags & (STG_OPT_SPLIT_BF16 | STG_OPT_F32_MFMA)) && !diag_env("STG_BWD_F32", 0);
}
int64_t txp_bwd_x6_wp_floats(const ModelLayout &L) { return (int64_t)(L.L + 1) * cv::kWpDwords; }
int launch_txp_bwd_x6(const TxpBwdArgs &a0, hipStream_t st) {
    TxpBwdArgs a = a0;
    STG_REQUIRE(a.wp, STG_EINVAL, "txp_bwd_x6: the prepared operands are missing");
    const bool bf = (a.lay.flags & STG_OPT_BF16_STORE) != 0;
    if (team_wanted(a.N, a.V, a.num_peds == nullptr, &a.team)) {
        const size_t lds = ((size_t)a.team.region_floats + 4 * team_ptab_floats() + kXrBwdWg + wave_param_floats(a.lay)) * sizeof(float);
        STG_REQUIRE(lds <= (size_t)kLdsBytes, STG_ELDS, "txp_bwd_team: V=%d needs %zu bytes of LDS", a.V, lds);
        return launch(Launch{"txp_bwd_team", dim3(team_grid(lds, a.N)), dim3(256), lds, st},
                      bf ? txp_bwd_team_kernel<true> : txp_bwd_team_kernel<false>, a);
    }
    STG_REQUIRE(a.V <= 16 * kX6Tiles / C, STG_EUNSUPPORTED, "txp_bwd_x6: V=%d outside the exact-bf16 kernels", a.V);
    const size_t per_wave = (size_t)(bwd6_region_floats(a.Vl) + bwd_ptab_floats(a.Vl)) * sizeof(float);
    const int wpb = wave_wpb(per_wave) == 8 ? 8 : 4;
    const size_t lds = per_wave * wpb + wave_param_floats(a.lay) * sizeof(float);
    bool ok;
    const Shape sh = canon_shape(a, &ok);
    STG_REQUIRE(ok, STG_EINVAL, "txp_bwd_x6: the canonical V=%d batch does not match its compiled layout", a.V);
    return launch(Launch{"txp_bwd_x6", dim3(wave_grid(lds, wpb, a.N)), dim3(wpb * 64), lds, st},
                  wpb == 8 ? bwd_x6_kernel<8>(bf, sh) : bwd_x6_kernel<4>(bf, sh), a);
}

static bool step_x6_plain(int debug_skip_f, int debug_skip_b, int stagger_f, int stagger_b) {
    const size_t pf = (size_t)(fwd6_region_floats(kCanonV) + ptab_floats(kCanonV)) * sizeof(float);
    const size_t pb = (size_t)(bwd6_region_floats(kCanonV) + bwd_ptab_floats(kCanonV)) * sizeof(float);
    return !debug_skip_f && !debug_skip_b && !stagger_f && !stagger_b && wave_wpb(pf) != 8 && wave_wpb(pb) != 8;
}
bool txp_step_x6_fits(const ModelLayout &L, const int32_t *num_peds, int N, int V) {
    TeamGeom g;
    const int skip = diag_env("STG_DEBUG_SKIP", 0);
    return is_canonical(L) && V == kCanonV && !num_peds && txp_fwd_x6_fits(L, V) && txp_bwd_x6_fits(L, V) &&
           !team_wanted(N, V, true, &g) &&
           step_x6_plain(skip, skip, diag_env("STG_STAGGER_F", 0), diag_env("STG_STAGGER_B", 0));
}
static bool txp_step_x6_applies(const TxpFwdArgs &f, const TxpBwdArgs &b) {
    if (!f.wpf || !b.wp || !f.ws || f.ws != b.ws || f.N != b.N || f.V != b.V || f.params != b.params) return false;
    if (f.lay.flags != b.lay.flags || !step_x6_plain(f.debug_skip, b.debug_skip, f.stagger, b.stagger)) return false;
    TeamGeom g;
    if (team_wanted(f.N, f.V, f.num_peds == nullptr, &g) || team_wanted(b.N, b.V, b.num_peds == nullptr, &g)) return false;
    bool okf, okb;
    if (canon_shape(f, &okf) != Shape::Canon32 || canon_shape(b, &okb) != Shape::Canon32) return false;
    return okf && okb && canon32_agg_matches(f);
}
int launch_txp_step_x6(const TxpFwdArgs &f, const TxpBwdArgs &b, hipStream_t st) {
    STG_REQUIRE(txp_step_x6_applies(f, b), STG_EINVAL, "txp_step_x6: the batch is outside the one-launch scene kernel");
    constexpr int wpb = 4;
    const size_t lds = ((size_t)step6_per_wave_floats(kCanonV) * wpb + wave_param_floats(f.lay)) * sizeof(float);
    const bool bf = (f.lay.flags & STG_OPT_BF16_STORE) != 0;
    STG_REQUIRE(2 * lds <= (size_t)kLdsBytes, STG_ELDS, "txp_step_x6: %zu bytes of LDS do not fit two workgroups per CU", lds);
    return launch(Launch{"txp_step_x6", dim3((f.N + wpb - 1) / wpb), dim3(wpb * 64), lds, st},
                  bf ? txp_step_x6_kernel<wpb, true> : txp_step_x6_kernel<wpb, false>, f, b);
}

}
```

social_stgcnn_amd/ops.py:

```python
import collections
import ctypes
import dataclasses
import math

import torch

from . import _lib
from ._lib import ModelDesc, check, lib, peds_arg, ptr, require_gpu, seed_u64, stream_ptr


def _adj_layout(adj, n, t, v):
    if adj.dim() == 3:
        if tuple(adj.shape) != (t, v, v):
            raise ValueError("adjacency %s does not match x (T=%d, V=%d)" % (tuple(adj.shape), t, v))
        return adj.contiguous(), 0
    if adj.dim() == 4:
        if tuple(adj.shape) != (n, t, v, v):
            raise ValueError("adjacency %s does not match x (N=%d, T=%d, V=%d)" % (tuple(adj.shape), n, t, v))
        if adj.stride()[1:] != (v * v, v, 1):
            adj = adj.contiguous()
        return adj, adj.stride(0)
    raise ValueError("adjacency must be (T,V,V) or (N,T,V,V), got %d dims" % adj.dim())


def adj_build(seq_rel, num_peds=None, normalize=True, out=None):
    require_gpu(seq_rel)
    _lib.as_f32(seq_rel, "seq_rel")
    n, v, c, t = seq_rel.shape
    if c != 2:
        raise ValueError("seq_rel must be (N,V,2,T)")
    peds = peds_arg(num_peds, n, seq_rel.device)
    if out is not None:
        nodes, adj = out
        if tuple(nodes.shape) != (n, t, v, 2) or tuple(adj.shape) != (n, t, v, v) or not (
                nodes.is_contiguous() and adj.is_contiguous()):
            raise ValueError("adj_build: out = (nodes (N,T,V,2), adj (N,T,V,V)), contiguous")
    else:
        nodes = torch.empty((n, t, v, 2), device=seq_rel.device, dtype=torch.float32)
        adj = torch.empty((n, t, v, v), device=seq_rel.device, dtype=torch.float32)
    sn, sv, sc, st = seq_rel.stride()
    check(lib().stg_adj_build(ptr(seq_rel), sn, sv, sc, st, ptr(peds), n, v, t, 1 if normalize else 0,
                              ptr(nodes), ptr(adj), stream_ptr()), "stg_adj_build")
    return nodes, adj


class _SpatialAgg(torch.autograd.Function):
    @staticmethod
    def forward(ctx, x, adj, num_peds):
        require_gpu(x, adj)
        _lib.as_f32(x, "x")
        _lib.as_f32(adj, "adj")
        n, c, t, v = x.shape
        adj_c, a_sn = _adj_layout(adj, n, t, v)
        peds = peds_arg(num_peds, n, x.device)
        y = torch.empty((n, c, t, v), device=x.device, dtype=torch.float32)
        sn, sc, st, sv = x.stride()
        check(lib().stg_spatial_agg_fwd(ptr(x), sn, sc, st, sv, ptr(adj_c), a_sn, ptr(peds), n, c, t, v, ptr(y),
                                        stream_ptr()), "stg_spatial_agg_fwd")
        ctx.save_for_backward(adj_c, peds if peds is not None else torch.empty(0))
        ctx.a_sn = a_sn
        ctx.has_peds = peds is not None
        return y

    @staticmethod
    def backward(ctx, dy):
        adj_c, peds = ctx.saved_tensors
        dy = dy.contiguous()
        n, c, t, v = dy.shape
        dx = torch.empty_like(dy)
        check(lib().stg_spatial_agg_bwd(ptr(dy), ptr(adj_c), ctx.a_sn, ptr(peds) if ctx.has_peds else None, n, c, t,
                                        v, ptr(dx), stream_ptr()), "stg_spatial_agg_bwd")
        return dx, None, None


def spatial_agg(x, adj, num_peds=None):
    return _SpatialAgg.apply(x, adj, num_peds)


class _ConvT(torch.autograd.Function):
    @staticmethod
    def forward(ctx, x, weight, bias, pad, num_peds):
        require_gpu(x, weight, bias)
        _lib.as_f32(x, "x")
        n, cin, t, v = x.shape
        cout, cin_w, kt, kw = weight.shape
        if cin_w != cin or kw != 1:
            raise ValueError("weight %s does not match input channels %d" % (tuple(weight.shape), cin))
        to = t + 2 * pad - kt + 1
        peds = peds_arg(num_peds, n, x.device)
        w = weight.contiguous()
        b = bias.contiguous() if bias is not None else None
        y = torch.empty((n, cout, to, v), device=x.device, dtype=torch.float32)
        sn, sc, st, sv = x.stride()
        check(lib().stg_conv_t_fwd(ptr(x), sn, sc, st, sv, ptr(w), ptr(b), ptr(peds), n, cin, cout, t, v, kt, pad,
                                   ptr(y), stream_ptr()), "stg_conv_t_fwd")
        ctx.save_for_backward(x, w, peds if peds is not None else torch.empty(0))
        ctx.has_peds = peds is not None
        ctx.has_bias = bias is not None
        ctx.pad = pad
        return y

    @staticmethod
    def backward(ctx, dy):
        x, w, peds = ctx.saved_tensors
        dy = dy.contiguous()
        n, cin, t, v = x.shape
        cout, _, kt, _ = w.shape
        dx = torch.empty((n, cin, t, v), device=x.device, dtype=torch.float32) if ctx.needs_input_grad[0] else None
        dw = torch.zeros_like(w)
        db = torch.zeros(cout, device=x.device, dtype=torch.float32) if ctx.has_bias else None
        sn, sc, st, sv = x.stride()
        check(lib().stg_conv_t_bwd(ptr(x), sn, sc, st, sv, ptr(w), ptr(dy), ptr(peds) if ctx.has_peds else None, n,
                                   cin, cout, t, v, kt, ctx.pad, ptr(dx), ptr(dw), ptr(db), stream_ptr()),
              "stg_conv_t_bwd")
        return dx, dw, db, None, None


def conv_t(x, weight, bias, pad=0, num_peds=None):
    return _ConvT.apply(x, weight, bias, pad, num_peds)


def flat_walk(items):
    off = 0
    for i, it in enumerate(items):
        cnt = it.numel() if torch.is_tensor(it) else math.prod(it)
        yield i, off, cnt
        off += cnt


class FlatPack:

    def __init__(self):
        self.flat = None

    def ensure(self, tensors):
        total = sum(t.numel() for t in tensors)
        dev = tensors[0].device
        flat = self.flat
        if (flat is not None and flat.device == dev and flat.numel() == total
                and all(tensors[i].data_ptr() == flat.data_ptr() + 4 * off and tensors[i].is_contiguous()
                        for i, off, _ in flat_walk(tensors))):
            return flat
        flat = torch.empty(total, device=dev, dtype=torch.float32)
        with torch.no_grad():
            for i, off, n in flat_walk(tensors):
                t = tensors[i]
                flat[off:off + n].copy_(t.detach().reshape(-1))
                t.data = flat[off:off + n].view(t.shape)
        self.flat = flat
        return flat


class KernelOptions(dict):
    DEFAULTS = {"wg_path": False, "split_bf16": False, "wg_waves": 0, "wave_path": False, "bf16_store": False,
                "f32_mfma": False, "separate_fb": False, "generic_wgrad": False}

    def __init__(self, **kw):
        bad = set(kw) - set(self.DEFAULTS)
        if bad:
            raise KeyError("unknown kernel options %s" % sorted(bad))
        super().__init__(self.DEFAULTS)
        self.update(kw)


OPTIONS = KernelOptions()


def make_desc(n_stgcnn, n_txpcnn, c_in, c_out, t_obs, t_pred, kt, residual0, use_mdn, training,
              eps=1e-5, momentum=0.1, options=None):
    o = OPTIONS if options is None else options
    flags = ((_lib.OPT_WG_PATH if o["wg_path"] else 0) | (_lib.OPT_SPLIT_BF16 if o["split_bf16"] else 0)
             | (_lib.OPT_WAVE_PATH if o["wave_path"] else 0)
             | (_lib.OPT_BF16_STORE if o["bf16_store"] else 0)
             | (_lib.OPT_F32_MFMA if o["f32_mfma"] else 0)
             | (_lib.OPT_SEPARATE_FB if o["separate_fb"] else 0)
             | (_lib.OPT_GENERIC_WGRAD if o["generic_wgrad"] else 0))
    return ModelDesc(n_stgcnn, n_txpcnn, c_in, c_out, t_obs, t_pred, kt, residual0, 1 if use_mdn else 0,
                     1 if training else 0, eps, momentum, flags, int(o["wg_waves"]))


class KernelTimer:
    MAX_KERNELS = 8

    def __init__(self):
        self.calls = {"model_fwd": [], "model_bwd": []}

    def events(self, name):
        ev = _lib.HipEvents(self.MAX_KERNELS + 1)
        self.calls[name].append(ev)
        return ev

    def kernel_ms(self, name):
        rows = []
        for ev in self.calls[name]:
            row = []
            hip = ev.hip()
            hip.hipEventSynchronize(ev.arr[0])
            for k in range(1, ev.n):
                ms = ctypes.c_float()
                if hip.hipEventElapsedTime(ctypes.byref(ms), ev.arr[k - 1], ev.arr[k]) != 0:
                    hip.hipGetLastError()
                    break
                row.append(ms.value)
            rows.append(row)
        if not rows:
            return []
        n = min(len(r) for r in rows)
        return [sum(r[k] for r in rows) / len(rows) for k in range(n)]

    def mean_ms(self, name):
        return sum(self.kernel_ms(name))


def _timer_of(holder):
    return getattr(holder, "timer", None) if holder is not None else None


def _size(n, what):
    if n < 0:
        check(int(n), what)
    return int(n)


def _ptr_array(tensors):
    return (ctypes.c_void_p * len(tensors))(*[t.data_ptr() for t in tensors]) if len(tensors) else None


@dataclasses.dataclass(eq=False)
class FwdRecord:
    desc: ModelDesc
    a_sn: int
    dead: frozenset
    shapes: list
    flat_params: torch.Tensor
    flat_buffers: torch.Tensor
    x: torch.Tensor
    adj_c: torch.Tensor
    peds: torch.Tensor
    ws: torch.Tensor
    stats: torch.Tensor = None
    nbt: list = None
    n: int = 0


def _check_model_input(x, adj, desc, flat_params, flat_buffers):
    require_gpu(x, adj, flat_params, flat_buffers)
    _lib.as_f32(x, "x")
    _lib.as_f32(adj, "adj")
    n, cin, t, v = x.shape
    if cin != desc.c_in or t != desc.t_obs:
        raise ValueError("input (N,%d,%d,V) does not match the model (input_feat=%d, seq_len=%d)"
                         % (cin, t, desc.c_in, desc.t_obs))
    return n, cin, t, v


def _fwd_buffers(desc, n, v, dev, save, training, holder):
    L, d = lib(), ctypes.byref(desc)
    out_t = desc.t_pred if desc.n_txpcnn > 0 else desc.t_obs
    y = torch.empty((n, desc.c_out, out_t, v), device=dev, dtype=torch.float32)
    ws = None
    if save:
        wsf = _size(L.stg_model_ws_floats(d, v), "stg_model_ws_floats")
        tail = _size(L.stg_model_ws_tail_floats(d, n, v), "stg_model_ws_tail_floats")
        ws = torch.empty(n * wsf + tail, device=dev, dtype=torch.float32)
    stats = None
    if training:
        sf = L.stg_model_stat_floats(d)
        stats = torch.empty((n, max(int(sf), 1)), device=dev, dtype=torch.float32)
    scr = None
    nscr = _size(L.stg_model_fwd_scratch_floats(d, n, v), "stg_model_fwd_scratch_floats")
    if nscr > 0:
        scr = torch.empty(nscr, device=dev, dtype=torch.float32)
    if holder is not None:
        holder.last_ws_floats = ws.numel() if save else 0
        holder._last_fwd_scratch = scr
    return y, ws, stats, scr


def _bwd_buffers(desc, n, v, dev):
    L, d = lib(), ctypes.byref(desc)
    np_ = int(L.stg_model_param_count(d))
    n_scratch = _size(L.stg_model_bwd_scratch_floats(d, n, v), "stg_model_bwd_scratch_floats")
    slabs = torch.empty(n_scratch, device=dev, dtype=torch.float32)
    grad = torch.empty(np_, device=dev, dtype=torch.float32)
    return slabs, grad


def _step_tail(flat_params, flat_buffers, step, stats, nbt):
    lr, lr_dev = step
    total = torch.empty(1, device=flat_params.device, dtype=torch.float32)
    tail = _lib.StepTail()
    tail.params, tail.lr_dev, tail.lr = ptr(flat_params), ptr(lr_dev), float(lr)
    tail.total = ptr(total)
    arr = None
    if stats is not None:
        arr = _ptr_array(nbt)
        tail.stats, tail.buffers, tail.nbt, tail.n_bn = ptr(stats), ptr(flat_buffers), arr, len(nbt)
    return tail, total, arr


def _grad_views(grad, shapes, dead, holder):
    if holder is not None:
        holder._flat_grad = grad
        holder._fwd_state = None
    return [None if i in dead else grad[off:off + cnt].view(shapes[i]) for i, off, cnt in flat_walk(shapes)]


class _FusedModel(torch.autograd.Function):

    @staticmethod
    def forward(ctx, x, adj, num_peds, desc, flat_params, flat_buffers, nbt, dead, holder, grad_on, defer_bn_fold,
                *params):
        n, cin, t, v = _check_model_input(x, adj, desc, flat_params, flat_buffers)
        L = lib()
        adj_c, a_sn = _adj_layout(adj, n, t, v)
        peds = peds_arg(num_peds, n, x.device)
        training = desc.bn_mode == 1
        need_grad = grad_on and any(ctx.needs_input_grad)
        if need_grad and ctx.needs_input_grad[0] and not (desc.flags & _lib.OPT_WG_PATH):
            fields = {f: getattr(desc, f) for f, _ in ModelDesc._fields_}
            fields["flags"] |= _lib.OPT_WG_PATH
            desc = ModelDesc(**fields)
        y, ws, stats, scr = _fwd_buffers(desc, n, v, x.device, need_grad, training, holder)
        sn, sc, st, sv = x.stride()
        timer = _timer_of(holder)
        ev = timer.events("model_fwd") if timer is not None else None
        check(L.stg_model_fwd(ctypes.byref(desc), ptr(flat_params), ptr(flat_buffers), ptr(x), sn, sc, st, sv,
                              ptr(adj_c), a_sn, ptr(peds), n, v, ptr(y), ptr(ws), ptr(stats), ptr(scr),
                              ev.arr if ev else None, ev.n if ev else 0, stream_ptr()),
              "stg_model_fwd")
        rec = FwdRecord(desc, a_sn, dead, [tuple(p.shape) for p in params], flat_params, flat_buffers, x, adj_c, peds,
                        ws)
        if training and defer_bn_fold:
            rec.stats, rec.nbt, rec.n = stats, nbt, n
        elif training:
            check(L.stg_bn_fold(ctypes.byref(desc), ptr(stats), ptr(peds), n, ptr(flat_buffers), _ptr_array(nbt),
                                len(nbt), stream_ptr()), "stg_bn_fold")
        if holder is not None:
            holder._fwd_state = rec if need_grad else None
        ctx.rec = rec
        ctx.holder = holder
        return y

    @staticmethod
    def backward(ctx, dy):
        if ctx.rec.ws is None:
            raise RuntimeError("backward through a forward that saved no activations")
        grads, dx = _launch_backward(ctx.rec, ctx.holder, dy=dy.contiguous(), need_dx=ctx.needs_input_grad[0])
        return (dx, None, None, None, None, None, None, None, None, None, None, *grads)


def _launch_backward(rec, holder, dy=None, need_dx=False, y=None, target=None, weights=None, step=None):
    L = lib()
    desc, x = rec.desc, rec.x
    n, cin, t, v = x.shape
    slabs, grad = _bwd_buffers(desc, n, v, x.device)
    sn, sc, st, sv = x.stride()
    timer = _timer_of(holder)
    ev = timer.events("model_bwd") if timer is not None else None
    head = (ctypes.byref(desc), ptr(rec.flat_params), ptr(rec.flat_buffers), ptr(x), sn, sc, st, sv, ptr(rec.adj_c),
            rec.a_sn, ptr(rec.peds), n, v)
    end = (ev.arr if ev else None, ev.n if ev else 0, stream_ptr())
    if dy is not None:
        out = torch.empty((n, cin, t, v), device=x.device, dtype=torch.float32) if need_dx else None
        name, rc = "stg_model_bwd", L.stg_model_bwd(*head, ptr(dy), ptr(rec.ws), ptr(slabs), ptr(grad), ptr(out), *end)
    else:
        out = losses = torch.empty(n, device=x.device, dtype=torch.float32)
        mid = (ptr(y), ptr(target), ptr(weights), ptr(losses), ptr(rec.ws), ptr(slabs), ptr(grad))
        if step is None:
            name, rc = "stg_model_bwd_nll", L.stg_model_bwd_nll(*head, *mid, *end)
        else:
            tail, total, keep = _step_tail(rec.flat_params, rec.flat_buffers, step, rec.stats, rec.nbt)
            name, rc = "stg_model_bwd_step", L.stg_model_bwd_step(*head, *mid, ctypes.addressof(tail), *end)
            out = (losses, total[0])
        if rc == _lib.EUNSUPPORTED:
            if ev is not None:
                timer.calls["model_bwd"].pop()
            return None
    check(rc, name)
    return _grad_views(grad, rec.shapes, rec.dead, holder), out


def backward_from_target(holder, y, target, weights=None, step=None):
    rec = getattr(holder, "_fwd_state", None)
    if rec is None:
        raise RuntimeError("backward_from_target: no fused forward with saved activations to start from")
    n, _, _, v = rec.x.shape
    if tuple(y.shape) != (n, 5, rec.desc.t_pred, v) or not y.is_contiguous():
        return None
    target = target.to(torch.float32).contiguous()
    if tuple(target.shape) != (n, rec.desc.t_pred, v, 2):
        raise ValueError("backward_from_target: target (N,P,V,2) expected, got %s" % (tuple(target.shape),))
    w = weights.to(torch.float32).contiguous() if weights is not None else None
    res = _launch_backward(rec, holder, y=y, target=target, weights=w, step=step)
    if res is None:
        return None
    for p, g in zip(holder._tensors()[0], res[0]):
        p.grad = g
    return res[1]


def fused_step(x, adj, num_peds, desc, flat_params, flat_buffers, nbt, dead, params, holder, target, weights, lr,
               lr_dev):
    n, cin, t, v = _check_model_input(x, adj, desc, flat_params, flat_buffers)
    if desc.bn_mode != 1 or desc.n_txpcnn < 1 or n == 0 or (desc.flags & _lib.OPT_SPLIT_BF16):
        return None
    target = target.to(torch.float32).contiguous()
    if tuple(target.shape) != (n, desc.t_pred, v, 2):
        raise ValueError("fused_step: target (N,P,V,2) expected, got %s" % (tuple(target.shape),))
    w = weights.to(torch.float32).contiguous() if weights is not None else None
    adj_c, a_sn = _adj_layout(adj, n, t, v)
    peds = peds_arg(num_peds, n, x.device)
    y, ws, stats, scr = _fwd_buffers(desc, n, v, x.device, True, True, holder)
    slabs, grad = _bwd_buffers(desc, n, v, x.device)
    if holder is not None:
        holder._last_bwd_scratch = slabs
    losses = torch.empty(n, device=x.device, dtype=torch.float32)
    tail, total, keep = _step_tail(flat_params, flat_buffers, (lr, lr_dev), stats, nbt)
    timer = _timer_of(holder)
    ev_f = timer.events("model_fwd") if timer is not None else None
    ev_b = timer.events("model_bwd") if timer is not None else None
    sn, sc, st, sv = x.stride()
    rc = lib().stg_model_step(ctypes.byref(desc), ptr(flat_params), ptr(flat_buffers), ptr(x), sn, sc, st, sv, ptr(adj_c),
                              a_sn, ptr(peds), n, v, ptr(y), ptr(ws), ptr(stats), ptr(scr), ptr(target), ptr(w),
                              ptr(losses), ptr(slabs), ptr(grad), ctypes.addressof(tail),
                              ev_f.arr if ev_f else None, ev_f.n if ev_f else 0,
                              ev_b.arr if ev_b else None, ev_b.n if ev_b else 0, stream_ptr())
    if rc == _lib.EUNSUPPORTED:
        if timer is not None:
            timer.calls["model_fwd"].pop()
            timer.calls["model_bwd"].pop()
        return None
    check(rc, "stg_model_step")
    return y, losses, total[0], _grad_views(grad, [tuple(p.shape) for p in params], dead, holder)


def fused_model(x, adj, num_peds, desc, flat_params, flat_buffers, nbt, dead, params, holder=None,
                defer_bn_fold=False):
    return _FusedModel.apply(x, adj, num_peds, desc, flat_params, flat_buffers, nbt, dead, holder,
                             torch.is_grad_enabled(), defer_bn_fold, *params)


class _BivariateNLL(torch.autograd.Function):

    @staticmethod
    def forward(ctx, pred, target, num_peds):
        require_gpu(pred, target)
        _lib.as_f32(pred, "V_pred")
        n, p, v, f = pred.shape
        if f != 5 or tuple(target.shape) != (n, p, v, 2):
            raise ValueError("bivariate_loss: V_pred (..,P,V,5) / V_trgt (..,P,V,2) expected, got %s / %s"
                             % (tuple(pred.shape), tuple(target.shape)))
        target = target.to(torch.float32).contiguous()
        peds = peds_arg(num_peds, n, pred.device)
        loss = torch.empty(n, device=pred.device, dtype=torch.float32)
        need = ctx.needs_input_grad[0]
        grad = torch.empty((n, 5, p, v), device=pred.device, dtype=torch.float32) if need else None
        sn, sp, sv, sf = pred.stride()
        check(lib().stg_nll_fwd(ptr(pred), sn, sf, sp, sv, ptr(target), ptr(peds), None, n, p, v, ptr(loss), ptr(grad),
                                stream_ptr()), "stg_nll_fwd")
        ctx.grad = grad
        return loss

    @staticmethod
    def backward(ctx, gloss):
        grad = ctx.grad
        n, _, p, v = grad.shape
        gloss = gloss.to(torch.float32).contiguous()
        out = torch.empty_like(grad)
        check(lib().stg_nll_bwd(ptr(grad), ptr(gloss), n, p, v, ptr(out), stream_ptr()), "stg_nll_bwd")
        return out.permute(0, 2, 3, 1), None, None


def bivariate_nll(pred, target, num_peds=None):
    return _BivariateNLL.apply(pred, target, num_peds)


def bivariate_nll_with_grad(y, target, num_peds=None, weights=None):
    require_gpu(y, target)
# ... 461 lines not shown
```

Before: 10.58 million scene-windows/s.

## Write hidden-layer dz gradients in place over workspace z slots in fused step

In the one-launch fused forward+backward step kernel, hidden TXP layer gradients dz are now written over the forward workspace z slots instead of a separate dz scratch region. The bf16 weight-gradient kernel reads dz from those slots using the workspace stride. The aim is a smaller memory footprint and better locality, since dz sits next to the plane data the weight-gradient pass already streams. It adds a SEPARATE_DZ opt-out flag, and the f32 weight-gradient kernel rejects the in-place mode.

```diff
diff --git a/include/stgcnn_hip.h b/include/stgcnn_hip.h
--- a/include/stgcnn_hip.h
+++ b/include/stgcnn_hip.h
@@ -60,6 +60,7 @@
 #define STG_OPT_F32_MFMA 16
 #define STG_OPT_SEPARATE_FB 32
 #define STG_OPT_GENERIC_WGRAD 64
+#define STG_OPT_SEPARATE_DZ 128
 #define STG_OPT_WAVE_PATH 4
 
 int64_t stg_model_param_count(const stg_model_desc *d);
@@ -267,6 +268,8 @@
 
 #include "stgcnn_hip_assoc_filter.h"
 
+#include "stgcnn_hip_step_plan.h"
+
 #ifdef __cplusplus
 }
 #endif
diff --git a/include/stgcnn_hip_step_plan.h b/include/stgcnn_hip_step_plan.h
--- /dev/null
+++ b/include/stgcnn_hip_step_plan.h
@@ -0,0 +1,11 @@
+#ifndef STGCNN_HIP_STEP_PLAN_H
+#define STGCNN_HIP_STEP_PLAN_H
+#ifndef STGCNN_HIP_H
+#error "include stgcnn_hip.h, which includes this file"
+#endif
+
+int stg_model_step_dz_in_place(const stg_model_desc *d, int has_num_peds, int N, int V);
+int64_t stg_model_ws_z_offset(const stg_model_desc *d, int V, int layer);
+int64_t stg_model_bwd_dz_offset(const stg_model_desc *d, int N, int V);
+
+#endif
diff --git a/social_stgcnn_amd/_lib.py b/social_stgcnn_amd/_lib.py
--- a/social_stgcnn_amd/_lib.py
+++ b/social_stgcnn_amd/_lib.py
@@ -11,6 +11,7 @@
 ABI_VERSION = 8
 OPT_WG_PATH, OPT_SPLIT_BF16, OPT_WAVE_PATH, OPT_BF16_STORE, OPT_F32_MFMA, OPT_SEPARATE_FB = 1, 2, 4, 8, 16, 32
 OPT_GENERIC_WGRAD = 64
+OPT_SEPARATE_DZ = 128
 EUNSUPPORTED = -2
 
 c_f = ctypes.c_void_p
@@ -158,6 +159,11 @@
     "stg_associate_streams_filtered": (c_i, [c_f, c_l, c_f, c_l, c_i, c_f, c_f, c_f, c_f, c_i, c_i, c_f, c_f, c_f, c_f,
                                              c_f, c_f, c_f, c_f, c_i, c_d, c_d, c_d, c_d, c_d, c_d, c_l, c_l, c_f]),
 }
+_SIGNATURES_STEP_PLAN = {
+    "stg_model_step_dz_in_place": (c_i, [ctypes.POINTER(ModelDesc), c_i, c_i, c_i]),
+    "stg_model_ws_z_offset": (c_l, [ctypes.POINTER(ModelDesc), c_i, c_i]),
+    "stg_model_bwd_dz_offset": (c_l, [ctypes.POINTER(ModelDesc), c_i, c_i]),
+}
 
 _lib = None
 
@@ -183,7 +189,7 @@
         h = ctypes.CDLL(LIB_PATH)
         for name, (res, args) in {**_SIGNATURES, **_SIGNATURES_SCORE_TIME, **_SIGNATURES_HARVEST,
                                     **_SIGNATURES_HARVEST_TIME, **_SIGNATURES_ASSOC_TIME,
-                                    **_SIGNATURES_ASSOC_FILTER}.items():
+                                    **_SIGNATURES_ASSOC_FILTER, **_SIGNATURES_STEP_PLAN}.items():
             fn = getattr(h, name)
             fn.restype = res
             fn.argtypes = args
diff --git a/social_stgcnn_amd/csrc/model_bwd.hip b/social_stgcnn_amd/csrc/model_bwd.hip
--- a/social_stgcnn_amd/csrc/model_bwd.hip
+++ b/social_stgcnn_amd/csrc/model_bwd.hip
@@ -419,6 +419,13 @@
 int64_t stg_model_bwd_stamps_offset(const stg_model_desc *d, int N, int V) {
     return stg::bwd_query("stg_model_bwd_stamps_offset:", d, N, V, &stg::BwdCarve::stamps);
 }
+int64_t stg_model_bwd_dz_offset(const stg_model_desc *d, int N, int V) {
+    stg::StepPlan p;
+    const int rc = stg::plan_sized("stg_model_bwd_dz_offset:", d, nullptr, N, V, 1, &p);
+    if (rc != STG_OK) return rc;
+    if (p.lay.n_txp == 0) return STG_EUNSUPPORTED;
+    return stg::bwd_query("stg_model_bwd_dz_offset:", d, N, V, &stg::BwdCarve::dzg);
+}
 
 }
 
@@ -447,6 +454,7 @@
     const int n_small = L.n_blk_params + L.n_txp;
     float *rows = b.scratch + cv.rows, *slab2 = b.scratch + cv.slab2;
     float *dzg = L.n_txp > 0 ? b.scratch + cv.dzg : nullptr;
+    const bool dz_in_place = deferred && p.dz_in_place;
     STG_REQUIRE(path.scene() || !(L.flags & STG_OPT_BF16_STORE), STG_EUNSUPPORTED,
                 "stg_model_bwd: bf16 storage (STG_OPT_BF16_STORE) is built for the wave-per-scene kernels only");
     STG_REQUIRE(!((L.flags & STG_OPT_BF16_STORE) && (L.flags & STG_OPT_SPLIT_BF16)), STG_EUNSUPPORTED,
@@ -482,7 +490,7 @@
         if (p.tail.wp >= 0) t.wp = reinterpret_cast<const unsigned *>(ws_end + p.tail.wp);
         if (cv.stamps >= 0) t.stamps = reinterpret_cast<unsigned long long *>(b.scratch + cv.stamps);
         STG_REQUIRE(!deferred || p.one_launch, STG_EINVAL, "stg_model_bwd: a deferred scene launch outside the one-launch step");
-        const int rcw = deferred ? launch_scene_step(*deferred, t, st) : launch_scene_bwd(path, t, st);
+        const int rcw = deferred ? launch_scene_step(*deferred, t, dz_in_place, st) : launch_scene_bwd(path, t, st);
         if (rcw != STG_OK) return rcw;
         slab_rows = N;
     } else {
@@ -531,6 +539,7 @@
         w.order = tier.order; w.order_peds = sorted ? so.order_peds : nullptr; w.key_start = tier.key_start;
         w.serpentine = tier.serpentine;
         w.slab2 = slab2; w.rows = wg.rows;
+        w.dz_in_ws = dz_in_place ? 1 : 0;
         for (int l = 0; l <= L.L + 1; ++l) w.wg_begin[l] = wg.wg_begin[l];
         if (!STG_SKIP(w, 1)) {
             const int rck = launch_txp_wgrad(w, wg, st);
diff --git a/social_stgcnn_amd/csrc/model_layout.hip b/social_stgcnn_amd/csrc/model_layout.hip
--- a/social_stgcnn_amd/csrc/model_layout.hip
+++ b/social_stgcnn_amd/csrc/model_layout.hip
@@ -24,7 +24,7 @@
     STG_REQUIRE(d->residual0 >= 0 && d->residual0 <= 2, STG_EINVAL, "residual0=%d", d->residual0);
     STG_REQUIRE(d->residual0 != 1 || d->c_in == d->c_out, STG_EINVAL, "identity residual needs c_in == c_out");
     STG_REQUIRE((d->flags & ~(STG_OPT_WG_PATH | STG_OPT_SPLIT_BF16 | STG_OPT_WAVE_PATH | STG_OPT_BF16_STORE | STG_OPT_F32_MFMA |
-                              STG_OPT_SEPARATE_FB | STG_OPT_GENERIC_WGRAD)) == 0, STG_EINVAL,
+                              STG_OPT_SEPARATE_FB | STG_OPT_GENERIC_WGRAD | STG_OPT_SEPARATE_DZ)) == 0, STG_EINVAL,
                 "unknown flags 0x%x", d->flags);
     STG_REQUIRE(d->wg_waves == 0 || d->wg_waves == 1 || d->wg_waves == 2 || d->wg_waves == 4 || d->wg_waves == 8,
                 STG_EINVAL, "wg_waves=%d (0 auto, 1, 2, 4, 8)", d->wg_waves);
@@ -97,11 +97,15 @@
     return path.kind == StepPath::SceneX6 && path.fwd_x6 && path.bwd_x6 && !(L.flags & STG_OPT_SEPARATE_FB) &&
            txp_step_x6_fits(L, num_peds, N, V);
 }
-int launch_scene_step(const TxpFwdArgs &f, const TxpBwdArgs &b, hipStream_t st) { return launch_txp_step_x6(f, b, st); }
+static bool step_dz_in_place(const ModelLayout &L, bool one_launch) { return one_launch && !(L.flags & STG_OPT_SEPARATE_DZ); }
+int launch_scene_step(const TxpFwdArgs &f, const TxpBwdArgs &b, bool dz_in_place, hipStream_t st) {
+    return launch_txp_step_x6(f, b, dz_in_place, st);
+}
 
 int plan_step(const stg_model_desc *d, const int32_t *num_peds, int N, int V, StepPlan *p) {
     const int rc = make_layout(d, &p->lay);
     p->sized = rc == STG_OK && N >= 0 && V > 0;
+    p->one_launch = p->dz_in_place = false;
     if (!p->sized) return rc;
     const ModelLayout &L = p->lay;
     p->path = choose_path(L, N, V);
@@ -109,6 +113,7 @@
     p->tail = ws_tail(L, p->path, N, V);
     p->fwd = fwd_carve(L, p->path, N, V);
     p->one_launch = step_one_launch(L, p->path, num_peds, N, V);
+    p->dz_in_place = step_dz_in_place(L, p->one_launch);
     return STG_OK;
 }
 int plan_sized(const char *what, const stg_model_desc *d, const int32_t *num_peds, int N, int V, int min_N, StepPlan *p) {
@@ -171,6 +176,20 @@
     stg::StepPlan p;
     const int rc = stg::plan_sized("stg_model_fwd_stamps_offset:", d, nullptr, N, V, 0, &p);
     return rc != STG_OK ? rc : p.fwd.stamps >= 0 ? p.fwd.stamps : STG_EUNSUPPORTED;
+}
+int stg_model_step_dz_in_place(const stg_model_desc *d, int has_num_peds, int N, int V) {
+    static const int32_t given = 0;
+    stg::StepPlan p;
+    const int rc = stg::plan_sized("stg_model_step_dz_in_place:", d, has_num_peds ? &given : nullptr, N, V, 0, &p);
+    return rc == STG_OK ? (p.dz_in_place ? 1 : 0) : rc;
+}
+int64_t stg_model_ws_z_offset(const stg_model_desc *d, int V, int layer) {
+    stg::ModelLayout l;
+    const int rc = stg::make_layout(d, &l);
+    if (rc != STG_OK) return rc;
+    if (V <= 0 || layer < 0 || layer >= l.L || l.n_txp == 0)
+        return stg::fail(STG_EINVAL, "stg_model_ws_z_offset: V=%d layer=%d (hidden TXP layers: %d)", V, layer, l.n_txp ? l.L : 0);
+    return l.ws_hdr_floats + (int64_t)l.ws_z[layer] * V;
 }
 int stg_scene_order(const int32_t *num_peds, int N, int V, int32_t *order, int32_t *key_start, void *stream) {
     STG_REQUIRE(N >= 0 && V > 0, STG_EINVAL, "stg_scene_order: bad sizes N=%d V=%d", N, V);
diff --git a/social_stgcnn_amd/csrc/step_plan.hpp b/social_stgcnn_amd/csrc/step_plan.hpp
--- a/social_stgcnn_amd/csrc/step_plan.hpp
+++ b/social_stgcnn_amd/csrc/step_plan.hpp
@@ -27,11 +27,11 @@
 int launch_scene_fwd(const StepPath &path, const TxpFwdArgs &a, hipStream_t st);
 int launch_scene_bwd(const StepPath &path, const TxpBwdArgs &a, hipStream_t st);
 
-int launch_scene_step(const TxpFwdArgs &f, const TxpBwdArgs &b, hipStream_t st);
+int launch_scene_step(const TxpFwdArgs &f, const TxpBwdArgs &b, bool dz_in_place, hipStream_t st);
 
 struct StepPlan {
     ModelLayout lay;
-    bool sized, one_launch;
+    bool sized, one_launch, dz_in_place;
     StepPath path;
     int64_t ws_stride;
     WsTail tail;
diff --git a/social_stgcnn_amd/csrc/txp_scene_common.hpp b/social_stgcnn_amd/csrc/txp_scene_common.hpp
--- a/social_stgcnn_amd/csrc/txp_scene_common.hpp
+++ b/social_stgcnn_amd/csrc/txp_scene_common.hpp
@@ -76,7 +76,7 @@
 int launch_txp_fwd_x6(const TxpFwdArgs &a, hipStream_t st);
 int launch_txp_bwd_x6(const TxpBwdArgs &a, hipStream_t st);
 bool txp_step_x6_fits(const ModelLayout &L, const int32_t *num_peds, int N, int V);
-int launch_txp_step_x6(const TxpFwdArgs &f, const TxpBwdArgs &b, hipStream_t st);
+int launch_txp_step_x6(const TxpFwdArgs &f, const TxpBwdArgs &b, bool dz_in_place, hipStream_t st);
 
 __host__ __device__ inline int ptab_floats(int v) { return ((Cfg::T * v + 1) / 2 + 3) & ~3; }
 __host__ __device__ inline int bwd_ptab_floats(int v) { return ptab_floats(v) + kRedMax; }
diff --git a/social_stgcnn_amd/csrc/txp_wgrad.hip b/social_stgcnn_amd/csrc/txp_wgrad.hip
--- a/social_stgcnn_amd/csrc/txp_wgrad.hip
+++ b/social_stgcnn_amd/csrc/txp_wgrad.hip
@@ -291,6 +291,7 @@
 
 int launch_txp_wgrad(const WgradArgs &w, const WgradGeom &g, hipStream_t st) {
     if (g.bf16mma) return launch_txp_wgrad_bf16(w, g, st);
+    STG_REQUIRE(!w.dz_in_ws, STG_EINVAL, "txp_wgrad: dz_l in the workspace is read by the bf16-pipe kernels only");
     const Launch lc{"txp_wgrad", dim3(g.grid), dim3(kWaves * 64), g.lds, st};
     const bool bf16 = (w.lay.flags & STG_OPT_BF16_STORE) != 0;
     if (g.nbuf == 3)
diff --git a/social_stgcnn_amd/csrc/txp_wgrad.hpp b/social_stgcnn_amd/csrc/txp_wgrad.hpp
--- a/social_stgcnn_amd/csrc/txp_wgrad.hpp
+++ b/social_stgcnn_amd/csrc/txp_wgrad.hpp
@@ -39,6 +39,7 @@
     const int32_t *key_start;
     int serpentine;
     int N, V;
+    int dz_in_ws;
     const float *ws;
     const float *dzg;
     int64_t ws_stride;
diff --git a/social_stgcnn_amd/csrc/txp_wgrad_bf16.hip b/social_stgcnn_amd/csrc/txp_wgrad_bf16.hip
--- a/social_stgcnn_amd/csrc/txp_wgrad_bf16.hip
+++ b/social_stgcnn_amd/csrc/txp_wgrad_bf16.hip
@@ -127,8 +127,17 @@
     const int64_t dzs_floats = dz_slot(V);
     const bool bf = BF;
     constexpr int64_t kDzScene = (int64_t)(kCanonLayout.L + 1) * dz_slot(kCanonV);
+    static_assert(kCanonLayout.ws_z[kCanonLayout.L - 1] == kCanonLayout.ws_z[0] + (kCanonLayout.L - 1) * C * P &&
+                      ((kCanonLayout.ws_hdr_floats + kCanonLayout.ws_z[0] * kCanonV) * 4) % 128 == 0 && (C * P * kCanonV * 4) % 128 == 0,
+                  "Canon32: the z slots are C * P units apart and 128-byte aligned");
+    const bool dz_ws = a.dz_in_ws != 0 && layer < (K32 ? kCanonLayout.L : L.L);
+    const float *const dz_base =
+        !dz_ws ? a.dzg + layer * dzs_floats
+               : a.ws + (K32 ? kCanonLayout.ws_hdr_floats + (int64_t)(kCanonLayout.ws_z[0] + layer * (C * P)) * kCanonV
+                             : L.ws_hdr_floats + (int64_t)L.ws_z[layer] * V);
+    const int64_t dz_stride = dz_ws ? (K32 ? kCanonWs32 : a.ws_stride) : (K32 ? kDzScene : (int64_t)(L.L + 1) * dzs_floats);
     auto plane32 = [&](int n) { return a.ws + n * kCanonWs32 + plane_off; };
-    auto dz32 = [&](int n) { return a.dzg + n * kDzScene + layer * (int64_t)dz_slot(kCanonV); };
+    auto dz32 = [&](int n) { return dz_base + n * dz_stride; };
     auto fetch = [&](int r) -> Item {
         Item it{0, 0, 0, 0, false, nullptr, nullptr};
         const int at = walk_item(r, wg, nwg, items, order != nullptr && a.serpentine);
@@ -155,7 +164,7 @@
         if (vfull == 0 || chunk >= nc) return it;
         const int wc = nc > 1 ? (vfull + nc - 1) / nc : vfull;
         it.pl = a.ws + n * a.ws_stride + plane_off;
-        it.dz = a.dzg + ((int64_t)n * (L.L + 1) + layer) * dzs_floats;
+        it.dz = dz_base + n * dz_stride;
         it.w0 = chunk * wc;
         it.vc = (vfull - it.w0) < wc ? (vfull - it.w0) : wc;
         it.swf = save_sw(vfull, bf);
@@ -383,7 +392,7 @@
             convert32(cur, s, sm + ib);
             n += nwg;
             pl += nwg * kCanonWs32;
-            dz += nwg * kDzScene;
+            dz += nwg * dz_stride;
             const bool nxt = n < a.N;
             load32(nxt, pl, dz, s);
             team_barrier();
diff --git a/social_stgcnn_amd/csrc/txp_x6.hip b/social_stgcnn_amd/csrc/txp_x6.hip
--- a/social_stgcnn_amd/csrc/txp_x6.hip
+++ b/social_stgcnn_amd/csrc/txp_x6.hip
@@ -237,7 +237,7 @@
     return ((img > tail ? img : tail) + 3) & ~3;
 }
 
-template <bool BF, typename CK, Shape SH = Shape::Generic>
+template <bool BF, typename CK, Shape SH = Shape::Generic, bool ZIN = false>
 __device__ __forceinline__ void txp_bwd_scene_x6(const TxpBwdArgs &a, const float *blk_params, int n, int vi, float *region,
                                                  ptab_t *ptab, const CK &ck) {
     const ModelLayout &L = a.lay;
@@ -291,7 +291,8 @@
     for (int t = 0; t < kX6Tiles; ++t) dcur[t] = f32x4{0.f, 0.f, 0.f, 0.f};
 
     for (int l = L.L; l >= 0; --l) {
-        float *dzo = a.dzg + ((int64_t)n * (L.L + 1) + l) * dz_slot(V);
+        float *dzo = (ZIN && l != L.L) ? const_cast<float *>(wsn) + L.ws_hdr_floats + (int64_t)lay_ws_z<SH>(L, l) * V
+                                       : a.dzg + ((int64_t)n * (L.L + 1) + l) * dz_slot(V);
         if (STG_SKIP(a, 512) || (l == L.L && STG_SKIP(a, 2048)) || (l != L.L && STG_SKIP(a, 4096))) {
         } else if (l == L.L) {
             const int wcw = ck.wc();
@@ -519,7 +520,7 @@
     return f > b ? f : b;
 }
 
-template <int WPB, bool BF>
+template <int WPB, bool BF, bool ZIN>
 __global__ __launch_bounds__(WPB * 64, 2) __attribute__((amdgpu_waves_per_eu(2, 2))) void txp_step_x6_kernel(
     const TxpFwdArgs f0, const TxpBwdArgs b0) {
     constexpr Shape S = Shape::Canon32;
@@ -546,7 +547,7 @@
     __builtin_amdgcn_fence(__ATOMIC_ACQUIRE, "wavefront");
     STG_X6_STAMP(f, n, 8);
     STG_X6_STAMP(b, n, 0);
-    txp_bwd_scene_x6<BF, SoloScene, S>(b, blk_p, n, kCanonV, region, ptab, SoloScene{kCanonV});
+    txp_bwd_scene_x6<BF, SoloScene, S, ZIN>(b, blk_p, n, kCanonV, region, ptab, SoloScene{kCanonV});
     __builtin_amdgcn_wave_barrier();
     STG_X6_STAMP(b, n, 8);
 }
@@ -805,14 +806,15 @@
     if (canon_shape(f, &okf) != Shape::Canon32 || canon_shape(b, &okb) != Shape::Canon32) return false;
     return okf && okb && canon32_agg_matches(f);
 }
-int launch_txp_step_x6(const TxpFwdArgs &f, const TxpBwdArgs &b, hipStream_t st) {
+int launch_txp_step_x6(const TxpFwdArgs &f, const TxpBwdArgs &b, bool dz_in_place, hipStream_t st) {
     STG_REQUIRE(txp_step_x6_applies(f, b), STG_EINVAL, "txp_step_x6: the batch is outside the one-launch scene kernel");
     constexpr int wpb = 4;
     const size_t lds = ((size_t)step6_per_wave_floats(kCanonV) * wpb + wave_param_floats(f.lay)) * sizeof(float);
     const bool bf = (f.lay.flags & STG_OPT_BF16_STORE) != 0;
     STG_REQUIRE(2 * lds <= (size_t)kLdsBytes, STG_ELDS, "txp_step_x6: %zu bytes of LDS do not fit two workgroups per CU", lds);
-    return launch(Launch{"txp_step_x6", dim3((f.N + wpb - 1) / wpb), dim3(wpb * 64), lds, st},
-                  bf ? txp_step_x6_kernel<wpb, true> : txp_step_x6_kernel<wpb, false>, f, b);
-}
-
-}
+    const auto k = dz_in_place ? (bf ? txp_step_x6_kernel<wpb, true, true> : txp_step_x6_kernel<wpb, false, true>)
+                               : (bf ? txp_step_x6_kernel<wpb, true, false> : txp_step_x6_kernel<wpb, false, false>);
+    return launch(Launch{"txp_step_x6", dim3((f.N + wpb - 1) / wpb), dim3(wpb * 64), lds, st}, k, f, b);
+}
+
+}
diff --git a/social_stgcnn_amd/ops.py b/social_stgcnn_amd/ops.py
--- a/social_stgcnn_amd/ops.py
+++ b/social_stgcnn_amd/ops.py
@@ -153,7 +153,7 @@
 
 class KernelOptions(dict):
     DEFAULTS = {"wg_path": False, "split_bf16": False, "wg_waves": 0, "wave_path": False, "bf16_store": False,
-                "f32_mfma": False, "separate_fb": False, "generic_wgrad": False}
+                "f32_mfma": False, "separate_fb": False, "generic_wgrad": False, "separate_dz": False}
 
     def __init__(self, **kw):
         bad = set(kw) - set(self.DEFAULTS)
@@ -174,7 +174,8 @@
              | (_lib.OPT_BF16_STORE if o["bf16_store"] else 0)
              | (_lib.OPT_F32_MFMA if o["f32_mfma"] else 0)
              | (_lib.OPT_SEPARATE_FB if o["separate_fb"] else 0)
-             | (_lib.OPT_GENERIC_WGRAD if o["generic_wgrad"] else 0))
+             | (_lib.OPT_GENERIC_WGRAD if o["generic_wgrad"] else 0)
+             | (_lib.OPT_SEPARATE_DZ if o["separate_dz"] else 0))
     return ModelDesc(n_stgcnn, n_txpcnn, c_in, c_out, t_obs, t_pred, kt, residual0, 1 if use_mdn else 0,
                      1 if training else 0, eps, momentum, flags, int(o["wg_waves"]))
 
```

Result: faster. 10.87 million scene-windows/s, median of 3 (+2.7%).
